# thangvubk/SoftGroup

Hardware: AMD Instinct MI355X
Metric: scans/sec ScanNet-v2-like inference (softgroup_scannet.yaml, full forward_test) (higher is better)
Workload: dtype f32

## Files before the change

### include/softgroup_hip.h

```cpp
#ifndef SOFTGROUP_HIP_H
#define SOFTGROUP_HIP_H

#include <stddef.h>
#include <stdint.h>

#ifdef __cplusplus
extern "C" {
#endif

typedef void *sg_stream_t;

#define SG_OK 0
#define SG_ERR_ARG (-1)
#define SG_ERR_WORKSPACE (-2)
#define SG_ERR_LAUNCH (-3)
#define SG_ERR_UNSUPPORTED (-4)

#define SG_BALLQUERY_MAX_NEIGHBORS 1000
#define SG_OCTREE_NUM_NODES 585
#define SG_OCTREE_NUM_LEAVES 512
#define SG_LISTS_SORTED 1
#define SG_LISTS_RADIUS 2

int sg_version(void);
const char *sg_last_error(void);
int sg_device_info(char *name_host, int name_cap, int *num_cu_host, int *clock_khz_host);

int sg_stream_release(sg_stream_t stream);
int sg_stream_create(sg_stream_t *stream_out);
int sg_stream_destroy(sg_stream_t stream);
int sg_stream_create_priority(sg_stream_t *stream_out, int level);

int sg_voxelize_idx_host(const int64_t *coords_host, int n, int ncol, int mode,
                         int32_t *input_map_host, int32_t *num_voxels_host,
                         int32_t *max_active_host);
int sg_voxelize_idx_fill_host(const int64_t *coords_host, int n, int ncol, int mode,
                              const int32_t *input_map_host, int num_voxels, int max_active,
                              int64_t *out_coords_host, int32_t *out_map_host);
size_t sg_voxelize_idx_workspace_bytes(int n);
int sg_voxelize_idx_build(const int64_t *coords, int n, int ncol, int mode, int32_t *input_map,
                          int32_t *meta, void *ws, size_t ws_bytes, sg_stream_t stream);
int sg_voxelize_idx_fill(const int64_t *coords, int n, int ncol, int mode,
                         const int32_t *input_map, int num_voxels, int max_active,
                         int64_t *out_coords, int32_t *out_map, void *ws, size_t ws_bytes,
                         sg_stream_t stream);

int sg_voxelize_fp(const float *feats, const int32_t *rules, int num_voxels, int max_active,
                   int channels, int average, float *out, sg_stream_t stream);
int sg_voxelize_bp(const float *d_out, const int32_t *rules, int num_voxels, int max_active,
                   int channels, int average, float *d_feats, sg_stream_t stream);

size_t sg_ballquery_workspace_bytes(int n);
int sg_ballquery_build_grid(const float *xyz, const int32_t *batch_idxs, int n, float radius,
                            void *ws, size_t ws_bytes, sg_stream_t stream);
int sg_ballquery_count(const float *xyz, const int32_t *batch_idxs, int n, float radius,
                       int32_t *start_len, int32_t *meta, void *ws, size_t ws_bytes,
                       sg_stream_t stream);
int sg_ballquery_fill(const float *xyz, const int32_t *batch_idxs, int n, float radius,
                      const int32_t *start_len, int32_t *idx, void *ws, size_t ws_bytes,
                      sg_stream_t stream);
size_t sg_scan_workspace_bytes(int n);
int sg_exclusive_scan_startlen(int32_t *start_len, int n, int32_t *meta, void *ws,
                               size_t ws_bytes, sg_stream_t stream);

int sg_octree_build_host(const float *points_host, const float *xyzwhl_host, int num_points,
                         int num_levels, float *boxes_host, int32_t *pt_inds_host,
                         int32_t *pt_start_len_host);
size_t sg_octree_build_workspace_bytes(int n);
int sg_octree_build(const float *points, int n, float *boxes, int32_t *pt_inds, int32_t *pt_start_len,
                    void *ws, size_t ws_bytes, sg_stream_t stream);
size_t sg_pyramid_inverse_map_workspace_bytes(int n_points, int n_voxels, int n_prop);
int sg_pyramid_inverse_map(const int32_t *proposals_idx, int64_t num_pairs, int n_prop,
                           const int32_t *l2p_map, int n_points, int n_voxels, int32_t *out_idx,
                           int32_t *out_offsets, int32_t *n_out_dev, void *ws, size_t ws_bytes,
                           sg_stream_t stream);
int sg_octree_ballquery_count(const float *points, const float *boxes, const int32_t *pt_inds,
                              const int32_t *pt_start_len, int n, float radius,
                              int32_t *start_len, sg_stream_t stream);
int sg_octree_ballquery_fill(const float *points, const float *boxes, const int32_t *pt_inds,
                             const int32_t *pt_start_len, int n, float radius,
                             const int32_t *start_len, int32_t *idx, sg_stream_t stream);

size_t sg_bfs_workspace_bytes(int n, int64_t n_edges);
int sg_bfs_cluster_label(const int32_t *bq_idxs, const int32_t *start_len, int n,
                         int64_t n_edges, int list_flags, const int32_t *seg_of_point,
                         const float *seg_thr, int n_seg, int32_t *n_cluster_host,
                         int32_t *sum_npoint_host, void *ws, size_t ws_bytes, sg_stream_t stream);
int sg_bfs_cluster_emit(const int32_t *bq_idxs, const int32_t *start_len, int n, int64_t n_edges,
                        const int32_t *seg_of_point, const float *seg_thr, int n_cluster,
                        int sum_npoint, int32_t *cluster_idxs, int32_t *cluster_offsets, void *ws,
                        size_t ws_bytes, sg_stream_t stream);

int sg_sec_mean(const float *inp, const int32_t *offsets, int n_seg, int channels, float *out,
                sg_stream_t stream);
int sg_sec_min(const float *inp, const int32_t *offsets, int n_seg, int channels, float *out,
               sg_stream_t stream);
int sg_sec_max(const float *inp, const int32_t *offsets, int n_seg, int channels, float *out,
               sg_stream_t stream);
int sg_global_avg_pool_fp(const float *feats, const int32_t *offsets, int n_seg, int channels,
                          float *out, sg_stream_t stream);
int sg_global_avg_pool_bp(float *d_feats, const int32_t *offsets, const float *d_out, int n_seg,
                          int channels, sg_stream_t stream);

int sg_get_mask_iou_on_cluster(const int32_t *proposals_idx, const int32_t *proposals_offset,
                               const int64_t *instance_labels, const int32_t *instance_pointnum,
                               int n_instance, int n_proposal, float *proposals_iou,
                               sg_stream_t stream);
int sg_get_mask_iou_on_pred(const int32_t *proposals_idx, const int32_t *proposals_offset,
                            const int64_t *instance_labels, const int32_t *instance_pointnum,
                            const float *mask_scores_sigmoid, int n_instance, int n_proposal,
                            float *proposals_iou, sg_stream_t stream);
int sg_get_mask_label(const int32_t *proposals_idx, const int32_t *proposals_offset,
                      const int64_t *instance_labels, const int64_t *instance_cls,
                      const float *proposals_iou, int n_instance, int n_proposal, float iou_thr,
                      float *mask_label, sg_stream_t stream);

size_t sg_spconv_hash_workspace_bytes(int num_rows);
int sg_spconv_subm_rulebook(const int32_t *indices, int num_rows, const int32_t *spatial_shape_host,
                            int32_t *nbr, void *ws, size_t ws_bytes, sg_stream_t stream);
int sg_spconv_down_build(const int32_t *indices, int num_rows, const int32_t *spatial_shape_host,
                         int32_t *in2out, int32_t *meta, void *ws, size_t ws_bytes,
                         sg_stream_t stream);
int sg_spconv_down_fill(const int32_t *indices, int num_rows, const int32_t *in2out,
                        int num_out_rows, int32_t *out_indices, int32_t *child, void *ws,
                        size_t ws_bytes, sg_stream_t stream);
int sg_spconv_inverse_rulebook(const int32_t *indices_fine, const int32_t *in2out, int num_rows,
                               int32_t *inv_nbr, sg_stream_t stream);

#define SG_PLAN_HIST_WORDS 40
size_t sg_spconv_plan_workspace_bytes(int num_out_rows);
int sg_spconv_plan(const int32_t *nbr, int num_out_rows, int kvol, int32_t *order,
                   uint32_t *tile_mask, int32_t *nbr_tiles, void *ws, size_t ws_bytes,
                   sg_stream_t stream);

#define SG_PYRAMID_MAX_LEVELS 10
typedef struct sg_plan_ptrs {
  int32_t *order;
  uint32_t *tile_mask;
  int32_t *nbr_tiles;
} sg_plan_ptrs;
typedef struct sg_pyramid_level {
  int rows;
  int32_t *indices;
  int32_t *nbr;
  sg_plan_ptrs subm;
  int32_t *in2out;
  int32_t *child;
  sg_plan_ptrs down;
  int32_t *inv;
  sg_plan_ptrs up;
} sg_pyramid_level;
size_t sg_spconv_pyramid_workspace_bytes(int num_rows, int n_levels);
int sg_spconv_pyramid_rows(const int32_t *indices, int num_rows, const int32_t *spatial_shape_host,
                           int n_levels, int32_t *rows_dev, void *ws, size_t ws_bytes,
                           sg_stream_t stream);
size_t sg_spconv_pyramid_build_workspace_bytes(const sg_pyramid_level *levels_host, int n_levels);
int sg_spconv_pyramid_build(const int32_t *indices, int num_rows, const int32_t *spatial_shape_host,
                            int n_levels, const sg_pyramid_level *levels_host, void *ws,
                            size_t ws_bytes, void *ws2, size_t ws2_bytes, sg_stream_t stream);

size_t sg_spconv_packed_weight_elems(int kvol, int cin, int cout);
int sg_spconv_pack_weight(const float *w, int cout, int kvol, int cin, int src_is_kio, float *w_k8,
                          sg_stream_t stream);

size_t sg_spconv_conv_workspace_bytes(int num_out_rows, int cout);
int sg_spconv_gather_conv_f32(const float *in, int num_in_rows, const int32_t *nbr,
                              int num_out_rows, int kvol, int cin, int cout, const float *w_k8,
                              const float *post_scale, const float *post_shift,
                              const float *residual, const float *act_scale,
                              const float *act_shift, float *out_act, const int32_t *order,
                              const uint32_t *tile_mask, const int32_t *nbr_tiles, float *out,
                              void *ws, size_t ws_bytes, sg_stream_t stream);

int sg_spconv_set_arithmetic(int mode);

int sg_spconv_set_combine(int mode);

int sg_grouping_set_lanes(int lanes);

int sg_spconv_set_chain(int mode);
int sg_spconv_chain_stats(int64_t *launches, int64_t *steps);

int sg_spconv_profile(int enable);
int sg_spconv_profile_read(double *total_ms, int *launches);
int sg_spconv_profile_detail(float *ms, int32_t *dims, int cap, int *calls);

typedef struct sg_mlp2 {
  const float *w1, *b1, *bn_scale, *bn_shift, *w2, *b2;
  int out;
} sg_mlp2;
int sg_pointwise_heads(const float *voxel_feats, const void *v2p_map, int v2p_is_int64, int n_points,
                       int channels, const sg_mlp2 *semantic, const sg_mlp2 *offset, float *output_feats,
                       float *semantic_scores, float *pt_offsets, int64_t *semantic_preds,
                       sg_stream_t stream);

size_t sg_spconv_packed_weight_elems_bf16(int kvol, int cin, int cout);
int sg_spconv_pack_weight_bf16(const float *w, int cout, int kvol, int cin, int src_is_kio,
                               uint16_t *w_k8_bf16, sg_stream_t stream);
size_t sg_spconv_conv_bf16_workspace_bytes(int num_out_rows, int cout);
int sg_spconv_gather_conv_bf16(const uint16_t *in, int num_in_rows, const int32_t *nbr, int num_out_rows,
                               int kvol, int cin, int cout, const uint16_t *w_k8_bf16,
                               const int32_t *order, const uint32_t *tile_mask, const int32_t *nbr_tiles,
                               uint16_t *out, void *ws, size_t ws_bytes, sg_stream_t stream);

int sg_spconv_transpose_table(const int32_t *nbr, int num_out_rows, int kvol, int32_t *nbr_t,
                              sg_stream_t stream);
size_t sg_spconv_wgrad_workspace_bytes(int num_out_rows, int kvol, int cin, int cout);
int sg_spconv_wgrad(const void *in, int in_is_bf16, const void *g_out, int g_is_bf16, const int32_t *nbr_t,
                    int num_out_rows, int kvol, int cin, int cout, float *dw_kio, void *ws,
                    size_t ws_bytes, sg_stream_t stream);

typedef struct sg_unet_block {
  int cin, cout;
  const float *bn1_scale, *bn1_shift;
  const float *w1;
  const float *bn2_scale, *bn2_shift;
  const float *w2;
  const float *w_i;
} sg_unet_block;
typedef struct sg_unet_level {
  int planes, n_blocks;
  const sg_unet_block *blocks;
  const sg_unet_block *tail;
  const float *down_bn_scale, *down_bn_shift, *down_w;
  const float *up_bn_scale, *up_bn_shift, *up_w;
} sg_unet_level;
typedef struct sg_unet_desc {
  int n_levels;
  const sg_unet_level *levels;
  int input_cin;
  const float *input_w;
  const float *out_bn_scale, *out_bn_shift;
  int input_cin_packed;
  int arithmetic;
} sg_unet_desc;
size_t sg_unet_arena_bytes(const sg_unet_desc *desc, int num_rows);
int sg_unet_forward(const sg_unet_desc *desc, const float *feats, const int32_t *indices,
                    int num_rows, const int32_t *spatial_shape_host, float *out, void *arena,
                    size_t arena_bytes, sg_stream_t stream);

typedef struct sg_train_bn {
  const float *weight, *bias;
  float *running_mean, *running_var;
  float momentum, eps;
  float *g_weight, *g_bias;
} sg_train_bn;
typedef struct sg_train_conv {
  const float *w;
  float *g_w;
} sg_train_conv;
typedef struct sg_unet_train_block {
  int cin, cout;
  sg_train_bn bn1, bn2;
  sg_train_conv c1, c2, ci;
} sg_unet_train_block;
typedef struct sg_unet_train_level {
  int planes, n_blocks;
  const sg_unet_train_block *blocks, *tail;
  sg_train_bn down_bn, up_bn;
  sg_train_conv down, up;
} sg_unet_train_level;
typedef struct sg_unet_train_desc {
  int n_levels;
  const sg_unet_train_level *levels;
  int input_cin;
  sg_train_conv input;
  sg_train_bn out_bn;
  int arithmetic;
} sg_unet_train_desc;
size_t sg_unet_train_arena_hint(const sg_unet_train_desc *desc, int num_rows);
int sg_unet_train_forward(const sg_unet_train_desc *desc, const float *feats, const int32_t *indices,
                          int num_rows, const int32_t *spatial_shape_host, float *out, void *arena,
                          size_t arena_bytes, size_t *arena_needed, void **tape, sg_stream_t stream);
int sg_unet_train_backward(void *tape, const float *g_out, float *g_feats, sg_stream_t stream);
void sg_unet_train_release(void *tape);

int sg_bn_relu_f32(const float *x, const float *scale, const float *shift, int64_t num_rows,
                   int channels, int relu, float *out, sg_stream_t stream);

int sg_gather_rows_f32(const float *in, const int32_t *index, int64_t num_out_rows, int channels,
                       float *out, sg_stream_t stream);
int sg_gather_rows_i64idx_f32(const float *in, const int64_t *index, int64_t num_out_rows,
                              int channels, float *out, sg_stream_t stream);

int sg_instance_npoint(const int32_t *proposals_idx, const float *mask_scores, int64_t num_pairs,
                       int stride, int n_classes, float mask_thr, int n_prop, int32_t *npoint,
                       sg_stream_t stream);
size_t sg_instance_runs_workspace_bytes(int n_kept, int n_points);
int sg_instance_runs(const int32_t *proposals_idx, const float *mask_scores, int64_t num_pairs,
                     int stride, int n_classes, float mask_thr, const int32_t *inst_of, int n_prop,
                     int n_kept, int n_points, int32_t *starts, int32_t *ends, int64_t *bounds,
                     int64_t runs_capacity, void *ws, size_t ws_bytes, sg_stream_t stream);

int64_t sg_rle_format_bound(int64_t total_runs, int digits);
int sg_rle_format_host(const int64_t *starts_host, const int64_t *lens_host,
                       const int64_t *bounds_host, int n_groups, char *out_host,
                       int64_t out_capacity, int64_t *out_offsets_host);
size_t sg_rle_format_device_workspace_bytes(int64_t run_capacity);
int64_t sg_rle_format_device_text_bytes(int64_t run_capacity, int64_t length);
int sg_rle_format_device(const int32_t *starts, const int32_t *ends, const int64_t *bounds, int n_inst,
                         int64_t run_capacity, int64_t length, uint8_t *text, int64_t text_capacity,
                         int64_t *text_off, void *ws, size_t ws_bytes, sg_stream_t stream);
int sg_rle_format_runs_host(const int32_t *starts_host, const int32_t *ends_host,
                            const int64_t *bounds_host, int n_groups, char *out_host,
                            int64_t out_capacity, int64_t *out_offsets_host);

size_t sg_panoptic_fusion_workspace_bytes(int n_inst, int n_points);
int sg_panoptic_fusion(const uint32_t *bits, int n_inst, int n_points, const int32_t *order,
                       const int32_t *label_id, const int64_t *semantic_preds, int cls_offset,
                       double skip_iou, int semantic_classes, int thing_class_min, uint32_t *out,
                       void *ws, size_t ws_bytes, sg_stream_t stream);

#define SG_NMS_IOU 0
#define SG_NMS_MIN 1
size_t sg_mask_nms_workspace_bytes(int n_inst, int64_t n_points);
int sg_mask_nms(const uint32_t *bits, int n_inst, int64_t n_points, const float *scores, const int32_t *labels,
                double thr, int measure, int class_agnostic, uint8_t *keep, int32_t *n_keep, int32_t *inter_out,
                void *ws, size_t ws_bytes, sg_stream_t stream);
int sg_mask_bits_from_runs(const int32_t *starts, const int32_t *ends, const int64_t *bounds, int64_t n_runs,
                           int n_inst, int64_t n_points, uint32_t *bits, sg_stream_t stream);

typedef struct sg_grouping_cfg {
  int n_points;
  int n_sem_classes;
  int n_seg;
  const int32_t *seg_class;
  const float *seg_thr;
  float score_thr;
  int min_npoint;
  float radius;
  int batch_size;
  float voxel_scale;
  int voxel_shape;
  int feat_channels;
} sg_grouping_cfg;
typedef struct sg_grouping_result {
  int n_selected, n_neighbours, n_proposals, sum_npoint, n_voxels, max_active;
  size_t proposals_idx;
  size_t proposals_offset;
  size_t voxel_coords;
  size_t voxel_offsets;
  size_t voxel_feats;
  size_t point_to_voxel;
  size_t arena_used, arena_needed;
  int deferred_classes;
  int reserved_;
} sg_grouping_result;
int sg_scan_grouping(const sg_grouping_cfg *cfg, const float *scores, const float *pt_offsets,
                     const float *coords_float, const int32_t *batch_idxs, const float *point_feats,
                     void *arena, size_t arena_bytes, sg_grouping_result *result_host,
                     sg_stream_t stream);

typedef struct sg_grouping_pp_cfg {
  sg_grouping_cfg base;
  int with_pyramid, with_octree, lvl_fusion;
  double radius;
  double base_size;
} sg_grouping_pp_cfg;
int sg_scan_grouping_pp(const sg_grouping_pp_cfg *cfg, const float *scores, const float *pt_offsets,
                        const float *coords_float, const int32_t *batch_idxs, const float *point_feats,
                        void *arena, size_t arena_bytes, sg_grouping_result *result_host,
                        sg_stream_t stream);

int sg_host_copy_2d(void *dst, int64_t dst_pitch_bytes, const void *src, int64_t src_pitch_bytes, int64_t rows,
                    int64_t row_bytes);
int sg_host_cast_f64_f32(float *dst, const double *src, int64_t n);
int sg_host_fill_i64_strided(int64_t *dst, int64_t pitch_elems, int64_t rows, int64_t value);
int sg_host_colmax_i64(const int64_t *src, int64_t rows, int64_t cols, int64_t *out_max);

typedef struct sg_instances_cfg {
  int n_proposals, n_classes;
  int score_stride;
  int64_t sum_npoint;
  int n_points;
  float cls_score_thr, mask_score_thr;
  int min_npoint;
} sg_instances_cfg;
typedef struct sg_instances_result {
  int n_kept;
  size_t off_class, off_score, off_text, text_bytes;
  size_t host_needed, arena_used, arena_needed;
  size_t bits;
  size_t label_id;
} sg_instances_result;
int sg_scan_instances(const sg_instances_cfg *cfg, const int32_t *proposals_idx, const float *mask_scores,
                      const float *cls_prob, const float *iou_scores, void *arena, size_t arena_bytes,
                      void *host_out, size_t host_bytes, sg_instances_result *result_host,
                      sg_stream_t stream);

typedef struct sg_linear {
  const float *w, *b;
  int out, in;
// ... 288 lines not shown
```

### softgroup_amd/_lib.py

```python
import ctypes as C
import os

_HERE = os.path.dirname(os.path.abspath(__file__))
LIB_PATH = os.path.join(_HERE, 'lib', os.environ.get('SG_LIB_NAME', 'libsoftgroup_hip.so'))

_lib = None

_vp, _i, _f, _i64, _sz, _d = C.c_void_p, C.c_int, C.c_float, C.c_int64, C.c_size_t, C.c_double
_pi32 = C.POINTER(C.c_int32)

SIGNATURES = {
    'sg_version': (_i, []),
    'sg_last_error': (C.c_char_p, []),
    'sg_device_info': (_i, [C.c_char_p, _i, C.POINTER(_i), C.POINTER(_i)]),
    'sg_stream_release': (_i, [_vp]),
    'sg_host_copy_2d': (_i, [_vp, _i64, _vp, _i64, _i64, _i64]),
    'sg_host_cast_f64_f32': (_i, [_vp, _vp, _i64]),
    'sg_host_fill_i64_strided': (_i, [_vp, _i64, _i64, _i64]),
    'sg_host_colmax_i64': (_i, [_vp, _i64, _i64, _vp]),
    'sg_stream_create': (_i, [_vp]),
    'sg_stream_create_priority': (_i, [_vp, _i]),
    'sg_stream_destroy': (_i, [_vp]),
    'sg_voxelize_idx_host': (_i, [_vp, _i, _i, _i, _vp, _pi32, _pi32]),
    'sg_voxelize_idx_fill_host': (_i, [_vp, _i, _i, _i, _vp, _i, _i, _vp, _vp]),
    'sg_voxelize_idx_workspace_bytes': (_sz, [_i]),
    'sg_voxelize_idx_build': (_i, [_vp, _i, _i, _i, _vp, _vp, _vp, _sz, _vp]),
    'sg_voxelize_idx_fill': (_i, [_vp, _i, _i, _i, _vp, _i, _i, _vp, _vp, _vp, _sz, _vp]),
    'sg_voxelize_fp': (_i, [_vp, _vp, _i, _i, _i, _i, _vp, _vp]),
    'sg_voxelize_bp': (_i, [_vp, _vp, _i, _i, _i, _i, _vp, _vp]),
    'sg_ballquery_workspace_bytes': (_sz, [_i]),
    'sg_ballquery_build_grid': (_i, [_vp, _vp, _i, _f, _vp, _sz, _vp]),
    'sg_ballquery_count': (_i, [_vp, _vp, _i, _f, _vp, _vp, _vp, _sz, _vp]),
    'sg_ballquery_fill': (_i, [_vp, _vp, _i, _f, _vp, _vp, _vp, _sz, _vp]),
    'sg_scan_workspace_bytes': (_sz, [_i]),
    'sg_exclusive_scan_startlen': (_i, [_vp, _i, _vp, _vp, _sz, _vp]),
    'sg_octree_build_host': (_i, [_vp, _vp, _i, _i, _vp, _vp, _vp]),
    'sg_octree_build_workspace_bytes': (_sz, [_i]),
    'sg_octree_build': (_i, [_vp, _i, _vp, _vp, _vp, _vp, _sz, _vp]),
    'sg_pyramid_inverse_map_workspace_bytes': (_sz, [_i, _i, _i]),
    'sg_pyramid_inverse_map': (_i, [_vp, _i64, _i, _vp, _i, _i, _vp, _vp, _vp, _vp, _sz, _vp]),
    'sg_octree_ballquery_count': (_i, [_vp, _vp, _vp, _vp, _i, _f, _vp, _vp]),
    'sg_octree_ballquery_fill': (_i, [_vp, _vp, _vp, _vp, _i, _f, _vp, _vp, _vp]),
    'sg_bfs_workspace_bytes': (_sz, [_i, _i64]),
    'sg_bfs_cluster_label': (_i, [_vp, _vp, _i, _i64, _i, _vp, _vp, _i, _pi32, _pi32, _vp, _sz, _vp]),
    'sg_bfs_cluster_emit': (_i, [_vp, _vp, _i, _i64, _vp, _vp, _i, _i, _vp, _vp, _vp, _sz, _vp]),
    'sg_sec_mean': (_i, [_vp, _vp, _i, _i, _vp, _vp]),
    'sg_sec_min': (_i, [_vp, _vp, _i, _i, _vp, _vp]),
    'sg_sec_max': (_i, [_vp, _vp, _i, _i, _vp, _vp]),
    'sg_global_avg_pool_fp': (_i, [_vp, _vp, _i, _i, _vp, _vp]),
    'sg_global_avg_pool_bp': (_i, [_vp, _vp, _vp, _i, _i, _vp]),
    'sg_get_mask_iou_on_cluster': (_i, [_vp, _vp, _vp, _vp, _i, _i, _vp, _vp]),
    'sg_get_mask_iou_on_pred': (_i, [_vp, _vp, _vp, _vp, _vp, _i, _i, _vp, _vp]),
    'sg_get_mask_label': (_i, [_vp, _vp, _vp, _vp, _vp, _i, _i, _f, _vp, _vp]),
    'sg_spconv_hash_workspace_bytes': (_sz, [_i]),
    'sg_spconv_subm_rulebook': (_i, [_vp, _i, _pi32, _vp, _vp, _sz, _vp]),
    'sg_spconv_pyramid_workspace_bytes': (_sz, [_i, _i]),
    'sg_spconv_pyramid_rows': (_i, [_vp, _i, _pi32, _i, _vp, _vp, _sz, _vp]),
    'sg_spconv_pyramid_build_workspace_bytes': (_sz, [_vp, _i]),
    'sg_spconv_pyramid_build': (_i, [_vp, _i, _pi32, _i, _vp, _vp, _sz, _vp, _sz, _vp]),
    'sg_spconv_down_build': (_i, [_vp, _i, _pi32, _vp, _vp, _vp, _sz, _vp]),
    'sg_spconv_down_fill': (_i, [_vp, _i, _vp, _i, _vp, _vp, _vp, _sz, _vp]),
    'sg_spconv_inverse_rulebook': (_i, [_vp, _vp, _i, _vp, _vp]),
    'sg_spconv_plan_workspace_bytes': (_sz, [_i]),
    'sg_spconv_plan': (_i, [_vp, _i, _i, _vp, _vp, _vp, _vp, _sz, _vp]),
    'sg_spconv_set_arithmetic': (_i, [_i]),
    'sg_spconv_set_combine': (_i, [_i]),
    'sg_spconv_set_chain': (_i, [_i]),
    'sg_grouping_set_lanes': (_i, [_i]),
    'sg_spconv_chain_stats': (_i, [_vp, _vp]),
    'sg_spconv_profile': (_i, [_i]),
    'sg_spconv_profile_read': (_i, [_vp, _vp]),
    'sg_spconv_profile_detail': (_i, [_vp, _vp, _i, _vp]),
    'sg_unet_arena_bytes': (_sz, [_vp, _i]),
    'sg_unet_forward': (_i, [_vp, _vp, _vp, _i, _vp, _vp, _vp, _sz, _vp]),
    'sg_unet_train_arena_hint': (_sz, [_vp, _i]),
    'sg_unet_train_forward': (_i, [_vp, _vp, _vp, _i, _vp, _vp, _vp, _sz, _vp, _vp, _vp]),
    'sg_unet_train_backward': (_i, [_vp, _vp, _vp, _vp]),
    'sg_unet_train_release': (None, [_vp]),
    'sg_pointwise_heads': (_i, [_vp, _vp, _i, _i, _i, _vp, _vp, _vp, _vp, _vp, _vp, _vp]),
    'sg_spconv_packed_weight_elems': (_sz, [_i, _i, _i]),
    'sg_spconv_pack_weight': (_i, [_vp, _i, _i, _i, _i, _vp, _vp]),
    'sg_spconv_conv_workspace_bytes': (_sz, [_i, _i]),
    'sg_spconv_gather_conv_f32': (_i, [_vp, _i, _vp, _i, _i, _i, _i, _vp, _vp, _vp, _vp, _vp, _vp,
                                       _vp, _vp, _vp, _vp, _vp, _vp, _sz, _vp]),
    'sg_spconv_packed_weight_elems_bf16': (_sz, [_i, _i, _i]),
    'sg_spconv_pack_weight_bf16': (_i, [_vp, _i, _i, _i, _i, _vp, _vp]),
    'sg_spconv_conv_bf16_workspace_bytes': (_sz, [_i, _i]),
    'sg_spconv_gather_conv_bf16': (_i, [_vp, _i, _vp, _i, _i, _i, _i, _vp, _vp, _vp, _vp, _vp, _vp, _sz,
                                        _vp]),
    'sg_spconv_transpose_table': (_i, [_vp, _i, _i, _vp, _vp]),
    'sg_spconv_wgrad_workspace_bytes': (_sz, [_i, _i, _i, _i]),
    'sg_spconv_wgrad': (_i, [_vp, _i, _vp, _i, _vp, _i, _i, _i, _i, _vp, _vp, _sz, _vp]),
    'sg_instance_npoint': (_i, [_vp, _vp, _i64, _i, _i, _f, _i, _vp, _vp]),
    'sg_instance_runs_workspace_bytes': (_sz, [_i, _i]),
    'sg_instance_runs': (_i, [_vp, _vp, _i64, _i, _i, _f, _vp, _i, _i, _i, _vp, _vp, _vp, _i64, _vp, _sz, _vp]),
    'sg_rle_format_bound': (_i64, [_i64, _i]),
    'sg_rle_format_host': (_i, [_vp, _vp, _vp, _i, _vp, _i64, _vp]),
    'sg_rle_format_device_workspace_bytes': (_sz, [_i64]),
    'sg_rle_format_device_text_bytes': (_i64, [_i64, _i64]),
    'sg_rle_format_device': (_i, [_vp, _vp, _vp, _i, _i64, _i64, _vp, _i64, _vp, _vp, _sz, _vp]),
    'sg_rle_format_runs_host': (_i, [_vp, _vp, _vp, _i, _vp, _i64, _vp]),
    'sg_panoptic_fusion_workspace_bytes': (_sz, [_i, _i]),
    'sg_panoptic_fusion': (_i, [_vp, _i, _i, _vp, _vp, _vp, _i, C.c_double, _i, _i, _vp, _vp, _sz, _vp]),
    'sg_mask_nms_workspace_bytes': (_sz, [_i, _i64]),
    'sg_mask_nms': (_i, [_vp, _i, _i64, _vp, _vp, _d, _i, _i, _vp, _vp, _vp, _vp, _sz, _vp]),
    'sg_mask_bits_from_runs': (_i, [_vp, _vp, _vp, _i64, _i, _i64, _vp, _vp]),
    'sg_scan_grouping': (_i, [_vp, _vp, _vp, _vp, _vp, _vp, _vp, _sz, _vp, _vp]),
    'sg_scan_grouping_pp': (_i, [_vp, _vp, _vp, _vp, _vp, _vp, _vp, _sz, _vp, _vp]),
    'sg_scan_instances': (_i, [_vp, _vp, _vp, _vp, _vp, _vp, _sz, _vp, _sz, _vp, _vp]),
    'sg_softmax_rows': (_i, [_vp, _i64, _i, _vp, _vp]),
    'sg_mlp_rows': (_i, [_vp, _vp, _i64, _i, _vp, _vp, _vp]),
    'sg_linear_rows': (_i, [_vp, _i64, _vp, _vp, _vp]),
    'sg_scan_arena_bytes': (_sz, [_vp, _i, _i]),
    'sg_scan_forward': (_i, [_vp, _vp, _vp, _sz, _vp, _sz, _vp, _sz, _vp, _vp]),
    'sg_eval_intersections': (_i, [_vp, _vp, _vp, _i, _i64, _vp, _i, _i, _vp, _vp]),
    'sg_eval_tally_workspace_bytes': (_sz, [_i64]),
    'sg_eval_class_tally': (_i, [_vp, _i, _vp, _i, _i64, _i64, _i, _i, _vp, _vp, _i, _vp, _vp, _vp, _vp, _vp,
                                 _vp, _sz, _vp]),
    'sg_eval_panoptic_workspace_bytes': (_sz, [_i64]),
    'sg_eval_panoptic_segments': (_i, [_vp, _i, _vp, _i, _vp, _i, _vp, _i, _i64, _i64, _i, _i64, _vp, _vp, _vp,
                                       _vp, _vp, _sz, _vp]),
    'sg_inst_rle_run_slots': (_i64, [_i64, _i]),
    'sg_inst_rle_parse': (_i, [_vp, _vp, _vp, _i, _i64, _i64, _vp, _vp, _vp, _i64, _vp, _vp, _vp]),
    'sg_inst_scan_workspace_bytes': (_sz, [_i64, _i, _i64, _i, _i, _i, _i, _vp]),
    'sg_inst_scan_update': (_i, [_vp, _i64, _vp, _vp, _vp, _i64, _vp, _vp, _vp, _i, _i, _i, _i64, _vp, _i, _i,
                                 _vp, _vp, _i64, _vp, _vp, _vp, _vp, _sz, _vp]),
    'sg_inst_scan_coverage': (_i, [_i64, _i, _i64, _i, _i, _i, _i, _vp, _vp, _vp, _i64, _d, _d, _vp, _vp, _vp, _vp,
                                   _sz, _vp]),
    'sg_inst_curves_workspace_bytes': (_sz, [_i64, _i]),
    'sg_inst_curves': (_i, [_vp, _vp, _i64, _vp, _i, _vp, _vp, _vp, _vp, _sz, _vp]),
    'sg_det_boxes_runs': (_i, [_vp, _i, _vp, _vp, _vp, _i64, _i64, _i64, _vp, _vp, _vp]),
    'sg_det_boxes_labels': (_i, [_vp, _i, _vp, _vp, _vp, _i, _i64, _i64, _vp, _vp, _vp, _vp, _vp]),
    'sg_det_match_workspace_bytes': (_sz, [_i64, _i]),
    'sg_det_match': (_i, [_vp, _vp, _vp, _i64, _vp, _vp, _i64, _vp, _i, _vp, _vp, _vp, _vp, _sz, _vp]),
    'sg_bn_relu_f32': (_i, [_vp, _vp, _vp, _i64, _i, _i, _vp, _vp]),
    'sg_gather_rows_f32': (_i, [_vp, _vp, _i64, _i, _vp, _vp]),
    'sg_gather_rows_i64idx_f32': (_i, [_vp, _vp, _i64, _i, _vp, _vp]),
    'sg_train_augment': (_i, [_vp, _i64, _i, _f, _vp, C.c_double, C.c_double, _vp, _vp, _vp, _vp]),
    'sg_train_blur': (_i, [_vp, _vp, _i, _i, _i, _i, _vp]),
    'sg_train_elastic': (_i, [_vp, _i64, _vp, _i, _i, _i, C.c_double, C.c_double, _vp, _vp]),
    'sg_train_crop_count': (_i, [_vp, _i64, C.c_double, _vp, _vp, _i, _vp, _vp]),
    'sg_train_compact_workspace_bytes': (_sz, [_i64]),
    'sg_train_compact': (_i, [_vp, _vp, _vp, _i, _vp, _vp, _vp, _i64, C.c_double, _vp, _vp, _i64, _vp, _vp, _vp, _vp,
                              _vp, _vp, _vp, _sz, _vp]),
    'sg_train_gather': (_i, [_vp, _i64, _vp, _vp, _i, _vp, _vp, _vp, _vp, _vp, _vp, _vp]),
    'sg_train_id_set_workspace_bytes': (_sz, []),
    'sg_train_id_set': (_i, [_vp, _i64, _i64, _vp, _i, _vp, _sz, _vp]),
    'sg_train_remap': (_i, [_vp, _i64, _vp, _vp, _i, _vp]),
    'sg_train_instance_workspace_bytes': (_sz, [_i64, _i]),
    'sg_train_instance_info': (_i, [_vp, _vp, _vp, _i64, _i, _i64, _vp, _vp, _vp, _vp, _sz, _vp]),
    'sg_test_x4_minima': (_i, [_vp, _i64, _vp, C.c_double, _vp, _vp]),
    'sg_test_x4_split': (_i, [_vp, _vp, _i, _vp, _vp, _i64, _vp, C.c_double, _vp, _vp, _vp, _vp, _vp, _vp, _vp]),
    'sg_kitti_decode_labels': (_i, [_vp, _i64, _vp, _vp, _vp, _vp, _vp]),
    'sg_mask_text_runs': (_i, [_vp, _vp, _vp, _i64, _i, _i64, _i, _i, _vp, _i64, _vp]),
    'sg_mask_text_bits': (_i, [_vp, _i, _i64, _i, _i, _vp, _i64, _vp]),
    'sg_decimal_lines_workspace_bytes': (_sz, [_i64]),
    'sg_decimal_lines': (_i, [_vp, _i64, _vp, _i, _vp, _i64, _vp, _vp, _sz, _vp]),
    'sg_panoptic_kitti_words': (_i, [_vp, _i64, _vp, _i, _vp, _vp, _vp, _vp]),
    'sg_parse_decimal_lines_workspace_bytes': (_sz, [_i64]),
    'sg_parse_decimal_lines': (_i, [_vp, _i64, _vp, _i64, _vp, _vp, _sz, _vp]),
    'sg_parse_mask_text': (_i, [_vp, _i64, _vp, _vp, _vp, _vp]),
    'sg_viz_paint_bits': (_i, [_vp, _i, _i64, _vp, _vp, _vp, _vp, _vp]),
    'sg_viz_paint_runs_workspace_bytes': (_sz, [_i, _i64]),
    'sg_viz_paint_runs': (_i, [_vp, _vp, _vp, _i64, _i, _i64, _vp, _vp, _vp, _vp, _vp, _sz, _vp]),
    'sg_viz_gt_labels': (_i, [_vp, _i64, _vp, _vp, _vp]),
    'sg_viz_instance_rank_workspace_bytes': (_sz, [_i]),
    'sg_viz_instance_rank': (_i, [_vp, _i, _vp, _vp, _sz, _vp]),
    'sg_viz_colors': (_i, [_i, _vp, _vp, _vp, _vp, _i, _vp, _i, _i64, _vp, _vp, _vp]),
    'sg_viz_ply_vertices_workspace_bytes': (_sz, [_i64]),
    'sg_viz_ply_vertices': (_i, [_vp, _vp, _vp, _vp, _i64, _vp, _i64, _vp, _vp, _sz, _vp]),
    'sg_loss_reduce_workspace_bytes': (_sz, []),
    'sg_pointwise_loss_fwd': (_i, [_vp, _vp, _vp, _i64, _vp, _vp, _vp, _i64, _i, _vp, _vp, _sz, _vp]),
    'sg_pointwise_loss_bwd': (_i, [_vp, _vp, _vp, _i64, _vp, _vp, _vp, _i64, _i, _vp, _vp, _vp, _vp, _vp, _vp]),
    'sg_assign_proposals_workspace_bytes': (_sz, [_i]),
    'sg_assign_proposals': (_i, [_vp, _vp, _i64, _f, _i, _f, _i64, _i, _i, _vp, _vp, _sz, _vp]),
    'sg_proposal_loss_fwd': (_i, [_vp, _vp, _vp, _vp, _vp, _i64, _i, _i, _i, _vp, _vp, _vp, _sz, _vp]),
    'sg_proposal_loss_bwd': (_i, [_vp, _vp, _vp, _vp, _vp, _vp, _vp, _i, _i, _vp, _vp, _vp]),
    'sg_mask_loss_fwd': (_i, [_vp, _vp, _vp, _vp, _i64, _i, _i, _vp, _vp, _vp, _sz, _vp]),
    'sg_mask_loss_bwd': (_i, [_vp, _vp, _vp, _vp, _vp, _vp, _i64, _i, _i, _vp, _vp]),
    'sg_optim_chunk_elems': (_i, []),
    'sg_optim_plan': (_i64, [_vp, _i, _vp, _i64]),
    'sg_optim_workspace_bytes': (_sz, []),
    'sg_optim_grad_norm': (_i, [_vp, _i, _vp, _i64, _vp, _f, _vp, _vp, _sz, _vp]),
    'sg_optim_adam_step': (_i, [_vp, _i, _vp, _i64, _d, _d, _d, _d, _d, _i, _vp, _vp, _vp, _i, _vp, _vp]),
    'sg_optim_sgd_step': (_i, [_vp, _i, _vp, _i64, _d, _d, _d, _d, _i, _vp, _vp, _vp, _i, _vp, _vp]),
    'sg_optim_scale_grads': (_i, [_vp, _i, _vp, _i64, _vp, _vp]),
    'sg_grid_downsample_workspace_bytes': (_sz, [_i]),
    'sg_grid_downsample': (_i, [_vp, _i, _d, _i, _vp, _vp, _vp, _vp, _sz, _vp]),
    'sg_nearest_default_cell': (_d, [_vp, _vp, _i64]),
    'sg_nearest_grid_bytes': (_sz, [_i]),
    'sg_nearest_build': (_i, [_vp, _i, _d, _vp, _sz, _vp, _vp]),
    'sg_nearest_query_workspace_bytes': (_sz, [_i]),
    'sg_nearest_query': (_i, [_vp, _i, _d, _vp, _sz, _vp, _i, _d, _vp, _vp, _vp, _vp, _sz, _vp]),
    'sg_mask_bits_gather': (_i, [_vp, _i, _i64, _vp, _i64, _vp, _vp, _vp]),
    'sg_mask_runs_workspace_bytes': (_sz, [_i, _i64]),
    'sg_mask_runs_count': (_i, [_vp, _i, _i64, _vp, _vp, _sz, _vp]),
    'sg_mask_runs_fill': (_i, [_vp, _i, _i64, _vp, _sz, _vp, _vp, _i64, _vp]),
}


class SoftGroupHipError(RuntimeError):
    pass


def lib():
    global _lib
    if _lib is None:
        import torch
        if not os.path.exists(LIB_PATH):
            raise SoftGroupHipError(
                f'{LIB_PATH} not found: the HIP extension is required (no CPU fallback). '
                'Build it with `python -c "import __graft_entry__ as g; g.build()"`.')
        L = C.CDLL(LIB_PATH)
        for name, (res, args) in SIGNATURES.items():
            fn = getattr(L, name)
            fn.restype = res
            fn.argtypes = args
        _lib = L
    return _lib


def check(rc, what=''):
    if rc != 0:
        msg = lib().sg_last_error()
        raise SoftGroupHipError(f'{what} failed ({rc}): {msg.decode() if msg else ""}')


def ptr(t):
    return None if t is None else t.data_ptr()


_raw_stream = None


def stream():
    global _raw_stream
    import torch
# ... 10 lines not shown
```

### softgroup_amd/csrc/common.h

```cpp
#pragma once
#include <hip/hip_runtime.h>
#include <stdint.h>
#include <stdio.h>

#include "../../include/softgroup_hip.h"

namespace sg {

constexpr int kWave = 64;

void set_error(const char *fmt, ...);
int32_t *pinned_words();

inline hipStream_t as_stream(sg_stream_t s) { return reinterpret_cast<hipStream_t>(s); }

inline int check_launch(const char *what) {
  hipError_t e = hipGetLastError();
  if (e != hipSuccess) {
    set_error("%s: %s", what, hipGetErrorString(e));
    return SG_ERR_LAUNCH;
  }
  return SG_OK;
}

// ... 9 lines not shown

struct Workspace {
  char *base;
  size_t size, off;
  Workspace(void *p, size_t n) : base(static_cast<char *>(p)), size(n), off(0) {}
  template <typename T>
  T *take(size_t count) {
    size_t bytes = align_up(count * sizeof(T));
    if (off + bytes > size) return nullptr;
    T *r = reinterpret_cast<T *>(base + off);
    off += bytes;
    return r;
  }
};

inline int grid_for(int64_t work_items, int block, int max_blocks = 256 * 8) {
  int64_t g = (work_items + block - 1) / block;
  if (g < 1) g = 1;
  if (g > max_blocks) g = max_blocks;
  return static_cast<int>(g);
}

__device__ __forceinline__ int lane_id() { return threadIdx.x & 63; }

__device__ __forceinline__ uint64_t mix64(uint64_t x) {
  x ^= x >> 33;
  x *= 0xff51afd7ed558ccdULL;
  x ^= x >> 33;
  x *= 0xc4ceb9fe1a85ec53ULL;
  return x ^ (x >> 33);
}

__device__ __forceinline__ int mask_prefix(uint64_t m) {
  return __builtin_amdgcn_mbcnt_hi(static_cast<uint32_t>(m >> 32),
                                   __builtin_amdgcn_mbcnt_lo(static_cast<uint32_t>(m), 0u));
}

template <int CTRL, int ROW_MASK = 0xf, int BANK_MASK = 0xf>
__device__ __forceinline__ int dpp_or_zero(int v) {
  return __builtin_amdgcn_update_dpp(0, v, CTRL, ROW_MASK, BANK_MASK, false);
}
__device__ __forceinline__ int wave_incl_scan(int v) {
  v += dpp_or_zero<0x111>(v);
  v += dpp_or_zero<0x112>(v);
  v += dpp_or_zero<0x114>(v);
  v += dpp_or_zero<0x118>(v);
  v += dpp_or_zero<0x142, 0xa>(v);
  v += dpp_or_zero<0x143, 0xc>(v);
  return v;
}
__device__ __forceinline__ int wave_sum(int v) {
  return __builtin_amdgcn_readlane(wave_incl_scan(v), 63);
}
__device__ __forceinline__ int wave_max(int v) {
#pragma unroll
  for (int o = 32; o > 0; o >>= 1) v = max(v, __shfl_xor(v, o, 64));
  return v;
}

template <int G>
__device__ __forceinline__ int group_lane() { return static_cast<int>(threadIdx.x) & (G - 1); }
template <int G>
__device__ __forceinline__ uint64_t group_mask() { return G == 64 ? ~0ull : ((1ull << (G & 63)) - 1ull); }
template <int G>
__device__ __forceinline__ uint64_t group_ballot(bool p) {
  const uint64_t b = __ballot(p);
  if (G == 64) return b;
  return (b >> (lane_id() & ~(G - 1))) & group_mask<G>();
}
template <int G>
__device__ __forceinline__ bool group_any(bool p) { return group_ballot<G>(p) != 0ull; }
template <int G>
__device__ __forceinline__ int group_mask_prefix(uint64_t m) {
  if (G == 64) return mask_prefix(m);
  return __popcll(m & ((1ull << group_lane<G>()) - 1ull));
}
template <int G>
__device__ __forceinline__ int group_incl_scan(int v) {
  static_assert(G == 8 || G == 16 || G == 32 || G == 64, "lane groups are 8, 16, 32 or 64 lanes");
  if (G == 8) {
    const int gl = group_lane<8>();
    int t = dpp_or_zero<0x111>(v);
    v += gl >= 1 ? t : 0;
    t = dpp_or_zero<0x112>(v);
    v += gl >= 2 ? t : 0;
    t = dpp_or_zero<0x114>(v);
    v += gl >= 4 ? t : 0;
    return v;
  }
  v += dpp_or_zero<0x111>(v);
  v += dpp_or_zero<0x112>(v);
  v += dpp_or_zero<0x114>(v);
  v += dpp_or_zero<0x118>(v);
  if (G >= 32) v += dpp_or_zero<0x142, 0xa>(v);
  if (G == 64) v += dpp_or_zero<0x143, 0xc>(v);
  return v;
}
int grouping_lanes_for(int64_t n_edges, int n);
int grouping_lanes_forced();

constexpr int kFillMax = 16;
struct FillList {
  uint32_t *p[kFillMax];
  size_t words[kFillMax];
  uint32_t pattern[kFillMax];
  int n = 0;
  void add(void *ptr, size_t bytes, int byte) {
    if (bytes == 0 || ptr == nullptr || n >= kFillMax) return;
    p[n] = static_cast<uint32_t *>(ptr);
    words[n] = bytes / 4;
    pattern[n] = 0x01010101u * static_cast<uint32_t>(byte & 0xff);
    ++n;
  }
};
static __global__ void __launch_bounds__(256) fill_many_kernel(FillList f) {
  const int r = blockIdx.y;
  uint32_t *p = f.p[r];
  const size_t w = f.words[r];
  const uint32_t v = f.pattern[r];
  const size_t head = (16 - (reinterpret_cast<uintptr_t>(p) & 15)) / 4 % 4;
  const size_t h = head < w ? head : w;
  const size_t quads = (w - h) / 4;
  uint4 *q = reinterpret_cast<uint4 *>(p + h);
  const uint4 vv = make_uint4(v, v, v, v);
  for (size_t i = blockIdx.x * 256ull + threadIdx.x; i < quads; i += gridDim.x * 256ull) q[i] = vv;
  if (blockIdx.x == 0) {
    if (threadIdx.x < h) p[threadIdx.x] = v;
    const size_t t0 = h + quads * 4;
    if (threadIdx.x < w - t0) p[t0 + threadIdx.x] = v;
  }
}
inline void fill_many(const FillList &f, hipStream_t stream) {
  if (f.n == 0) return;
  size_t mx = 0;
  for (int i = 0; i < f.n; ++i) mx = f.words[i] > mx ? f.words[i] : mx;
  const int gx = grid_for(static_cast<int64_t>(mx / 4 + 1), 256, 1024);
  fill_many_kernel<<<dim3(gx, f.n), 256, 0, stream>>>(f);
}

extern thread_local int t_conv_arith;
void conv_chain_begin(hipStream_t stream);
bool conv_chain_recording();
int conv_chain_end();
void conv_chain_abort();
int conv_chain_concat(const float *a, const float *b, int64_t rows, int ca, int cb, const float *scale,
                      const float *shift, float *out, float *out_act);
int conv_chain_bn_relu(const float *x, const float *scale, const float *shift, int64_t rows, int c, float *out);
int conv_chain_check_abort(const char *who);
int conv_gather_rows(const void *in, int num_in_rows, const int32_t *nbr, int M_out, int K, int Cin, int Cout,
                     const float *w_k8, const float *post_scale, const float *post_shift, const void *residual,
                     const float *act_scale, const float *act_shift, void *out_act, const int32_t *order,
                     const uint32_t *tile_mask, const int32_t *nbr_tiles, void *out, void *ws, size_t ws_bytes,
                     sg_stream_t stream, int in16, int out16, int res16);
int spconv_wgrad_layout(const void *in, int in_bf16, const void *g_out, int g_bf16, const int32_t *nbr_t, int M_out,
                        int K, int Cin, int Cout, float *dw, int out_oki, void *ws, size_t ws_bytes,
                        sg_stream_t stream);
struct PackJob {
  const float *w;
  float *out;
  int cout, kvol, cin, mode;
};
int spconv_pack_weights(const PackJob *jobs, int n, sg_stream_t stream);
size_t octree_stash_bytes(int n);
int octree_ballquery_count_stash(const float *points, const float *boxes, const int32_t *pt_inds,
                                 const int32_t *pt_start_len, int n, float radius, int32_t *start_len, int32_t *stash,
                                 hipStream_t stream);
int octree_ballquery_fill_stash(const float *points, const float *boxes, const int32_t *pt_inds,
                                const int32_t *pt_start_len, int n, float radius, const int32_t *start_len,
                                const int32_t *stash, int32_t *idx, hipStream_t stream);
void conv_release_stream(int dev, hipStream_t stream);
void unet_release_stream(int dev, hipStream_t stream);
void scan_release_stream(int dev, hipStream_t stream);
void bfs_release_stream(int dev, hipStream_t stream);
constexpr int kBfsGiantMin = 16384;
struct BfsDefer {
  bool deferred = false;
  hipStream_t side = nullptr;
};
void bfs_emit_defer(BfsDefer *d);
int bfs_emit_join(const BfsDefer &d, hipStream_t stream);
int bfs_label_max_kept(const void *ws);
int bfs_count_kept_members(const void *ws, size_t ws_bytes, int n, int64_t n_edges, const int32_t *l2p, int n_pts,
                           const float *thr_dev, int32_t *out, hipStream_t stream);

}
```

### softgroup_amd/csrc/spconv_conv.hip

```cpp
#include <stdlib.h>

#include <atomic>
#include <cstdio>
#include <map>
#include <mutex>
#include <utility>
#include <vector>

#include "common.h"

namespace sg {

typedef float f32x16 __attribute__((ext_vector_type(16)));
typedef float f4 __attribute__((ext_vector_type(4)));
typedef float f2 __attribute__((ext_vector_type(2)));
typedef __bf16 bf16x8 __attribute__((ext_vector_type(8)));
typedef __bf16 bf16x2 __attribute__((ext_vector_type(2)));

__device__ __forceinline__ void split3(const float (&x)[8], bf16x8 &h, bf16x8 &m, bf16x8 &l) {
#pragma unroll
  for (int j = 0; j < 4; ++j) {
    const f2 v = {x[2 * j], x[2 * j + 1]};
    const bf16x2 hh = __builtin_convertvector(v, bf16x2);
    const f2 r = v - __builtin_convertvector(hh, f2);
    const bf16x2 mm = __builtin_convertvector(r, bf16x2);
    const f2 r2 = r - __builtin_convertvector(mm, f2);
    const bf16x2 ll = __builtin_convertvector(r2, bf16x2);
    h[2 * j] = hh[0]; h[2 * j + 1] = hh[1];
    m[2 * j] = mm[0]; m[2 * j + 1] = mm[1];
    l[2 * j] = ll[0]; l[2 * j + 1] = ll[1];
  }
}
__device__ __forceinline__ bf16x8 round_bf16(const float (&x)[8]) {
  bf16x8 h;
#pragma unroll
  for (int j = 0; j < 4; ++j) {
    const f2 v = {x[2 * j], x[2 * j + 1]};
    const bf16x2 hh = __builtin_convertvector(v, bf16x2);
    h[2 * j] = hh[0]; h[2 * j + 1] = hh[1];
  }
  return h;
}
__device__ __forceinline__ uint16_t bf16_rne(float x) {
  const uint32_t u = __builtin_bit_cast(uint32_t, x);
  return static_cast<uint16_t>((u + 0x7fffu + ((u >> 16) & 1u)) >> 16);
}
__device__ __forceinline__ float bf16_f32(uint16_t b) {
  return __builtin_bit_cast(float, static_cast<uint32_t>(b) << 16);
}

#ifndef SG_WHATIF
#define SG_WHATIF 0
#endif

constexpr int kTileRows = 32;
constexpr int kWavesPerWg = 4;
constexpr int kCk = 16;
constexpr int kMaxK = 27;
constexpr int kTicketStride = 32;
constexpr unsigned kOob = 0x80000000u;

__device__ __forceinline__ void lds_dma_b128(const void *gsrc, unsigned lds_dst) {
  unsigned keep;
  asm volatile("s_mov_b32 %0, m0\n\ts_mov_b32 m0, %2\n\ts_nop 0\n\tglobal_load_lds_dwordx4 %1, off\n\t"
               "s_mov_b32 m0, %0"
               : "=&s"(keep) : "v"(gsrc), "s"(lds_dst) : "memory");
}
__device__ __forceinline__ void lds_dma_b32(const void *gsrc, unsigned lds_dst) {
  unsigned keep;
  asm volatile("s_mov_b32 %0, m0\n\ts_mov_b32 m0, %2\n\ts_nop 0\n\tglobal_load_lds_dword %1, off\n\t"
               "s_mov_b32 m0, %0"
               : "=&s"(keep) : "v"(gsrc), "s"(lds_dst) : "memory");
}

struct ConvArgs {
  const float *in;
  const int32_t *nbr;
  const float *w;
  const float *post_scale;
  const float *post_shift;
  const float *residual;
  const float *act_scale;
  const float *act_shift;
  float *out_act;
  const int32_t *order;
  const uint32_t *tile_mask;
  const int32_t *nbr_tiles;
  float *out;
  int M_out, K, Cin, Cout;
  int col_units;
  int blocks_per_unit;
  int ksplit;
  int k_per_split;
  int num_units;
  unsigned magic_upt, magic_cu, magic_nsl;
  int out16, res16;
  int dyn_rounds;
  unsigned *queue;
  unsigned long long *trace;
  unsigned *done;
  float *out_final;
};

template <int NBW, bool VEC>
__global__ void __launch_bounds__(256) gather_conv_tile_kernel(ConvArgs p) {
  extern __shared__ __attribute__((aligned(16))) char smem_raw[];
  const int wave = threadIdx.x >> 6, lane = threadIdx.x & 63;
  int32_t *nbr_lds = reinterpret_cast<int32_t *>(smem_raw) + wave * kTileRows * kMaxK;
  const int cin_pad = (p.Cin + kCk - 1) / kCk * kCk;
  const int c8 = (p.Cin + 7) / 8;

  const int num_tiles = (p.M_out + kTileRows - 1) / kTileRows;
  const int units_per_tile = p.col_units * p.ksplit;
  const long long unit = static_cast<long long>(blockIdx.x) * kWavesPerWg + wave;
  const bool valid = unit < static_cast<long long>(num_tiles) * units_per_tile;
  int tile = valid ? static_cast<int>(unit / units_per_tile) : 0;
  const int sub = valid ? static_cast<int>(unit % units_per_tile) : 0;
  const int cu = sub % p.col_units, ks = sub / p.col_units;
  const int nb0 = cu * p.blocks_per_unit;
  const int nbw = valid ? min(p.blocks_per_unit, (p.Cout + 31) / 32 - nb0) : 0;
  const int k_lo = ks * p.k_per_split, k_hi = min(p.K, k_lo + p.k_per_split);

  const int arow = lane & 31, ahalf = lane >> 5;
  int my_row = -1;
  if (valid) {
    const int pos = tile * kTileRows + arow;
    if (p.order) my_row = p.order[pos];
    else if (pos < p.M_out) my_row = pos;
  }
  if (valid) {
    for (int e = lane; e < kTileRows * p.K; e += 64) {
      const int r = e / p.K, k = e - r * p.K;
      const int row = __shfl(my_row, r, 64);
      nbr_lds[r * kMaxK + k] = row >= 0 ? p.nbr[static_cast<long long>(row) * p.K + k] : -1;
    }
  }
  __syncthreads();
  if (!valid) return;

  uint32_t mask = p.tile_mask ? p.tile_mask[tile] : 0xffffffffu;
  mask &= (k_hi >= 32 ? 0xffffffffu : ((1u << k_hi) - 1u)) & ~((1u << k_lo) - 1u);

  f32x16 acc[NBW];
#pragma unroll
  for (int n = 0; n < NBW; ++n)
#pragma unroll
    for (int r = 0; r < 16; ++r) acc[n][r] = 0.f;

  const int n_slices = cin_pad / kCk;
  const int col = nb0 * 32 + arow;
  int coff[NBW];
#pragma unroll
  for (int n = 0; n < NBW; ++n) coff[n] = min(col + min(n, nbw - 1) * 32, p.Cout - 1);

  auto load_raw = [&](int k, int s, float (&a)[8], float (&b)[NBW][8]) {
    const int c = s * kCk + ahalf * 8;
    const int src = nbr_lds[arow * kMaxK + k];
    const bool present = src >= 0;
    const float *row = p.in + static_cast<unsigned>((present ? src : 0) * p.Cin + c);
    if (VEC) {
      const float4 v0 = *reinterpret_cast<const float4 *>(row);
      const float4 v1 = *reinterpret_cast<const float4 *>(row + 4);
      a[0] = v0.x; a[1] = v0.y; a[2] = v0.z; a[3] = v0.w;
      a[4] = v1.x; a[5] = v1.y; a[6] = v1.z; a[7] = v1.w;
#pragma unroll
      for (int j = 0; j < 8; ++j) a[j] = present ? a[j] : 0.f;
    } else {
#pragma unroll
      for (int j = 0; j < 8; ++j) {
        const float v = row[max(0, min(j, p.Cin - 1 - c))];
        a[j] = (present && c + j < p.Cin) ? v : 0.f;
      }
    }
    const int blk = min(c >> 3, c8 - 1);
    const unsigned wbase = static_cast<unsigned>((k * c8 + blk) * p.Cout) * 8u;
#pragma unroll
    for (int n = 0; n < NBW; ++n) {
      const float4 w0 = *reinterpret_cast<const float4 *>(p.w + wbase + coff[n] * 8);
      const float4 w1 = *reinterpret_cast<const float4 *>(p.w + wbase + coff[n] * 8 + 4);
      b[n][0] = w0.x; b[n][1] = w0.y; b[n][2] = w0.z; b[n][3] = w0.w;
      b[n][4] = w1.x; b[n][5] = w1.y; b[n][6] = w1.z; b[n][7] = w1.w;
    }
  };

  float a_cur[8], a_nxt[8];
  float b_cur[NBW][8], b_nxt[NBW][8];

  int k = mask ? __builtin_ctz(mask) : -1;
  int s = 0;
  if (k >= 0) load_raw(k, 0, a_nxt, b_nxt);
  while (k >= 0) {
#pragma unroll
    for (int j = 0; j < 8; ++j) {
      a_cur[j] = a_nxt[j];
#pragma unroll
      for (int n = 0; n < NBW; ++n) b_cur[n][j] = b_nxt[n][j];
    }
    int k2 = k, s2 = s + 1;
    if (s2 == n_slices) {
      s2 = 0;
      const uint32_t rest = mask & ~((2u << k) - 1u);
      k2 = rest ? __builtin_ctz(rest) : -1;
    }
    if (k2 >= 0) load_raw(k2, s2, a_nxt, b_nxt);
    __builtin_amdgcn_sched_barrier(0);
#pragma unroll
    for (int j = 0; j < 8; ++j)
#pragma unroll
      for (int n = 0; n < NBW; ++n)
        acc[n] = __builtin_amdgcn_mfma_f32_32x32x2f32(a_cur[j], b_cur[n][j], acc[n], 0, 0, 0);
    __builtin_amdgcn_sched_barrier(0);
    k = k2;
    s = s2;
  }

  const bool final_out = p.ksplit == 1;
  float *out = p.out + (final_out ? 0 : static_cast<long long>(ks) * p.M_out * p.Cout);
  const bool add_res = p.residual != nullptr && final_out;
  const bool post = p.post_scale != nullptr && final_out;
  const bool act = p.out_act != nullptr && final_out;
  float ps[NBW], pb[NBW], as[NBW], ab[NBW];
#pragma unroll
  for (int n = 0; n < NBW; ++n) {
    ps[n] = post ? p.post_scale[coff[n]] : 1.f;
    pb[n] = post ? p.post_shift[coff[n]] : 0.f;
    as[n] = act ? p.act_scale[coff[n]] : 1.f;
    ab[n] = act ? p.act_shift[coff[n]] : 0.f;
  }
#pragma unroll
  for (int reg = 0; reg < 16; ++reg) {
    const int r = (reg & 3) + 8 * (reg >> 2) + 4 * ahalf;
    const int row = __shfl(my_row, r, 64);
    if (row < 0) continue;
    const long long off = static_cast<long long>(row) * p.Cout + col;
#pragma unroll
    for (int n = 0; n < NBW; ++n) {
      if (n < nbw && col + n * 32 < p.Cout) {
        float v = acc[n][reg];
        if (add_res) v += p.residual[off + n * 32];
        if (post) v = fmaxf(fmaf(v, ps[n], pb[n]), 0.f);
        out[off + n * 32] = v;
        if (act) p.out_act[off + n * 32] = fmaxf(fmaf(v, as[n], ab[n]), 0.f);
      }
    }
  }
}

constexpr int kRowsAt = kTileRows * kMaxK, kMaskAt = kRowsAt + kTileRows;
constexpr int kMetaInts = kMaskAt + 4;

template <int CK, int DEPTH, int TRACE, int NBW, int SPLIT, int WV, int AT, int CHAIN, int R16 = 0>
__device__ __forceinline__ void conv_layer_body(const ConvArgs &p, unsigned in_bytes, unsigned w_bytes) {
  static_assert(!R16 || (SPLIT == 2 && AT), "bf16 rows: bf16-operand arithmetic, line-wise gather");
  constexpr int AUX = CHAIN ? 16 : 0;
  static_assert(!SPLIT || CK == 16 || AT, "split-precision path: 16-channel slices");
  static_assert(!AT || (SPLIT && CK == 32), "line-wise gather: split path, 32-channel items");
  static_assert(WV == 2 || WV == 4 || WV == 8 || WV == 16, "2, 4, 8 or 16 waves per workgroup");
  constexpr int RR = 16 / WV;
  constexpr int WV_SHIFT = WV == 2 ? 1 : WV == 4 ? 2 : WV == 8 ? 3 : 4;
  constexpr int HC = CK / 2;
  constexpr int NQ = HC / 4;
  extern __shared__ __attribute__((aligned(16))) char smem_raw[];
  const int wave = __builtin_amdgcn_readfirstlane(threadIdx.x >> 6), lane = threadIdx.x & 63;
  const int arow = lane & 31, ahalf = lane >> 5;
  float *red = reinterpret_cast<float *>(smem_raw);
  int32_t *meta_lds = reinterpret_cast<int32_t *>(red + WV * NBW * 16 * 64);

  const int G = gridDim.x;
  const int units_per_tile = p.col_units * p.ksplit;
  const int num_units = p.num_units;
  const int n_slices = R16 ? (p.Cin + 63) / 64 : p.Cin / CK;
  const int c8 = p.Cin / 8;
  const int tileK = kTileRows * p.K;
  const int nbr_base = arow * p.K;
  const bool final_out = p.ksplit == 1;
  const bool add_res = p.residual != nullptr && final_out;
  const bool post = p.post_scale != nullptr && final_out;
  const bool act = p.out_act != nullptr && final_out;
  const bool combine = p.done != nullptr && !final_out;
  const int num_tiles = (p.M_out + kTileRows - 1) / kTileRows;
  const unsigned out_bytes = static_cast<unsigned>(p.M_out) * p.Cout * 4u;
  const bool out16 = SPLIT == 2 && p.out16 != 0, res16 = SPLIT == 2 && p.res16 != 0;
  const unsigned fin_bytes = out16 ? out_bytes >> 1 : out_bytes;
  const unsigned res_bytes = res16 ? out_bytes >> 1 : out_bytes;

  const __amdgpu_buffer_rsrc_t rs_in =
      __builtin_amdgcn_make_buffer_rsrc(const_cast<float *>(p.in), 0, in_bytes, 0x00020000);
  const __amdgpu_buffer_rsrc_t rs_w =
      __builtin_amdgcn_make_buffer_rsrc(const_cast<float *>(p.w), 0, w_bytes, 0x00020000);
  const __amdgpu_buffer_rsrc_t rs_res = __builtin_amdgcn_make_buffer_rsrc(
      const_cast<float *>(add_res ? p.residual : p.in), 0, add_res ? res_bytes : 0u, 0x00020000);
  const __amdgpu_buffer_rsrc_t rs_out = __builtin_amdgcn_make_buffer_rsrc(
      p.out, 0, final_out ? fin_bytes : out_bytes * static_cast<unsigned>(p.ksplit), 0x00020000);
  const __amdgpu_buffer_rsrc_t rs_act = __builtin_amdgcn_make_buffer_rsrc(
      act ? p.out_act : p.out, 0, act ? fin_bytes : 0u, 0x00020000);
  const bool c_res = combine && p.residual != nullptr, c_act = combine && p.out_act != nullptr;
  const __amdgpu_buffer_rsrc_t rs_cres = __builtin_amdgcn_make_buffer_rsrc(
      const_cast<float *>(c_res ? p.residual : p.in), 0, c_res ? res_bytes : 0u, 0x00020000);
  const __amdgpu_buffer_rsrc_t rs_cout = __builtin_amdgcn_make_buffer_rsrc(
      combine ? p.out_final : p.out, 0, combine ? fin_bytes : 0u, 0x00020000);
  const __amdgpu_buffer_rsrc_t rs_cact = __builtin_amdgcn_make_buffer_rsrc(
      c_act ? p.out_act : p.out, 0, c_act ? fin_bytes : 0u, 0x00020000);
  auto ld_row = [&](const __amdgpu_buffer_rsrc_t &rs, unsigned off, int n, bool h16) -> float {
    if constexpr (SPLIT == 2) {
      if (h16)
        return bf16_f32(static_cast<uint16_t>(__builtin_amdgcn_raw_buffer_load_b16(rs, off >> 1, n * 64, AUX)));
    }
    return __builtin_bit_cast(float, __builtin_amdgcn_raw_buffer_load_b32(rs, off, n * 128, AUX));
  };
  auto st_row = [&](float v, const __amdgpu_buffer_rsrc_t &rs, unsigned off, unsigned base, int n, bool h16) {
    if constexpr (SPLIT == 2) {
      if (h16) {
        __builtin_amdgcn_raw_buffer_store_b16(static_cast<short>(bf16_rne(v)), rs, off >> 1, base + n * 64, AUX);
        return;
      }
    }
    __builtin_amdgcn_raw_buffer_store_b32(__builtin_bit_cast(unsigned, v), rs, off, base + n * 128, AUX);
  };

  auto udiv = [](unsigned x, unsigned magic) { return magic ? __umulhi(x, magic) : x; };

  const int group = 8 * units_per_tile;
  const int full = num_units / group * group;
  struct Unit { int tile, cu, ks; };
  auto decode = [&](int u) {
    Unit d;
    int sub;
    if (u < full) {
      const int blk = udiv(u >> 3, p.magic_upt);
      const int i = u - blk * group;
      d.tile = blk * 8 + (i & 7);
      sub = i >> 3;
    } else {
      d.tile = udiv(u, p.magic_upt);
      sub = u - d.tile * units_per_tile;
    }
    d.ks = udiv(sub, p.magic_cu);
    d.cu = sub - d.ks * p.col_units;
    return d;
  };

  int32_t *ctl = meta_lds + 2 * kMetaInts;
  const unsigned meta_lds_addr = __builtin_amdgcn_readfirstlane(
      static_cast<unsigned>(reinterpret_cast<uintptr_t>(meta_lds)));
  auto dma_meta = [&](int tile, int buf) {
    const unsigned dst = meta_lds_addr + static_cast<unsigned>(buf * kMetaInts) * 4u;
    const int32_t *blk = p.nbr_tiles + static_cast<long long>(tile) * tileK;
#pragma unroll
    for (int q = 0; q < 4; ++q) {
      const int e = q * 256 + lane * 4;
      if (e < tileK) lds_dma_b128(blk + e, dst + q * 1024);
    }
    if (lane < kTileRows) lds_dma_b32(p.order + tile * kTileRows + lane, dst + kRowsAt * 4);
    if (lane == 0) lds_dma_b32(p.tile_mask + tile, dst + kMaskAt * 4);
  };
  (void)num_tiles;

  constexpr int NPL = SPLIT == 2 ? 1 : 3;
  constexpr int NB_ = R16 ? 4 : AT ? 2 * NPL : SPLIT ? NPL : NQ;
  struct Slice { f4 a[NQ]; f4 b[NBW][NB_]; int nsl; };
  const int plane_bytes = p.K * c8 * p.Cout * 16;
  const int planes_at = 2 * plane_bytes;
  struct Ctx {
    const int32_t *meta;
    uint32_t wg_mask;
    int col, ks, k, s, kp, sp, rem;
    int pair;
    int v_w;
    float ps[NBW], pb[NBW], as[NBW], ab[NBW];
    unsigned o_off[RR];
    bool col_ok;
  };

  Slice S[DEPTH];
  float resv[NBW][RR];

  f4 *tr_lds = reinterpret_cast<f4 *>(ctl + 4) + wave * 256;
  const unsigned row_pitch = static_cast<unsigned>(p.Cin) * 4u, lane_chunk = static_cast<unsigned>(lane & 7) * 16u;
  auto load = [&](const Ctx &c, int k, int s, Slice &S) {
    if constexpr (R16) {
#pragma unroll
      for (int q = 0; q < 4; ++q) {
        const unsigned src = static_cast<unsigned>(c.meta[(8 * q + (lane >> 3)) * p.K + k]);
        const unsigned v_a = __umul24(src, row_pitch >> 1) + lane_chunk;
        S.a[q] = __builtin_bit_cast(f4, __builtin_amdgcn_raw_buffer_load_b128(rs_in, v_a, s * 128, AUX));
      }
      const int s_w = planes_at + (k * c8 + s * 8) * p.Cout * 16;
      const int nsl = s * 64 + 64 <= p.Cin ? 4 : 2;
      S.nsl = nsl;
#pragma unroll
      for (int n = 0; n < NBW; ++n)
#pragma unroll
        for (int sl = 0; sl < 4; ++sl)
          S.b[n][sl] = __builtin_bit_cast(f4, __builtin_amdgcn_raw_buffer_load_b128(
                                                  rs_w, c.v_w + n * 512, s_w + (sl < nsl ? sl : sl - 2) * (2 * p.Cout * 16), 0));
      return;
    }
    if constexpr (AT) {
#pragma unroll
      for (int q = 0; q < 4; ++q) {
        unsigned src = static_cast<unsigned>(c.meta[(8 * q + (lane >> 3)) * p.K + k]);
        if (SG_WHATIF & 16) src = static_cast<unsigned>(c.pair * 32 + 8 * q + (lane >> 3)) % static_cast<unsigned>(p.M_out);
        const unsigned v_a = __umul24(src, row_pitch) + lane_chunk;
        S.a[q] = __builtin_bit_cast(f4, __builtin_amdgcn_raw_buffer_load_b128(rs_in, v_a, s * 128, AUX));
      }
      const int s_w = planes_at + (k * c8 + s * 4) * p.Cout * 16;
#pragma unroll
      for (int n = 0; n < NBW; ++n)
#pragma unroll
        for (int sl = 0; sl < 2; ++sl)
#pragma unroll
          for (int pl = 0; pl < NPL; ++pl) {
            if ((SG_WHATIF & 1) && pl > 0) { S.b[n][sl * NPL + pl] = S.b[n][sl * NPL]; continue; }
            S.b[n][sl * NPL + pl] = __builtin_bit_cast(f4, __builtin_amdgcn_raw_buffer_load_b128(
                                                             rs_w, c.v_w + n * 512,
                                                             s_w + sl * (2 * p.Cout * 16) + pl * plane_bytes, 0));
          }
      return;
    }
    const int src = c.meta[nbr_base + k];
    const unsigned v_a = src >= 0 ? static_cast<unsigned>(src * p.Cin + ahalf * HC) * 4u : kOob;
    const int s_a = s * (CK * 4);
#pragma unroll
    for (int q = 0; q < NQ; ++q)
      S.a[q] = __builtin_bit_cast(f4, __builtin_amdgcn_raw_buffer_load_b128(rs_in, v_a + q * 16, s_a, AUX));
    if constexpr (SPLIT) {
      const int s_w = planes_at + (k * c8 + s * 2) * p.Cout * 16;
#pragma unroll
      for (int n = 0; n < NBW; ++n)
#pragma unroll
        for (int pl = 0; pl < NPL; ++pl)
          S.b[n][pl] = __builtin_bit_cast(f4, __builtin_amdgcn_raw_buffer_load_b128(
                                                  rs_w, c.v_w + n * 512, s_w + pl * plane_bytes, 0));
    } else {
      const int s_w = (k * c8 + s * (CK / 8)) * p.Cout * 32;
#pragma unroll
      for (int n = 0; n < NBW; ++n)
#pragma unroll
        for (int q = 0; q < NQ; ++q)
          S.b[n][q] = __builtin_bit_cast(f4, __builtin_amdgcn_raw_buffer_load_b128(
                                                 rs_w, c.v_w + n * 1024 + (q & 1) * 16,
                                                 s_w + (q >> 1) * (p.Cout * 32), 0));
    }
  };

  auto advance = [&](const Ctx &c, int &k, int &s) {
    if (++s == n_slices) {
      s = 0;
      const uint32_t rest = c.wg_mask & ~((2u << k) - 1u);
      k = rest ? __builtin_ctz(rest) : k;
    }
  };

  auto setup = [&](const Unit &d, int buf, Ctx &c) {
    c.ks = d.ks;
    c.pair = d.tile * p.col_units + d.cu;
    c.meta = meta_lds + buf * kMetaInts;
    uint32_t m = static_cast<uint32_t>(c.meta[kMaskAt]);
    if (!final_out) {
      const int k_lo = d.ks * p.k_per_split, k_hi = min(p.K, k_lo + p.k_per_split);
      m &= ((1u << k_hi) - 1u) & ~((1u << k_lo) - 1u);
    }
    m = __builtin_amdgcn_readfirstlane(m);
    c.wg_mask = m;
    c.col = d.cu * (32 * NBW) + arow;
    c.col_ok = c.col < p.Cout;
    const int colc = min(c.col, p.Cout - 1);
    c.v_w = SPLIT ? (ahalf * p.Cout + colc) * 16 : (ahalf * (HC / 8) * p.Cout + colc) * 32;
    const int items = __builtin_popcount(m) * n_slices;
    const int per = (items + WV - 1) >> WV_SHIFT;
    const int begin = min(items, wave * per);
    c.rem = min(items, begin + per) - begin;
    int rank = udiv(begin, p.magic_nsl);
    c.s = begin - rank * n_slices;
    uint32_t mm = m;
    for (; rank > 0; --rank) mm &= mm - 1u;
    c.k = mm ? __builtin_ctz(mm) : 0;
    load(c, c.k, c.s, S[0]);
    c.kp = c.k;
    c.sp = c.s;
#pragma unroll
    for (int i = 1; i < DEPTH - 1; ++i) {
      if (i < c.rem) advance(c, c.kp, c.sp);
      load(c, c.kp, c.sp, S[i]);
    }
    int row4[RR];
#pragma unroll
    for (int rr = 0; rr < RR; ++rr) {
      const int reg = wave * RR + rr;
      row4[rr] = c.meta[kRowsAt + (reg & 3) + 8 * (reg >> 2) + 4 * ahalf];
    }
#pragma unroll
    for (int rr = 0; rr < RR; ++rr) {
      const unsigned off = (row4[rr] >= 0 && c.col_ok)
                               ? static_cast<unsigned>(row4[rr] * p.Cout + c.col) * 4u : kOob;
      c.o_off[rr] = off;
#pragma unroll
      for (int n = 0; n < NBW; ++n)
        resv[n][rr] = ld_row(rs_res, off, n, res16);
    }
#pragma unroll
    for (int n = 0; n < NBW; ++n) {
      c.ps[n] = c.pb[n] = c.as[n] = c.ab[n] = 0.f;
      if (post) {
        c.ps[n] = p.post_scale[colc + 32 * n];
        c.pb[n] = p.post_shift[colc + 32 * n];
      }
      if (act) {
        c.as[n] = p.act_scale[colc + 32 * n];
        c.ab[n] = p.act_shift[colc + 32 * n];
      }
    }
  };

  f32x16 acc[NBW];
  auto compute = [&](Slice &S) {
    if constexpr (R16) {
#pragma unroll
      for (int q = 0; q < 4; ++q) {
        const int r = 8 * q + (lane >> 3);
        tr_lds[r * 8 + ((lane & 7) ^ ((r >> 1) & 7))] = S.a[q];
      }
      f4 fr[4];
#pragma unroll
      for (int sl = 0; sl < 4; ++sl) fr[sl] = tr_lds[arow * 8 + ((sl * 2 + ahalf) ^ ((arow >> 1) & 7))];
      const int nsl = __builtin_amdgcn_readfirstlane(S.nsl);
#pragma unroll
      for (int sl = 0; sl < 4; ++sl) {
        if (sl >= 2 && nsl == 2) break;
#pragma unroll
        for (int n = 0; n < NBW; ++n)
          acc[n] = __builtin_amdgcn_mfma_f32_32x32x16_bf16(__builtin_bit_cast(bf16x8, fr[sl]),
                                                           __builtin_bit_cast(bf16x8, S.b[n][sl]), acc[n], 0, 0, 0);
      }
      return;
    }
    if constexpr (AT) {
#pragma unroll
      for (int q = 0; q < 4; ++q) {
        const int r = 8 * q + (lane >> 3);
        if (!(SG_WHATIF & 8)) tr_lds[r * 8 + ((lane & 7) ^ ((r >> 1) & 7))] = S.a[q];
      }
      f4 fr[2][2];
#pragma unroll
      for (int sl = 0; sl < 2; ++sl)
#pragma unroll
        for (int j = 0; j < 2; ++j)
          fr[sl][j] = (SG_WHATIF & 8) ? S.a[sl * 2 + j] : tr_lds[arow * 8 + ((sl * 4 + ahalf * 2 + j) ^ ((arow >> 1) & 7))];
#pragma unroll
      for (int sl = 0; sl < 2; ++sl) {
        const float af[8] = {fr[sl][0][0], fr[sl][0][1], fr[sl][0][2], fr[sl][0][3],
                             fr[sl][1][0], fr[sl][1][1], fr[sl][1][2], fr[sl][1][3]};
        if constexpr (SPLIT == 2) {
          const bf16x8 ah = round_bf16(af);
#pragma unroll
          for (int n = 0; n < NBW; ++n)
            acc[n] = __builtin_amdgcn_mfma_f32_32x32x16_bf16(ah, __builtin_bit_cast(bf16x8, S.b[n][sl]), acc[n],
                                                             0, 0, 0);
          continue;
        }
        bf16x8 ah, am, al;
        if (SG_WHATIF & 2) {
          ah = __builtin_bit_cast(bf16x8, fr[sl][0]);
          am = __builtin_bit_cast(bf16x8, fr[sl][1]);
          al = ah;
        } else {
          split3(af, ah, am, al);
        }
#pragma unroll
        for (int n = 0; n < NBW; ++n) {
          const bf16x8 bh = __builtin_bit_cast(bf16x8, S.b[n][sl * 3 + 0]);
          const bf16x8 bm = __builtin_bit_cast(bf16x8, S.b[n][sl * 3 + 1]);
          const bf16x8 bl = __builtin_bit_cast(bf16x8, S.b[n][sl * 3 + 2]);
          if (SG_WHATIF & 4) {
            typedef int i4 __attribute__((ext_vector_type(4)));
            const i4 ax = __builtin_bit_cast(i4, al) ^ __builtin_bit_cast(i4, am) ^ __builtin_bit_cast(i4, ah);
            const i4 bx = __builtin_bit_cast(i4, bh) ^ __builtin_bit_cast(i4, bm) ^ __builtin_bit_cast(i4, bl);
            acc[n] = __builtin_amdgcn_mfma_f32_32x32x16_bf16(__builtin_bit_cast(bf16x8, ax), __builtin_bit_cast(bf16x8, bx),
                                                             acc[n], 0, 0, 0);
            continue;
          }
          acc[n] = __builtin_amdgcn_mfma_f32_32x32x16_bf16(al, bh, acc[n], 0, 0, 0);
          acc[n] = __builtin_amdgcn_mfma_f32_32x32x16_bf16(am, bm, acc[n], 0, 0, 0);
          acc[n] = __builtin_amdgcn_mfma_f32_32x32x16_bf16(ah, bl, acc[n], 0, 0, 0);
          acc[n] = __builtin_amdgcn_mfma_f32_32x32x16_bf16(am, bh, acc[n], 0, 0, 0);
          acc[n] = __builtin_amdgcn_mfma_f32_32x32x16_bf16(ah, bm, acc[n], 0, 0, 0);
          acc[n] = __builtin_amdgcn_mfma_f32_32x32x16_bf16(ah, bh, acc[n], 0, 0, 0);
        }
      }
      return;
    }
    if constexpr (SPLIT) {
      const float af[8] = {S.a[0][0], S.a[0][1], S.a[0][2], S.a[0][3], S.a[1][0], S.a[1][1], S.a[1][2], S.a[1][3]};
      if constexpr (SPLIT == 2) {
        const bf16x8 ah = round_bf16(af);
#pragma unroll
        for (int n = 0; n < NBW; ++n)
          acc[n] = __builtin_amdgcn_mfma_f32_32x32x16_bf16(ah, __builtin_bit_cast(bf16x8, S.b[n][0]), acc[n], 0,
                                                           0, 0);
        return;
      }
      bf16x8 ah, am, al;
      split3(af, ah, am, al);
#pragma unroll
      for (int n = 0; n < NBW; ++n) {
        const bf16x8 bh = __builtin_bit_cast(bf16x8, S.b[n][0]);
        const bf16x8 bm = __builtin_bit_cast(bf16x8, S.b[n][1]);
        const bf16x8 bl = __builtin_bit_cast(bf16x8, S.b[n][2]);
        acc[n] = __builtin_amdgcn_mfma_f32_32x32x16_bf16(al, bh, acc[n], 0, 0, 0);
        acc[n] = __builtin_amdgcn_mfma_f32_32x32x16_bf16(am, bm, acc[n], 0, 0, 0);
        acc[n] = __builtin_amdgcn_mfma_f32_32x32x16_bf16(ah, bl, acc[n], 0, 0, 0);
        acc[n] = __builtin_amdgcn_mfma_f32_32x32x16_bf16(am, bh, acc[n], 0, 0, 0);
        acc[n] = __builtin_amdgcn_mfma_f32_32x32x16_bf16(ah, bm, acc[n], 0, 0, 0);
        acc[n] = __builtin_amdgcn_mfma_f32_32x32x16_bf16(ah, bh, acc[n], 0, 0, 0);
      }
      return;
    }
#pragma unroll
    for (int q = 0; q < NQ; ++q) {
      asm volatile("" : "+v"(S.a[q]));
#pragma unroll
      for (int n = 0; n < NBW; ++n) asm volatile("" : "+v"(S.b[n][q]));
    }
    __builtin_amdgcn_sched_barrier(0);
#pragma unroll
    for (int q = 0; q < NQ; ++q)
#pragma unroll
      for (int j = 0; j < 4; ++j)
#pragma unroll
        for (int n = 0; n < NBW; ++n)
          acc[n] = __builtin_amdgcn_mfma_f32_32x32x2f32(S.a[q][j], S.b[n][q][j], acc[n], 0, 0, 0);
  };

  unsigned long long stamp[8];
  auto mark = [&](int i) {
    if constexpr (TRACE) stamp[i] = __builtin_readcyclecounter();
  };

  const int xcd = blockIdx.x & 7;
  const int dyn0 = (p.dyn_rounds == 1 ? 1 : 2) * G;
  const bool draws = p.queue != nullptr && dyn0 < num_units;
  const bool draw_first = draws && p.dyn_rounds == 1;
  auto barrier = [] {
    asm volatile("s_waitcnt lgkmcnt(0)\n\ts_barrier" ::: "memory");
  };

  if (static_cast<int>(blockIdx.x) >= num_units) return;
  int round = 0, u = blockIdx.x, buf = 0;
  Unit du = decode(u);
  unsigned ticket = 0;
  bool drawing = true;
  if (wave == 0) {
    if (lane == 0 && draw_first)
      ticket = __hip_atomic_fetch_add(p.queue + xcd * kTicketStride, 1u, __ATOMIC_RELAXED, __HIP_MEMORY_SCOPE_AGENT);
    dma_meta(du.tile, 0);
    asm volatile("s_waitcnt vmcnt(0)" ::: "memory");
  }
  barrier();
  Ctx c;
  setup(du, 0, c);

  while (true) {
    mark(0);
    int un_w0 = -1;
    if (wave == 0) {
      if ((round == 0 && !draw_first) || !draws) {
        const int r = round + 1;
        const int b = static_cast<int>(blockIdx.x);
        const int rev = (G & 7) == 0 ? G - 8 - (b & ~7) + (b & 7) : G - 1 - b;
        un_w0 = r * G + ((__builtin_popcount(r) & 1) ? rev : b);
      } else if (drawing) {
        const unsigned t = __builtin_amdgcn_readfirstlane(ticket);
        un_w0 = dyn0 + static_cast<int>(t) * 8 + xcd;
      }
      if (un_w0 >= num_units || un_w0 < 0) {
        un_w0 = -1;
        drawing = false;
      }
      if (un_w0 >= 0) dma_meta(decode(un_w0).tile, buf ^ 1);
      if (lane == 0) ctl[buf ^ 1] = un_w0;
    }
#pragma unroll
    for (int n = 0; n < NBW; ++n)
#pragma unroll
      for (int r = 0; r < 16; ++r) acc[n][r] = 0.f;
    {
      int kp = c.kp, sp = c.sp, issued = DEPTH - 1;
      const int rem = c.rem;
      for (int g = rem / DEPTH; g > 0; --g) {
#pragma unroll
        for (int i = 0; i < DEPTH; ++i) {
          int k2 = kp, s2 = sp;
          advance(c, k2, s2);
          const bool more = issued < rem;
          kp = more ? k2 : kp;
          sp = more ? s2 : sp;
          ++issued;
          load(c, kp, sp, S[(i + DEPTH - 1) % DEPTH]);
          __builtin_amdgcn_sched_barrier(0);
          compute(S[i]);
          __builtin_amdgcn_sched_barrier(0);
        }
      }
      const int tail = rem % DEPTH;
#pragma unroll
      for (int i = 0; i < DEPTH - 1; ++i)
        if (i < tail) compute(S[i]);
    }
    if constexpr (TRACE) { asm volatile("" : "+v"(acc[0][0])); }
    mark(1);

    if (wave == 0) {
      asm volatile("s_waitcnt vmcnt(0)" ::: "memory");
      if (lane == 0 && draws)
        ticket = __hip_atomic_fetch_add(p.queue + xcd * kTicketStride, 1u, __ATOMIC_RELAXED,
                                        __HIP_MEMORY_SCOPE_AGENT);
    }

    barrier();
    mark(2);
#pragma unroll
    for (int n = 0; n < NBW; ++n)
#pragma unroll
      for (int reg = 0; reg < 16; ++reg) red[((wave * NBW + n) * 16 + reg) * 64 + lane] = acc[n][reg];
    barrier();
    mark(3);
    const int un = __builtin_amdgcn_readfirstlane(ctl[buf ^ 1]);
    const bool has_next = un >= 0;
    const Unit dn = decode(has_next ? un : u);

    float v[NBW][RR], va[NBW][RR];
    unsigned o_off[RR];
    {
      float part[NBW][RR][WV];
#pragma unroll
      for (int n = 0; n < NBW; ++n)
#pragma unroll
        for (int rr = 0; rr < RR; ++rr) {
          const int reg = wave * RR + rr;
#pragma unroll
          for (int w = 0; w < WV; ++w) part[n][rr][w] = red[((w * NBW + n) * 16 + reg) * 64 + lane];
        }
#pragma unroll
      for (int rr = 0; rr < RR; ++rr) {
#pragma unroll
        for (int n = 0; n < NBW; ++n) {
          float t = part[n][rr][0];
#pragma unroll
          for (int w = 1; w < WV; ++w) t += part[n][rr][w];
          t += resv[n][rr];
          if (post) t = fmaxf(fmaf(t, c.ps[n], c.pb[n]), 0.f);
          v[n][rr] = t;
          va[n][rr] = fmaxf(fmaf(t, c.as[n], c.ab[n]), 0.f);
        }
        o_off[rr] = c.o_off[rr];
      }
    }
    const unsigned o_base = final_out ? 0u : static_cast<unsigned>(c.ks) * out_bytes;
    const int rem_done = c.rem;
    const int pair_done = c.pair, col_done = c.col;
    setup(dn, has_next ? (buf ^ 1) : buf, c);
    mark(4);
    if (combine) {
#pragma unroll
      for (int rr = 0; rr < RR; ++rr)
#pragma unroll
        for (int n = 0; n < NBW; ++n)
          __builtin_amdgcn_raw_buffer_store_b32(__builtin_bit_cast(unsigned, v[n][rr]), rs_out, o_off[rr],
                                                o_base + n * 128, 16);
    } else {
#pragma unroll
    for (int rr = 0; rr < RR; ++rr)
#pragma unroll
      for (int n = 0; n < NBW; ++n) st_row(v[n][rr], rs_out, o_off[rr], o_base, n, out16 && final_out);
    }
    if (act) {
#pragma unroll
      for (int rr = 0; rr < RR; ++rr)
#pragma unroll
        for (int n = 0; n < NBW; ++n) st_row(va[n][rr], rs_act, o_off[rr], 0u, n, out16);
    }
    if (combine) {
      asm volatile("s_waitcnt vmcnt(0)" ::: "memory");
      barrier();
      if (wave == 0 && lane == 0) {
        const unsigned arrived = __hip_atomic_fetch_add(p.done + pair_done, 1u, __ATOMIC_RELAXED,
                                                        __HIP_MEMORY_SCOPE_AGENT);
        ctl[3] = arrived == static_cast<unsigned>(p.ksplit - 1);
      }
      barrier();
      if (__builtin_amdgcn_readfirstlane(ctl[3]) != 0) {
        const int colc = min(col_done, p.Cout - 1);
        float ps[NBW], pb[NBW], as[NBW], ab[NBW];
#pragma unroll
        for (int n = 0; n < NBW; ++n) {
          ps[n] = pb[n] = as[n] = ab[n] = 0.f;
          if (p.post_scale) { ps[n] = p.post_scale[colc + 32 * n]; pb[n] = p.post_shift[colc + 32 * n]; }
          if (c_act) { as[n] = p.act_scale[colc + 32 * n]; ab[n] = p.act_shift[colc + 32 * n]; }
        }
        auto part = [&](int ks, int rr, int n) {
          return __builtin_bit_cast(float, __builtin_amdgcn_raw_buffer_load_b32(
                                               rs_out, o_off[rr], static_cast<unsigned>(ks) * out_bytes + n * 128, 16));
        };
        float t[NBW][RR];
#pragma unroll
        for (int rr = 0; rr < RR; ++rr)
#pragma unroll
          for (int n = 0; n < NBW; ++n) t[n][rr] = part(0, rr, n);
        int ks = 1;
        for (; ks + 3 < p.ksplit; ks += 4) {
          float q[4][NBW][RR];
#pragma unroll
          for (int j = 0; j < 4; ++j)
#pragma unroll
            for (int rr = 0; rr < RR; ++rr)
#pragma unroll
              for (int n = 0; n < NBW; ++n) q[j][n][rr] = part(ks + j, rr, n);
#pragma unroll
          for (int j = 0; j < 4; ++j)
#pragma unroll
            for (int rr = 0; rr < RR; ++rr)
#pragma unroll
              for (int n = 0; n < NBW; ++n) t[n][rr] += q[j][n][rr];
        }
        for (; ks < p.ksplit; ++ks) {
          float q[NBW][RR];
#pragma unroll
          for (int rr = 0; rr < RR; ++rr)
#pragma unroll
            for (int n = 0; n < NBW; ++n) q[n][rr] = part(ks, rr, n);
#pragma unroll
          for (int rr = 0; rr < RR; ++rr)
#pragma unroll
            for (int n = 0; n < NBW; ++n) t[n][rr] += q[n][rr];
        }
        float res[NBW][RR];
#pragma unroll
        for (int rr = 0; rr < RR; ++rr)
#pragma unroll
          for (int n = 0; n < NBW; ++n)
            res[n][rr] = ld_row(rs_cres, o_off[rr], n, res16);
#pragma unroll
        for (int rr = 0; rr < RR; ++rr)
#pragma unroll
          for (int n = 0; n < NBW; ++n) {
            float x = t[n][rr] + res[n][rr];
            if (p.post_scale) x = fmaxf(fmaf(x, ps[n], pb[n]), 0.f);
            st_row(x, rs_cout, o_off[rr], 0u, n, out16);
            st_row(fmaxf(fmaf(x, as[n], ab[n]), 0.f), rs_cact, o_off[rr], 0u, n, out16);
          }
      }
    }
    mark(5);
    if constexpr (TRACE) {
      if (lane == 0 && p.trace && wave < kWavesPerWg) {
        unsigned long long *t = p.trace + (static_cast<long long>(u) * kWavesPerWg + wave) * 8;
        for (int i = 0; i < 6; ++i) t[i] = stamp[i];
        unsigned hw, xcc;
        asm volatile("s_getreg_b32 %0, hwreg(HW_REG_HW_ID)" : "=s"(hw));
        asm volatile("s_getreg_b32 %0, hwreg(HW_REG_XCC_ID)" : "=s"(xcc));
        t[6] = static_cast<unsigned long long>(blockIdx.x);
        t[7] = (static_cast<unsigned long long>(rem_done) << 48) | (static_cast<unsigned long long>(xcc & 0xf) << 32) | hw;
      }
    }
    if (!has_next) break;
    u = un;
    ++round;
    buf ^= 1;
  }
}

template <int CK, int DEPTH, int TRACE, int WPE, int NBW = 1, int SPLIT = 0, int WV = 4, int AT = 0, int R16 = 0>
__global__ void __launch_bounds__(64 * WV, WPE) gather_conv_persistent_kernel(ConvArgs p, unsigned in_bytes,
                                                                             unsigned w_bytes) {
  conv_layer_body<CK, DEPTH, TRACE, NBW, SPLIT, WV, AT, 0, R16>(p, in_bytes, w_bytes);
}

struct ChainStep {
  const float *in, *w, *post_scale, *post_shift, *residual, *act_scale, *act_shift;
  float *out_act;
  const int32_t *order;
  const uint32_t *tile_mask;
  const int32_t *nbr_tiles;
  float *out;
  unsigned *done;
  float *out_final;
  int M_out, K, Cin, Cout, col_units, ksplit, k_per_split, num_units;
  unsigned magic_upt, magic_cu, magic_nsl, in_bytes, w_bytes;
  int kind;
  int pad_[2];
};
constexpr int kChainMax = 22;
struct ChainArgs {
  ChainStep s[kChainMax];
  unsigned *bar;
  unsigned *abort_host;
  unsigned long long *trace;
  int n;
};
static_assert(sizeof(ChainArgs) <= 4096, "the step list must fit the kernel-argument segment");
constexpr int kChainWV = 8;
constexpr int kChainBarWords = 18 * 32;
constexpr unsigned long long kChainTimeout = 200000000ull;

__device__ __forceinline__ bool chain_barrier(unsigned *bar, unsigned epoch, unsigned *abort_host, int *flag_lds,
                                              unsigned long long *stamp) {
  asm volatile("s_waitcnt vmcnt(0)" ::: "memory");
  __syncthreads();
  if (threadIdx.x == 0) {
    if (stamp) stamp[2] = __builtin_amdgcn_s_memrealtime();
    const unsigned x = blockIdx.x & 7, nx = (gridDim.x + 7u - x) >> 3;
    int ok = 1;
    const unsigned old = __hip_atomic_fetch_add(bar + x * 32, 1u, __ATOMIC_RELAXED, __HIP_MEMORY_SCOPE_AGENT);
    if (old == nx * epoch - 1u) {
      const unsigned groups = gridDim.x < 8u ? gridDim.x : 8u;
      const unsigned o2 = __hip_atomic_fetch_add(bar + 8 * 32, 1u, __ATOMIC_RELAXED, __HIP_MEMORY_SCOPE_AGENT);
      if (o2 == groups * epoch - 1u)
        for (unsigned j = 0; j < groups; ++j)
          __hip_atomic_store(bar + (9 + j) * 32, epoch, __ATOMIC_RELAXED, __HIP_MEMORY_SCOPE_AGENT);
    }
    const unsigned long long t0 = __builtin_amdgcn_s_memrealtime();
    unsigned spins = 0;
    while (__hip_atomic_load(bar + (9 + x) * 32, __ATOMIC_RELAXED, __HIP_MEMORY_SCOPE_AGENT) < epoch) {
      __builtin_amdgcn_s_sleep(2);
      if ((++spins & 255u) == 0u) {
        if (__hip_atomic_load(bar + 17 * 32, __ATOMIC_RELAXED, __HIP_MEMORY_SCOPE_AGENT) != 0u) { ok = 0; break; }
        if (__builtin_amdgcn_s_memrealtime() - t0 > kChainTimeout) {
          __hip_atomic_store(bar + 17 * 32, 1u, __ATOMIC_RELAXED, __HIP_MEMORY_SCOPE_AGENT);
          __hip_atomic_store(abort_host, 1u, __ATOMIC_RELAXED, __HIP_MEMORY_SCOPE_SYSTEM);
          ok = 0;
          break;
        }
      }
    }
    *flag_lds = ok;
    if (stamp) stamp[3] = __builtin_amdgcn_s_memrealtime();
  }
  __syncthreads();
  return *flag_lds != 0;
}

__device__ __forceinline__ void chain_elementwise(const ChainStep &s) {
  const int ca4 = s.Cin >> 2, cb4 = s.kind == 1 ? s.Cout >> 2 : 0, c4 = ca4 + cb4;
  const unsigned total = static_cast<unsigned>(s.M_out) * c4;
  const __amdgpu_buffer_rsrc_t ra = __builtin_amdgcn_make_buffer_rsrc(
      const_cast<float *>(s.in), 0, static_cast<unsigned>(s.M_out) * ca4 * 16u, 0x00020000);
  const __amdgpu_buffer_rsrc_t rb = __builtin_amdgcn_make_buffer_rsrc(
      const_cast<float *>(cb4 ? s.residual : s.in), 0, static_cast<unsigned>(s.M_out) * cb4 * 16u, 0x00020000);
  const __amdgpu_buffer_rsrc_t ro = __builtin_amdgcn_make_buffer_rsrc(s.out, 0, total * 16u, 0x00020000);
  const __amdgpu_buffer_rsrc_t roa = __builtin_amdgcn_make_buffer_rsrc(
      s.out_act ? s.out_act : s.out, 0, s.out_act ? total * 16u : 0u, 0x00020000);
  const float *sc = s.kind == 1 ? s.act_scale : s.post_scale, *sh = s.kind == 1 ? s.act_shift : s.post_shift;
  for (unsigned t = blockIdx.x * blockDim.x + threadIdx.x; t < total; t += gridDim.x * blockDim.x) {
    const unsigned r = t / c4, c = t - r * c4;
    f4 v;
    if (c < static_cast<unsigned>(ca4))
      v = __builtin_bit_cast(f4, __builtin_amdgcn_raw_buffer_load_b128(ra, (r * ca4 + c) * 16u, 0, 16));
    else
      v = __builtin_bit_cast(f4, __builtin_amdgcn_raw_buffer_load_b128(rb, (r * cb4 + (c - ca4)) * 16u, 0, 16));
    f4 a = v;
    if (sc != nullptr) {
      const f4 k = *reinterpret_cast<const f4 *>(sc + 4 * c), h = *reinterpret_cast<const f4 *>(sh + 4 * c);
#pragma unroll
      for (int j = 0; j < 4; ++j) a[j] = fmaxf(fmaf(v[j], k[j], h[j]), 0.f);
    }
    if (s.kind == 1) {
      __builtin_amdgcn_raw_buffer_store_b128(__builtin_bit_cast(__attribute__((ext_vector_type(4))) unsigned, v), ro, t * 16u, 0, 16);
      __builtin_amdgcn_raw_buffer_store_b128(__builtin_bit_cast(__attribute__((ext_vector_type(4))) unsigned, a), roa, t * 16u, 0, 16);
    } else {
      __builtin_amdgcn_raw_buffer_store_b128(__builtin_bit_cast(__attribute__((ext_vector_type(4))) unsigned, a), ro, t * 16u, 0, 16);
    }
  }
}

template <int SPLIT>
__global__ void __launch_bounds__(64 * kChainWV, 1) conv_chain_kernel(ChainArgs a) {
  extern __shared__ __attribute__((aligned(16))) char smem_raw[];
  int *flag_lds = reinterpret_cast<int *>(smem_raw) + kChainWV * 16 * 64 + 2 * kMetaInts + 2;
#pragma nounroll
  for (int i = 0; i < a.n; ++i) {
    const ChainStep &s = a.s[i];
    unsigned long long *stamp = a.trace ? a.trace + (static_cast<size_t>(i) * gridDim.x + blockIdx.x) * 4 : nullptr;
    if (stamp && threadIdx.x == 0) stamp[0] = __builtin_amdgcn_s_memrealtime();
    if (s.kind == 0) {
      ConvArgs p;
      p.in = s.in; p.nbr = nullptr; p.w = s.w; p.post_scale = s.post_scale; p.post_shift = s.post_shift;
      p.residual = s.residual; p.act_scale = s.act_scale; p.act_shift = s.act_shift; p.out_act = s.out_act;
      p.order = s.order; p.tile_mask = s.tile_mask; p.nbr_tiles = s.nbr_tiles; p.out = s.out;
      p.M_out = s.M_out; p.K = s.K; p.Cin = s.Cin; p.Cout = s.Cout;
      p.col_units = s.col_units; p.blocks_per_unit = 1; p.ksplit = s.ksplit; p.k_per_split = s.k_per_split;
      p.num_units = s.num_units;
      p.magic_upt = s.magic_upt; p.magic_cu = s.magic_cu; p.magic_nsl = s.magic_nsl;
      p.queue = nullptr; p.dyn_rounds = 2; p.out16 = 0; p.res16 = 0; p.trace = nullptr; p.done = s.done; p.out_final = s.out_final;
      conv_layer_body<32, 2, 0, 1, SPLIT, kChainWV, 1, 1>(p, s.in_bytes, s.w_bytes);
    } else {
      chain_elementwise(s);
    }
    if (stamp && threadIdx.x == 0) stamp[1] = __builtin_amdgcn_s_memrealtime();
    if (i + 1 < a.n && !chain_barrier(a.bar, static_cast<unsigned>(i + 1), a.abort_host, flag_lds, stamp)) return;
  }
}

__global__ void __launch_bounds__(256) conv_reduce_kernel(const float4 *__restrict__ partial,
                                                         const float4 *__restrict__ residual,
                                                         const float *__restrict__ post_scale,
                                                         const float *__restrict__ post_shift,
                                                         const float *__restrict__ act_scale,
                                                         const float *__restrict__ act_shift,
                                                         float4 *__restrict__ out_act,
                                                         int ksplit, long long n4, int cout4,
                                                         float4 *__restrict__ out) {
  for (long long t = blockIdx.x * 256LL + threadIdx.x; t < n4; t += gridDim.x * 256LL) {
    float4 a = partial[t];
    for (int s = 1; s < ksplit; ++s) {
      const float4 b = partial[s * n4 + t];
      a.x += b.x; a.y += b.y; a.z += b.z; a.w += b.w;
    }
    if (residual) {
      const float4 r = residual[t];
      a.x += r.x; a.y += r.y; a.z += r.z; a.w += r.w;
    }
    if (post_scale) {
      const int c = static_cast<int>(t % cout4) * 4;
      a.x = fmaxf(fmaf(a.x, post_scale[c], post_shift[c]), 0.f);
      a.y = fmaxf(fmaf(a.y, post_scale[c + 1], post_shift[c + 1]), 0.f);
      a.z = fmaxf(fmaf(a.z, post_scale[c + 2], post_shift[c + 2]), 0.f);
      a.w = fmaxf(fmaf(a.w, post_scale[c + 3], post_shift[c + 3]), 0.f);
    }
    out[t] = a;
    if (out_act) {
      const int c = static_cast<int>(t % cout4) * 4;
      a.x = fmaxf(fmaf(a.x, act_scale[c], act_shift[c]), 0.f);
      a.y = fmaxf(fmaf(a.y, act_scale[c + 1], act_shift[c + 1]), 0.f);
      a.z = fmaxf(fmaf(a.z, act_scale[c + 2], act_shift[c + 2]), 0.f);
      a.w = fmaxf(fmaf(a.w, act_scale[c + 3], act_shift[c + 3]), 0.f);
      out_act[t] = a;
    }
  }
}

__global__ void __launch_bounds__(256) gather_conv_scalar_kernel(
    const float *__restrict__ in, const int32_t *__restrict__ nbr, int M_out, int K, int Cin,
    int Cout, const float *__restrict__ w_k8, const float *__restrict__ post_scale,
    const float *__restrict__ post_shift, const float *__restrict__ residual,
    const float *__restrict__ act_scale, const float *__restrict__ act_shift,
    float *__restrict__ out_act, float *__restrict__ out) {
  const int64_t total = static_cast<int64_t>(M_out) * Cout;
  const int c8 = (Cin + 7) / 8;
  for (int64_t t = blockIdx.x * 256LL + threadIdx.x; t < total; t += gridDim.x * 256LL) {
    const int j = static_cast<int>(t / Cout), co = static_cast<int>(t - static_cast<int64_t>(j) * Cout);
    float acc = 0.f;
    for (int k = 0; k < K; ++k) {
      const int s = nbr[static_cast<int64_t>(j) * K + k];
      if (s < 0) continue;
      const float *x = in + static_cast<int64_t>(s) * Cin;
      for (int ci = 0; ci < Cin; ++ci)
        acc = fmaf(x[ci], w_k8[((static_cast<int64_t>(k) * c8 + (ci >> 3)) * Cout + co) * 8 + (ci & 7)], acc);
    }
    if (residual) acc += residual[t];
    if (post_scale) acc = fmaxf(fmaf(acc, post_scale[co], post_shift[co]), 0.f);
    out[t] = acc;
    if (out_act) out_act[t] = fmaxf(fmaf(acc, act_scale[co], act_shift[co]), 0.f);
  }
}

__global__ void __launch_bounds__(256) pack_weight_kernel(const float *__restrict__ w, int cout, int K,
                                                         int cin, int src_kio,
                                                         float *__restrict__ out) {
  const int c8 = (cin + 7) / 8;
  const int64_t total = static_cast<int64_t>(K) * c8 * cout * 8;
  for (int64_t t = blockIdx.x * 256LL + threadIdx.x; t < total; t += gridDim.x * 256LL) {
    const int j = static_cast<int>(t & 7);
    int64_t r = t >> 3;
    const int co = static_cast<int>(r % cout);
    r /= cout;
    const int blk = static_cast<int>(r % c8), k = static_cast<int>(r / c8);
    const int ci = blk * 8 + j;
    float v = 0.f;
    if (ci < cin) {
      if (src_kio == 0) v = w[(static_cast<int64_t>(co) * K + k) * cin + ci];
      else if (src_kio == 1) v = w[(static_cast<int64_t>(k) * cin + ci) * cout + co];
      else v = w[(static_cast<int64_t>(ci) * K + (src_kio == 3 ? K - 1 - k : k)) * cout + co];
    }
    out[t] = v;
    uint16_t *planes = reinterpret_cast<uint16_t *>(out + total);
    const uint16_t h = bf16_rne(v);
    const float rest = v - bf16_f32(h);
    const uint16_t m = bf16_rne(rest);
    const uint16_t l = bf16_rne(rest - bf16_f32(m));
    planes[t] = h;
    planes[total + t] = m;
    planes[2 * total + t] = l;
  }
}

constexpr int kPackBatch = 64;
struct PackBatchArgs {
  const float *w[kPackBatch];
  float *out[kPackBatch];
  int cout[kPackBatch], K[kPackBatch], cin[kPackBatch], mode[kPackBatch];
  int block0[kPackBatch + 1];
  int n;
};
static_assert(sizeof(PackBatchArgs) <= 4096, "the batch travels as kernel arguments");
__global__ void __launch_bounds__(256) pack_weights_kernel(const PackBatchArgs a) {
  int j0 = 0, j1 = a.n;
  while (j1 - j0 > 1) {
    const int mid = (j0 + j1) >> 1;
    if (a.block0[mid] <= static_cast<int>(blockIdx.x)) j0 = mid; else j1 = mid;
  }
  const float *__restrict__ w = a.w[j0];
  float *__restrict__ out = a.out[j0];
  const int cout = a.cout[j0], K = a.K[j0], cin = a.cin[j0], src_kio = a.mode[j0];
  const int c8 = (cin + 7) / 8;
  const int64_t total = static_cast<int64_t>(K) * c8 * cout * 8;
  const int64_t stride = static_cast<int64_t>(a.block0[j0 + 1] - a.block0[j0]) * 256;
  for (int64_t t = (blockIdx.x - a.block0[j0]) * 256LL + threadIdx.x; t < total; t += stride) {
    const int j = static_cast<int>(t & 7);
    int64_t r = t >> 3;
    const int co = static_cast<int>(r % cout);
    r /= cout;
    const int blk = static_cast<int>(r % c8), k = static_cast<int>(r / c8);
    const int ci = blk * 8 + j;
    float v = 0.f;
    if (ci < cin) {
      if (src_kio == 0) v = w[(static_cast<int64_t>(co) * K + k) * cin + ci];
      else if (src_kio == 1) v = w[(static_cast<int64_t>(k) * cin + ci) * cout + co];
      else v = w[(static_cast<int64_t>(ci) * K + (src_kio == 3 ? K - 1 - k : k)) * cout + co];
    }
    out[t] = v;
    uint16_t *planes = reinterpret_cast<uint16_t *>(out + total);
    const uint16_t h = bf16_rne(v);
    const float rest = v - bf16_f32(h);
    const uint16_t m = bf16_rne(rest);
    const uint16_t l = bf16_rne(rest - bf16_f32(m));
    planes[t] = h;
    planes[total + t] = m;
    planes[2 * total + t] = l;
  }
}

int spconv_pack_weights(const PackJob *jobs, int n, sg_stream_t stream) {
  for (int at = 0; at < n; at += kPackBatch) {
    PackBatchArgs a;
    a.n = n - at < kPackBatch ? n - at : kPackBatch;
    a.block0[0] = 0;
// ... 153 lines not shown
    *static_cast<volatile unsigned *>(it->second) = 0u;
    set_error("%s: a grid barrier of an earlier multi-layer conv launch timed out (its workgroups were not "
              "co-resident: another process on this GPU?); that forward's results are invalid. "
              "SG_CONV_CHAIN=0 launches the layers one by one", who);
    return SG_ERR_LAUNCH;
  }
  return SG_OK;
}

static int chain_flush() {
  ChainRec &c = t_chain;
  if (c.args.n == 0) return SG_OK;
  int dev = 0;
  hipGetDevice(&dev);
  static int num_cu = 0;
  static std::once_flag once;
  std::call_once(once, [&] {
    hipDeviceGetAttribute(&num_cu, hipDeviceAttributeMultiprocessorCount, dev);
    if (num_cu <= 0) num_cu = 256;
  });
  c.args.bar = take_done(c.stream, kChainBarWords);
  if (c.args.bar == nullptr) {
    set_error("conv chain: no barrier block");
    return SG_ERR_LAUNCH;
  }
  const size_t lds = static_cast<size_t>(kChainWV) * 16 * 64 * sizeof(float) + 2 * kMetaInts * sizeof(int32_t) + 16 +
                     static_cast<size_t>(kChainWV) * 4096;
  static const int grid_env = getenv("SG_CHAIN_GRID") ? atoi(getenv("SG_CHAIN_GRID")) : 0;
  static const bool serial = !(getenv("SG_CHAIN_SERIAL") && atoi(getenv("SG_CHAIN_SERIAL")) == 0);
  int grid = num_cu >= 8 ? num_cu - num_cu % 8 : num_cu;
  if (grid_env >= 8 && grid_env < grid) grid = grid_env - grid_env % 8;
  const bool prof = g_conv_prof.enabled && c.conv_steps > 0;
  {
    std::lock_guard<std::mutex> lock(g_chain_mu);
    unsigned *&ab = g_chain_abort[dev];
    if (ab == nullptr) {
      if (hipHostMalloc(reinterpret_cast<void **>(&ab), 64, hipHostMallocMapped) != hipSuccess) {
        ab = nullptr;
        set_error("conv chain: pinned allocation failed");
        return SG_ERR_LAUNCH;
      }
      *ab = 0u;
    }
    c.args.abort_host = ab;
    hipEvent_t &mine = g_chain_events[{dev, c.stream}];
    if (mine == nullptr && hipEventCreateWithFlags(&mine, hipEventDisableTiming) != hipSuccess) {
      mine = nullptr;
      set_error("conv chain: event creation failed");
      return SG_ERR_LAUNCH;
    }
    hipEvent_t &last = g_chain_last[dev];
    if (serial && last != nullptr && last != mine) hipStreamWaitEvent(c.stream, last, 0);
    if (prof) {
      hipEventRecord(g_conv_prof.take(), c.stream);
      for (int v : {-c.conv_steps, 0, 0, 0, 0}) g_conv_prof.dims.push_back(v);
    }
    static const char *trace_env = getenv("SG_CHAIN_TRACE");
    c.args.trace = nullptr;
    const size_t trace_bytes = static_cast<size_t>(c.args.n) * grid * 4 * sizeof(unsigned long long);
    if (trace_env) {
      hipMalloc(&c.args.trace, trace_bytes);
      hipMemsetAsync(c.args.trace, 0, trace_bytes, c.stream);
    }
    if (c.b16)
      conv_chain_kernel<2><<<grid, 64 * kChainWV, lds, c.stream>>>(c.args);
    else
      conv_chain_kernel<1><<<grid, 64 * kChainWV, lds, c.stream>>>(c.args);
    if (prof) hipEventRecord(g_conv_prof.take(), c.stream);
    hipEventRecord(mine, c.stream);
    last = mine;
    if (trace_env && c.args.trace) {
      hipStreamSynchronize(c.stream);
      std::vector<unsigned long long> h(trace_bytes / 8);
      hipMemcpy(h.data(), c.args.trace, trace_bytes, hipMemcpyDeviceToHost);
      hipFree(c.args.trace);
      if (FILE *f = fopen(trace_env, "ab")) {
        long long hdr[4] = {c.args.n, grid, 0, 0};
        fwrite(hdr, 8, 4, f);
        for (int i = 0; i < c.args.n; ++i) {
          const ChainStep &st = c.args.s[i];
          long long d[8] = {st.kind, st.M_out, st.K, st.Cin, st.Cout, st.num_units, st.ksplit, st.col_units};
          fwrite(d, 8, 8, f);
        }
        fwrite(h.data(), 8, h.size(), f);
        fclose(f);
      }
    }
  }
  g_chain_launches.fetch_add(1, std::memory_order_relaxed);
  g_chain_steps.fetch_add(c.args.n, std::memory_order_relaxed);
  c.args.n = 0;
  c.conv_steps = 0;
  c.arith_set = false;
  return check_launch("conv chain");
}

static int chain_push(const ChainStep &st, bool b16, bool counts) {
  ChainRec &c = t_chain;
  const bool conv = st.kind == 0;
  if (c.args.n > 0 && (c.args.n == kChainMax || (conv && c.arith_set && c.b16 != b16))) {
    const int rc = chain_flush();
    if (rc != SG_OK) return rc;
  }
  if (conv) {
    c.b16 = b16;
    c.arith_set = true;
  }
  c.args.s[c.args.n++] = st;
  if (counts) ++c.conv_steps;
  return SG_OK;
}

void conv_chain_begin(hipStream_t stream) {
  ChainRec &c = t_chain;
  c.mode = chain_enabled() ? 2 : 1;
  c.stream = stream;
  c.args.n = 0;
  c.conv_steps = 0;
  c.arith_set = false;
}
bool conv_chain_recording() { return t_chain.mode == 2; }
int conv_chain_end() {
  const int rc = t_chain.mode == 2 ? chain_flush() : SG_OK;
  t_chain.mode = 0;
  t_chain.args.n = 0;
  return rc;
}
void conv_chain_abort() {
  t_chain.mode = 0;
  t_chain.args.n = 0;
  t_chain.conv_steps = 0;
}
int conv_chain_concat(const float *a, const float *b, int64_t rows, int ca, int cb, const float *scale,
                      const float *shift, float *out, float *out_act) {
  ChainStep st = {};
  st.kind = 1;
  st.in = a; st.residual = b; st.act_scale = scale; st.act_shift = shift; st.out = out; st.out_act = out_act;
  st.M_out = static_cast<int>(rows); st.Cin = ca; st.Cout = cb;
  return chain_push(st, t_chain.b16, false);
}
int conv_chain_bn_relu(const float *x, const float *scale, const float *shift, int64_t rows, int c, float *out) {
  ChainStep st = {};
  st.kind = 2;
  st.in = x; st.post_scale = scale; st.post_shift = shift; st.out = out;
  st.M_out = static_cast<int>(rows); st.Cin = c; st.Cout = 0;
  return chain_push(st, t_chain.b16, false);
}

typedef void (*PersistentFn)(ConvArgs, unsigned, unsigned);
struct SplitVariant {
  PersistentFn fn, fn_trace;
  PersistentFn fn_b16;
  PersistentFn fn_r16;
  int nbw, wv, ck, at;
  size_t lds;
  int occ, occ_b16, occ_r16;
};
#ifndef SG_B16_DEPTH
#define SG_B16_DEPTH 2
#endif
#ifndef SG_B16_WPE_PLUS
#define SG_B16_WPE_PLUS 0
#endif
template <int CK, int WPE, int NBW, int WV, int AT>
constexpr PersistentFn r16_variant() {
  if constexpr (AT) return gather_conv_persistent_kernel<CK, SG_B16_DEPTH, 0, WPE + SG_B16_WPE_PLUS, NBW, 2, WV, 1, 1>;
  else return nullptr;
}
#define SG_SPLIT_VARIANT(CK, DEPTH, WPE, NBW, WV, AT)                                            \
  {gather_conv_persistent_kernel<CK, DEPTH, 0, WPE, NBW, 1, WV, AT>,                              \
   gather_conv_persistent_kernel<CK, DEPTH, 1, WPE, NBW, 1, WV, AT>,                              \
   gather_conv_persistent_kernel<CK, SG_B16_DEPTH, 0, WPE + SG_B16_WPE_PLUS, NBW, 2, WV, AT>,     \
   r16_variant<CK, WPE, NBW, WV, AT>(), NBW, WV, CK, AT, 0, 0, 0, 0}
constexpr int kSplitVariants = 9;
static SplitVariant g_split_variants[kSplitVariants] = {
    SG_SPLIT_VARIANT(32, 2, 2, 2, 2, 1),  SG_SPLIT_VARIANT(32, 2, 3, 1, 2, 1),
    SG_SPLIT_VARIANT(32, 2, 2, 2, 4, 1),  SG_SPLIT_VARIANT(32, 2, 3, 1, 4, 1), SG_SPLIT_VARIANT(32, 2, 1, 1, 8, 1),
    SG_SPLIT_VARIANT(16, 2, 3, 2, 4, 0),  SG_SPLIT_VARIANT(16, 2, 4, 1, 4, 0), SG_SPLIT_VARIANT(16, 2, 2, 1, 8, 0),
    SG_SPLIT_VARIANT(16, 2, 1, 1, 16, 0),
};

static int launch_persistent_split(ConvArgs a, int num_tiles, long long in_bytes, long long w_bytes,
                                   hipStream_t stream, bool b16, bool in16) {
  static int num_cu = 0;
  static std::once_flag once;
  std::call_once(once, [] {
    int dev = 0;
    hipGetDevice(&dev);
    hipDeviceGetAttribute(&num_cu, hipDeviceAttributeMultiprocessorCount, dev);
    if (num_cu <= 0) num_cu = 256;
    auto prepare = [](SplitVariant &v) {
      v.lds = static_cast<size_t>(v.wv) * v.nbw * 16 * 64 * sizeof(float) + 2 * kMetaInts * sizeof(int32_t) + 16 +
              (v.at ? static_cast<size_t>(v.wv) * 4096 : 0);
      int o = 0;
      hipOccupancyMaxActiveBlocksPerMultiprocessor(&o, v.fn, 64 * v.wv, v.lds);
      v.occ = o < 1 ? 1 : o;
      o = 0;
      hipOccupancyMaxActiveBlocksPerMultiprocessor(&o, v.fn_b16, 64 * v.wv, v.lds);
      v.occ_b16 = o < 1 ? 1 : o;
      o = 0;
      if (v.fn_r16) hipOccupancyMaxActiveBlocksPerMultiprocessor(&o, v.fn_r16, 64 * v.wv, v.lds);
      v.occ_r16 = o < 1 ? 1 : o;
    };
    for (SplitVariant &v : g_split_variants) prepare(v);
  });
  static const int nbw_env = getenv("SG_CONV_NBW") ? atoi(getenv("SG_CONV_NBW")) : 2;
  static const int wv_env = getenv("SG_CONV_WV") ? atoi(getenv("SG_CONV_WV")) : 0;
  static const float min_rounds = getenv("SG_CONV_ROUNDS") ? atof(getenv("SG_CONV_ROUNDS")) : 2.5f;
  static const int at_env = getenv("SG_CONV_AT") ? atoi(getenv("SG_CONV_AT")) : 1;
  const int NB = (a.Cout + 31) / 32;
  const unsigned long long row_bytes = (in16 ? 2ull : 4ull) * a.Cin;
  const unsigned absent_at = static_cast<unsigned>((0xFFFFFFull * row_bytes) & 0xFFFFFFFFull);
  const int use_at = ((at_env != 0 || in16) && a.Cin % 32 == 0 && in_bytes / static_cast<long long>(row_bytes) < (1LL << 24) - 1 &&
                      static_cast<long long>(absent_at) >= in_bytes) ? 1 : 0;
  if (in16 && (!use_at || !b16)) {
    set_error("sg_unet_forward(bf16 rows): a layer with %d input channels / %lld input bytes cannot take the line-wise bf16 gather",
              a.Cin, in_bytes);
    return SG_ERR_ARG;
  }
  int pick = -1;
  static const int w2_max = getenv("SG_CONV_W2_MAX") ? atoi(getenv("SG_CONV_W2_MAX")) : 108;
  static const int w2_nbw = getenv("SG_CONV_W2_NBW") ? atoi(getenv("SG_CONV_W2_NBW")) : 2;
  static const float w2_rounds = getenv("SG_CONV_W2_ROUNDS") ? atof(getenv("SG_CONV_W2_ROUNDS")) : 1.5f;
  const bool use_w2 = wv_env == 2 || (wv_env == 0 && a.K * (a.Cin / 32) <= w2_max);
  for (int i = 0; i < kSplitVariants; ++i) {
    const SplitVariant &v = g_split_variants[i];
    if (v.at != use_at) continue;
    if (v.wv == 2 && (!use_w2 || a.ksplit > 1 || v.nbw > w2_nbw)) continue;
    if (a.ksplit > 1) {
      if (v.nbw == 1 && v.wv == 4) { pick = i; break; }
      continue;
    }
    pick = i;
    if (v.nbw == 2 && (a.Cout % 64 != 0 || nbw_env < 2)) continue;
    if (wv_env && v.wv != wv_env) continue;
    const long long units = static_cast<long long>(num_tiles) * (NB / v.nbw);
    if (wv_env || units >= static_cast<long long>((v.wv == 2 ? w2_rounds : min_rounds) * num_cu * (in16 ? v.occ_r16 : b16 ? v.occ_b16 : v.occ))) {
      pick = i;
      break;
    }
  }
  const bool chain_layer = t_chain.mode != 0 && use_at != 0;
  if (chain_layer) {
    for (int i = 0; i < kSplitVariants; ++i)
      if (g_split_variants[i].at == 1 && g_split_variants[i].nbw == 1 && g_split_variants[i].wv == kChainWV) pick = i;
  }
  const SplitVariant &v = g_split_variants[pick];
  a.col_units = NB / v.nbw;
  a.blocks_per_unit = v.nbw;
  const long long units = static_cast<long long>(num_tiles) * a.col_units * a.ksplit;
  a.num_units = static_cast<int>(units);
  auto magic = [](unsigned d) { return d <= 1 ? 0u : static_cast<unsigned>((1ULL << 32) / d) + 1u; };
  a.magic_upt = magic(static_cast<unsigned>(a.col_units * a.ksplit));
  a.magic_cu = magic(static_cast<unsigned>(a.col_units));
  a.magic_nsl = magic(static_cast<unsigned>(in16 ? (a.Cin + 63) / 64 : a.Cin / v.ck));
  if (t_chain.mode == 2) {
    if (chain_layer && !in16 && !a.out16 && !a.res16 && (a.ksplit == 1 || a.done != nullptr) && stream == t_chain.stream) {
      ChainStep st = {};
      st.kind = 0;
      st.in = a.in; st.w = a.w; st.post_scale = a.post_scale; st.post_shift = a.post_shift; st.residual = a.residual;
      st.act_scale = a.act_scale; st.act_shift = a.act_shift; st.out_act = a.out_act; st.order = a.order;
      st.tile_mask = a.tile_mask; st.nbr_tiles = a.nbr_tiles; st.out = a.out; st.done = a.done; st.out_final = a.out_final;
      st.M_out = a.M_out; st.K = a.K; st.Cin = a.Cin; st.Cout = a.Cout; st.col_units = a.col_units;
      st.ksplit = a.ksplit; st.k_per_split = a.k_per_split; st.num_units = a.num_units;
      st.magic_upt = a.magic_upt; st.magic_cu = a.magic_cu; st.magic_nsl = a.magic_nsl;
      st.in_bytes = static_cast<unsigned>(in_bytes); st.w_bytes = static_cast<unsigned>(w_bytes);
      return chain_push(st, b16, a.K > 1);
    }
    const int rc = chain_flush();
    if (rc != SG_OK) return rc;
  }
  static const bool dyn_env = getenv("SG_CONV_STATIC") && atoi(getenv("SG_CONV_STATIC")) == 0;
  static const int dyn_rounds_env = getenv("SG_CONV_DYN_ROUNDS") ? atoi(getenv("SG_CONV_DYN_ROUNDS")) : 2;
  a.queue = dyn_env ? take_tickets(stream) : nullptr;
  a.dyn_rounds = dyn_rounds_env == 1 ? 1 : 2;
  long long g = static_cast<long long>(num_cu) * (in16 ? v.occ_r16 : b16 ? v.occ_b16 : v.occ);
  if (g >= 8) g -= g % 8;
  if (units < g) g = units >= 8 ? (units + 7) / 8 * 8 : units;
  const unsigned ib = static_cast<unsigned>(in_bytes), wb = static_cast<unsigned>(w_bytes);
  if (in16) {
    v.fn_r16<<<static_cast<int>(g), 64 * v.wv, v.lds, stream>>>(a, ib, wb);
    return check_launch("sg_spconv_gather_conv(bf16 rows)");
  }
  if (b16) {
    v.fn_b16<<<static_cast<int>(g), 64 * v.wv, v.lds, stream>>>(a, ib, wb);
    return check_launch("sg_spconv_gather_conv_f32(bf16 operands)");
  }
  static const char *trace_env = getenv("SG_CONV_TRACE");
  if (trace_env) {
    const size_t nb = static_cast<size_t>(units) * kWavesPerWg * 8 * sizeof(unsigned long long);
    unsigned long long *dbuf = nullptr;
    hipMalloc(&dbuf, nb);
    hipMemsetAsync(dbuf, 0, nb, stream);
    a.trace = dbuf;
    v.fn_trace<<<static_cast<int>(g), 64 * v.wv, v.lds, stream>>>(a, ib, wb);
    hipStreamSynchronize(stream);
    std::vector<unsigned long long> h(nb / 8);
    hipMemcpy(h.data(), dbuf, nb, hipMemcpyDeviceToHost);
    hipFree(dbuf);
    if (FILE *f = fopen(trace_env, "ab")) {
      long long hdr[8] = {a.M_out, a.K, a.Cin, a.Cout, units, a.col_units, v.wv, g};
      fwrite(hdr, 8, 8, f);
      fwrite(h.data(), 8, h.size(), f);
      fclose(f);
    }
  } else {
    v.fn<<<static_cast<int>(g), 64 * v.wv, v.lds, stream>>>(a, ib, wb);
  }
  return check_launch("sg_spconv_gather_conv_f32(split)");
}


}

using namespace sg;

extern "C" {

int sg_spconv_set_arithmetic(int mode) {
  SG_REQUIRE(mode >= -1 && mode <= 2, "sg_spconv_set_arithmetic: mode must be -1, 0, 1 or 2");
  g_arith_override = mode;
  return SG_OK;
}

int sg_spconv_set_combine(int mode) {
  SG_REQUIRE(mode >= -1 && mode <= 1, "sg_spconv_set_combine: mode must be -1, 0 or 1");
  g_combine_override = mode;
  return SG_OK;
}

int sg_spconv_set_chain(int mode) {
  SG_REQUIRE(mode >= -1 && mode <= 1, "sg_spconv_set_chain: mode must be -1, 0 or 1");
  g_chain_override = mode;
  return SG_OK;
}

int sg_spconv_chain_stats(int64_t *launches, int64_t *steps) {
  if (launches) *launches = g_chain_launches.load(std::memory_order_relaxed);
  if (steps) *steps = g_chain_steps.load(std::memory_order_relaxed);
  return SG_OK;
}

int sg_spconv_profile(int enable) {
  g_conv_prof.enabled = enable != 0;
  if (enable) {
    g_conv_prof.used = 0;
    g_conv_prof.dims.clear();
  }
  return SG_OK;
}

int sg_spconv_profile_detail(float *ms, int32_t *dims, int cap, int *calls) {
  const int n = static_cast<int>(g_conv_prof.used / 2);
  if (calls) *calls = n;
  for (int i = 0; i < n && i < cap; ++i) {
    if (hipEventSynchronize(g_conv_prof.pool[2 * i + 1]) != hipSuccess) {
      set_error("sg_spconv_profile_detail: event synchronisation failed");
      return SG_ERR_LAUNCH;
    }
    float t = 0.f;
    hipEventElapsedTime(&t, g_conv_prof.pool[2 * i], g_conv_prof.pool[2 * i + 1]);
    if (ms) ms[i] = t;
    if (dims)
      for (int j = 0; j < 5; ++j) dims[5 * i + j] = g_conv_prof.dims[5 * static_cast<size_t>(i) + j];
  }
  return SG_OK;
}

int sg_spconv_profile_read(double *total_ms, int *launches) {
  double sum = 0.0;
  for (size_t i = 0; i + 1 < g_conv_prof.used; i += 2) {
    if (hipEventSynchronize(g_conv_prof.pool[i + 1]) != hipSuccess) {
      set_error("sg_spconv_profile_read: event synchronisation failed");
      return SG_ERR_LAUNCH;
    }
    float ms = 0.f;
    hipEventElapsedTime(&ms, g_conv_prof.pool[i], g_conv_prof.pool[i + 1]);
    sum += ms;
  }
  if (total_ms) *total_ms = sum;
  if (launches) *launches = static_cast<int>(g_conv_prof.used / 2);
  return SG_OK;
}

static size_t packed_k8_elems(int kvol, int cin, int cout) {
  return static_cast<size_t>(kvol) * ((cin + 7) / 8) * cout * 8;
}
size_t sg_spconv_packed_weight_elems(int kvol, int cin, int cout) {
  const size_t n = packed_k8_elems(kvol, cin, cout);
  return n + 3 * n / 2;
}

int sg_spconv_pack_weight(const float *w, int cout, int kvol, int cin, int src_is_kio, float *w_k8,
                          sg_stream_t stream) {
  SG_REQUIRE(cout > 0 && kvol > 0 && cin > 0 && src_is_kio >= 0 && src_is_kio <= 3,
             "sg_spconv_pack_weight: bad arguments");
  const int64_t total = static_cast<int64_t>(packed_k8_elems(kvol, cin, cout));
  pack_weight_kernel<<<grid_for(total, 256), 256, 0, as_stream(stream)>>>(w, cout, kvol, cin,
                                                                         src_is_kio, w_k8);
  return check_launch("sg_spconv_pack_weight");
}

size_t sg_spconv_conv_workspace_bytes(int M_out, int Cout) {
  const int num_tiles = (M_out + kTileRows - 1) / kTileRows;
  if (num_tiles * ((Cout + 31) / 32) >= 1024) return 256;
  return static_cast<size_t>(kMaxK) * M_out * Cout * sizeof(float) + 256;
}

static int gather_conv_impl(const float *in, int num_in_rows, const int32_t *nbr, int M_out,
                            int K, int Cin, int Cout, const float *w_k8, const float *post_scale,
                            const float *post_shift, const float *residual, const float *act_scale,
                            const float *act_shift, float *out_act, const int32_t *order,
                            const uint32_t *tile_mask, const int32_t *nbr_tiles, float *out,
                            void *ws, size_t ws_bytes, sg_stream_t stream_, int in16, int out16, int res16) {
  SG_REQUIRE(M_out >= 0 && K >= 1 && K <= kMaxK && Cin >= 1 && Cout >= 1,
             "sg_spconv_gather_conv_f32: bad arguments (M_out=%d K=%d Cin=%d Cout=%d)", M_out, K,
             Cin, Cout);
  SG_REQUIRE((post_scale == nullptr) == (post_shift == nullptr),
             "sg_spconv_gather_conv_f32: post_scale and post_shift must come together");
  SG_REQUIRE((out_act == nullptr) == (act_scale == nullptr) && (out_act == nullptr) == (act_shift == nullptr),
             "sg_spconv_gather_conv_f32: act_scale, act_shift and out_act must come together");
  if (M_out == 0) return SG_OK;
  hipStream_t stream = as_stream(stream_);
  struct ProfScope {
    hipStream_t st;
    bool on;
    ProfScope(hipStream_t s, bool count, int m, int k, int ci, int co, int rows_in)
        : st(s), on(g_conv_prof.enabled && count && t_chain.mode != 2) {
      if (on) {
        hipEventRecord(g_conv_prof.take(), st);
        for (int v : {m, k, ci, co, rows_in}) g_conv_prof.dims.push_back(v);
      }
    }
    ~ProfScope() {
      if (on) hipEventRecord(g_conv_prof.take(), st);
    }
  } prof_scope(stream, K > 1, M_out, K, Cin, Cout, num_in_rows);
  if (Cout % 4 != 0) {
    if (t_chain.mode == 2) {
      const int rc = chain_flush();
      if (rc != SG_OK) return rc;
    }
    gather_conv_scalar_kernel<<<grid_for(static_cast<int64_t>(M_out) * Cout, 256, 256 * 32), 256, 0,
                                stream>>>(in, nbr, M_out, K, Cin, Cout, w_k8, post_scale, post_shift,
                                          residual, act_scale, act_shift, out_act, out);
    return check_launch("sg_spconv_gather_conv_f32(scalar)");
  }
  const int NB = (Cout + 31) / 32;
  const int num_tiles = (M_out + kTileRows - 1) / kTileRows;
  const long long in_bytes_ll = static_cast<long long>(num_in_rows) * Cin * (in16 ? 2 : 4);
  const long long w_bytes_ll = static_cast<long long>(sg_spconv_packed_weight_elems(K, Cin, Cout)) * 4;
  const bool persistent = Cin % 16 == 0 && in_bytes_ll < (1LL << 31) && num_in_rows > 0 &&
                          static_cast<long long>(M_out) * Cout * 4 * kMaxK < (1LL << 32) &&
                          static_cast<long long>(num_tiles) * kTileRows * K * 4 < (1LL << 31) &&
                          order != nullptr && tile_mask != nullptr && nbr_tiles != nullptr &&
                          reinterpret_cast<uintptr_t>(nbr_tiles) % 16 == 0;
  static const int split_env = getenv("SG_CONV_SPLIT") ? atoi(getenv("SG_CONV_SPLIT")) : 1;
  static const int split_min_cin = getenv("SG_CONV_SPLIT_MIN_CIN") ? atoi(getenv("SG_CONV_SPLIT_MIN_CIN")) : 16;
  const int arith_ov = t_conv_arith >= 0 ? t_conv_arith : g_arith_override.load(std::memory_order_relaxed);
  const int split_on = arith_ov >= 0 ? arith_ov : split_env;
  const bool split = persistent && split_on != 0 && Cin >= split_min_cin;
  static const int target_env = getenv("SG_CONV_TARGET") ? atoi(getenv("SG_CONV_TARGET")) : 0;
  const int target = target_env > 0 ? target_env : split ? 1024 : 2048;
  const int waves_per_unit = persistent ? kWavesPerWg : 1;
  int bpu = 1;
  if (!persistent) {
    bpu = NB < 4 ? NB : 4;
    while (bpu > 1 && static_cast<long long>(num_tiles) * ((NB + bpu - 1) / bpu) < target) --bpu;
  }
  const int col_units = (NB + bpu - 1) / bpu;
  int ksplit = 1;
  const long long waves = static_cast<long long>(num_tiles) * col_units * waves_per_unit;
  if (waves < target / 2) {
    const long long want = (target / 2 + waves - 1) / waves;
    ksplit = static_cast<int>(want < K ? want : K);
    const size_t need = static_cast<size_t>(ksplit) * M_out * Cout * sizeof(float);
    if (ksplit > 1 && (ws == nullptr || ws_bytes < need)) ksplit = 1;
  }
  const int k_per_split = (K + ksplit - 1) / ksplit;
  ksplit = (K + k_per_split - 1) / k_per_split;

  ConvArgs a;
  a.in = in; a.nbr = nbr; a.w = w_k8; a.post_scale = post_scale; a.post_shift = post_shift;
  a.residual = residual; a.act_scale = act_scale; a.act_shift = act_shift; a.out_act = out_act;
  a.order = order; a.tile_mask = tile_mask; a.nbr_tiles = nbr_tiles;
  a.out = ksplit > 1 ? static_cast<float *>(ws) : out;
  a.M_out = M_out; a.K = K; a.Cin = Cin; a.Cout = Cout;
  a.col_units = col_units; a.blocks_per_unit = bpu; a.ksplit = ksplit; a.k_per_split = k_per_split;
  a.trace = nullptr;
  a.queue = nullptr;
  a.dyn_rounds = 2;
  a.out16 = out16;
  a.res16 = res16;
  static const int combine_env = getenv("SG_CONV_COMBINE") ? atoi(getenv("SG_CONV_COMBINE")) : 1;
  a.done = nullptr;
  a.out_final = out;
  const int combine_ov = g_combine_override.load(std::memory_order_relaxed);
  if ((combine_ov >= 0 ? combine_ov : combine_env) != 0 && persistent && ksplit > 1 &&
      static_cast<long long>(num_tiles) * col_units <= kDoneCounters)
    a.done = take_done(stream, static_cast<size_t>(num_tiles) * col_units);
  const long long units = static_cast<long long>(num_tiles) * col_units * ksplit;
  a.num_units = static_cast<int>(units);
  auto magic = [](unsigned d) { return d <= 1 ? 0u : static_cast<unsigned>((1ULL << 32) / d) + 1u; };
  a.magic_upt = magic(static_cast<unsigned>(col_units * ksplit));
  a.magic_cu = magic(static_cast<unsigned>(col_units));
  a.magic_nsl = 0;

  if (!split && t_chain.mode == 2) {
    const int rc = chain_flush();
    if (rc != SG_OK) return rc;
  }
  if (in16 || out16 || res16) {
    SG_REQUIRE(split && split_on == 2, "sg_unet_forward(bf16 rows): layer K=%d Cin=%d Cout=%d does not run on the bf16-operand "
               "persistent kernel", K, Cin, Cout);
    SG_REQUIRE(ksplit == 1 || a.done != nullptr, "sg_unet_forward(bf16 rows): an offset-split layer needs the in-launch combine");
  }
  if (split) {
    const int rc = launch_persistent_split(a, num_tiles, in_bytes_ll, w_bytes_ll, stream, split_on == 2, in16 != 0);
    if (rc != SG_OK) return rc;
    if (t_chain.mode == 2 && t_chain.args.n > 0) return SG_OK;
  } else if (persistent) {
    const size_t lds = static_cast<size_t>(kWavesPerWg) * 16 * 64 * sizeof(float) +
                       2 * kMetaInts * sizeof(int32_t) + 16;
    constexpr int kSliceCh = 16;
    static int num_cu = 0, occ = 0;
    static std::once_flag once;
    std::call_once(once, [&] {
      int dev = 0;
      hipGetDevice(&dev);
      hipDeviceGetAttribute(&num_cu, hipDeviceAttributeMultiprocessorCount, dev);
      if (num_cu <= 0) num_cu = 256;
      hipOccupancyMaxActiveBlocksPerMultiprocessor(&occ, gather_conv_persistent_kernel<kSliceCh, 2, 0, 5>, 256, lds);
      if (occ < 1) occ = 1;
    });
    a.magic_nsl = magic(static_cast<unsigned>(Cin / kSliceCh));
    static const bool dyn_env = getenv("SG_CONV_STATIC") && atoi(getenv("SG_CONV_STATIC")) == 0;
    a.queue = dyn_env ? take_tickets(stream) : nullptr;
    a.dyn_rounds = 2;
    long long g = static_cast<long long>(num_cu) * occ;
    if (g >= 8) g -= g % 8;
    if (units < g) g = units >= 8 ? (units + 7) / 8 * 8 : units;
    const unsigned ib_ = static_cast<unsigned>(in_bytes_ll), wb_ = static_cast<unsigned>(w_bytes_ll);
    static const char *trace_env = getenv("SG_CONV_TRACE");
    if (trace_env) {
      const size_t nb = static_cast<size_t>(units) * kWavesPerWg * 8 * sizeof(unsigned long long);
      unsigned long long *dbuf = nullptr;
      hipMalloc(&dbuf, nb);
      hipMemsetAsync(dbuf, 0, nb, stream);
      a.trace = dbuf;
      gather_conv_persistent_kernel<kSliceCh, 2, 1, 5><<<static_cast<int>(g), 256, lds, stream>>>(a, ib_, wb_);
      hipStreamSynchronize(stream);
      std::vector<unsigned long long> h(nb / 8);
      hipMemcpy(h.data(), dbuf, nb, hipMemcpyDeviceToHost);
      hipFree(dbuf);
      if (FILE *f = fopen(trace_env, "ab")) {
        long long hdr[8] = {M_out, K, Cin, Cout, units, col_units, ksplit, g};
        fwrite(hdr, 8, 8, f);
        fwrite(h.data(), 8, h.size(), f);
        fclose(f);
      }
    } else {
      gather_conv_persistent_kernel<kSliceCh, 2, 0, 5><<<static_cast<int>(g), 256, lds, stream>>>(a, ib_, wb_);
    }
  } else {
    const size_t lds = kWavesPerWg * kTileRows * kMaxK * sizeof(int32_t);
    const int grid = static_cast<int>((units + kWavesPerWg - 1) / kWavesPerWg);
    const bool vec = (Cin % kCk) == 0;
    switch (bpu) {
      case 1: launch_tile<1>(a, grid, lds, vec, stream); break;
      case 2: launch_tile<2>(a, grid, lds, vec, stream); break;
      case 3: launch_tile<3>(a, grid, lds, vec, stream); break;
      default: launch_tile<4>(a, grid, lds, vec, stream); break;
    }
  }
  if (ksplit > 1 && a.done == nullptr) {
    const long long n4 = static_cast<long long>(M_out) * Cout / 4;
    conv_reduce_kernel<<<grid_for(n4, 256), 256, 0, stream>>>(
        reinterpret_cast<const float4 *>(ws), reinterpret_cast<const float4 *>(residual), post_scale,
        post_shift, act_scale, act_shift, reinterpret_cast<float4 *>(out_act), ksplit, n4, Cout / 4,
        reinterpret_cast<float4 *>(out));
  }
  return check_launch("sg_spconv_gather_conv_f32");
}

int sg_spconv_gather_conv_f32(const float *in, int num_in_rows, const int32_t *nbr, int M_out,
                              int K, int Cin, int Cout, const float *w_k8, const float *post_scale,
                              const float *post_shift, const float *residual, const float *act_scale,
                              const float *act_shift, float *out_act, const int32_t *order,
                              const uint32_t *tile_mask, const int32_t *nbr_tiles, float *out,
                              void *ws, size_t ws_bytes, sg_stream_t stream_) {
  return gather_conv_impl(in, num_in_rows, nbr, M_out, K, Cin, Cout, w_k8, post_scale, post_shift, residual, act_scale,
                          act_shift, out_act, order, tile_mask, nbr_tiles, out, ws, ws_bytes, stream_, 0, 0, 0);
}

}

namespace sg {
int conv_gather_rows(const void *in, int num_in_rows, const int32_t *nbr, int M_out, int K, int Cin, int Cout,
                     const float *w_k8, const float *post_scale, const float *post_shift, const void *residual,
                     const float *act_scale, const float *act_shift, void *out_act, const int32_t *order,
                     const uint32_t *tile_mask, const int32_t *nbr_tiles, void *out, void *ws, size_t ws_bytes,
                     sg_stream_t stream, int in16, int out16, int res16) {
  return gather_conv_impl(static_cast<const float *>(in), num_in_rows, nbr, M_out, K, Cin, Cout, w_k8, post_scale, post_shift,
                          static_cast<const float *>(residual), act_scale, act_shift, static_cast<float *>(out_act), order,
                          tile_mask, nbr_tiles, static_cast<float *>(out), ws, ws_bytes, stream, in16, out16, res16);
}
}
```

### softgroup_amd/csrc/unet_exec.hip

```cpp
#include <map>
#include <mutex>
#include <utility>
#include <vector>

#include <stdlib.h>

#include "common.h"
#include "radix_sort.h"
#include "unet_common.h"

namespace sg {

__global__ void __launch_bounds__(256) batch_max_kernel(const int32_t *__restrict__ indices, int M,
                                                       int32_t *__restrict__ bmax) {
  int m = 0;
  for (int i = blockIdx.x * 256 + threadIdx.x; i < M; i += gridDim.x * 256) m = max(m, indices[4 * i]);
#pragma unroll
  for (int o = 32; o > 0; o >>= 1) m = max(m, __shfl_xor(m, o, 64));
  if ((threadIdx.x & 63) == 0 && m > 0) atomicMax(bmax, m);
}
__device__ __forceinline__ uint64_t spread3(uint32_t v) {
  uint64_t x = v & 0x1fffffu;
  x = (x | (x << 32)) & 0x1f00000000ffffull;
  x = (x | (x << 16)) & 0x1f0000ff0000ffull;
  x = (x | (x << 8)) & 0x100f00f00f00f00full;
  x = (x | (x << 4)) & 0x10c30c30c30c30c3ull;
  x = (x | (x << 2)) & 0x1249249249249249ull;
  return x;
}
__global__ void __launch_bounds__(256) morton_key_kernel(const int32_t *__restrict__ indices, int M,
                                                        int dim_bits, const int32_t *__restrict__ bmax,
                                                        uint32_t *__restrict__ key, int32_t *__restrict__ val) {
  const int i = blockIdx.x * 256 + threadIdx.x;
  if (i >= M) return;
  const int4 c = reinterpret_cast<const int4 *>(indices)[i];
  const int bb = 32 - __clz(*bmax);
  const uint64_t code = (static_cast<uint64_t>(static_cast<uint32_t>(c.x)) << (3 * dim_bits)) |
                        (spread3(c.y) << 2) | (spread3(c.z) << 1) | spread3(c.w);
  const int total = bb + 3 * dim_bits;
  key[i] = static_cast<uint32_t>(total > 24 ? code >> (total - 24) : code);
  val[i] = i;
}
__global__ void __launch_bounds__(256) permute_indices_kernel(const int32_t *__restrict__ indices,
                                                             const int32_t *__restrict__ perm, int M,
                                                             int32_t *__restrict__ out) {
  const int i = blockIdx.x * 256 + threadIdx.x;
  if (i < M) reinterpret_cast<int4 *>(out)[i] = reinterpret_cast<const int4 *>(indices)[perm[i]];
}
template <bool SCATTER>
__global__ void __launch_bounds__(256) permute_rows_kernel(const float4 *__restrict__ in,
                                                          const int32_t *__restrict__ perm, int64_t rows,
                                                          int c4, float4 *__restrict__ out) {
  const int64_t total = rows * c4;
  for (int64_t t = blockIdx.x * 256LL + threadIdx.x; t < total; t += gridDim.x * 256LL) {
    const int64_t r = t / c4;
    const int c = static_cast<int>(t - r * c4);
    const int64_t o = perm[r];
    if (SCATTER) out[o * c4 + c] = in[t];
    else out[t] = in[o * c4 + c];
  }
}

__global__ void __launch_bounds__(256) concat2_kernel(const float4 *__restrict__ a,
                                                     const float4 *__restrict__ b, int64_t rows,
                                                     int ca4, int cb4,
                                                     const float4 *__restrict__ scale,
                                                     const float4 *__restrict__ shift,
                                                     float4 *__restrict__ out,
                                                     float4 *__restrict__ out_act) {
  const int c4 = ca4 + cb4;
  const int64_t total = rows * c4;
  for (int64_t t = blockIdx.x * 256LL + threadIdx.x; t < total; t += gridDim.x * 256LL) {
    const int64_t r = t / c4;
    const int c = static_cast<int>(t - r * c4);
    const float4 v = c < ca4 ? a[r * ca4 + c] : b[r * cb4 + (c - ca4)];
    out[t] = v;
    if (out_act) {
      const float4 s = scale[c], h = shift[c];
      out_act[t] = make_float4(fmaxf(fmaf(v.x, s.x, h.x), 0.f), fmaxf(fmaf(v.y, s.y, h.y), 0.f),
                               fmaxf(fmaf(v.z, s.z, h.z), 0.f), fmaxf(fmaf(v.w, s.w, h.w), 0.f));
    }
  }
}

__device__ __forceinline__ float bf16_to_f32(uint32_t h) { return __builtin_bit_cast(float, h << 16); }
__device__ __forceinline__ uint32_t f32_to_bf16(float x) {
  const uint32_t u = __builtin_bit_cast(uint32_t, x);
  return (u + 0x7fffu + ((u >> 16) & 1u)) >> 16;
}
__global__ void __launch_bounds__(256) concat2_bf16_kernel(const uint2 *__restrict__ a, const uint2 *__restrict__ b,
                                                          int64_t rows, int ca4, int cb4,
                                                          const float4 *__restrict__ scale,
                                                          const float4 *__restrict__ shift, uint2 *__restrict__ out,
                                                          uint2 *__restrict__ out_act) {
  const int c4 = ca4 + cb4;
  const int64_t total = rows * c4;
  for (int64_t t = blockIdx.x * 256LL + threadIdx.x; t < total; t += gridDim.x * 256LL) {
    const int64_t r = t / c4;
    const int c = static_cast<int>(t - r * c4);
    const uint2 v = c < ca4 ? a[r * ca4 + c] : b[r * cb4 + (c - ca4)];
    out[t] = v;
    if (out_act) {
      const float4 s = scale[c], h = shift[c];
      const float x0 = fmaxf(fmaf(bf16_to_f32(v.x & 0xffffu), s.x, h.x), 0.f), x1 = fmaxf(fmaf(bf16_to_f32(v.x >> 16), s.y, h.y), 0.f);
      const float x2 = fmaxf(fmaf(bf16_to_f32(v.y & 0xffffu), s.z, h.z), 0.f), x3 = fmaxf(fmaf(bf16_to_f32(v.y >> 16), s.w, h.w), 0.f);
      out_act[t] = make_uint2(f32_to_bf16(x0) | (f32_to_bf16(x1) << 16), f32_to_bf16(x2) | (f32_to_bf16(x3) << 16));
    }
  }
}

struct IdentSegs {
  int32_t *order[SG_PYRAMID_MAX_LEVELS];
  uint32_t *mask[SG_PYRAMID_MAX_LEVELS];
  int rows[SG_PYRAMID_MAX_LEVELS];
  int n;
};
__global__ void __launch_bounds__(256) ident_plan_kernel(IdentSegs s) {
  const int l = blockIdx.y;
  const int rows = s.rows[l], tiles = (rows + 31) / 32, padded = tiles * 32;
  for (int i = blockIdx.x * 256 + threadIdx.x; i < padded; i += gridDim.x * 256) s.order[l][i] = i < rows ? i : -1;
  for (int i = blockIdx.x * 256 + threadIdx.x; i < tiles + SG_PLAN_HIST_WORDS; i += gridDim.x * 256)
    s.mask[l][i] = i < tiles ? 1u : (i == tiles + 1 ? static_cast<uint32_t>(tiles) : 0u);
}

static bool index_stream_on() {
  static const bool on = getenv("SG_UNET_INDEX_STREAM") && atoi(getenv("SG_UNET_INDEX_STREAM")) != 0;
  return on;
}
struct StreamState {
  std::mutex mu;
  int32_t *host_rows = nullptr;
  int32_t *dev_rows = nullptr;
  hipStream_t istream = nullptr;
  hipEvent_t ev_start = nullptr, ev_index = nullptr;
  bool ready = false;
};
static std::mutex table_mu;
static std::map<std::pair<int, hipStream_t>, StreamState *> table;

void unet_release_stream(int dev, hipStream_t stream) {
  StreamState *st = nullptr;
  {
    std::lock_guard<std::mutex> g(table_mu);
    auto it = table.find(std::make_pair(dev, stream));
    if (it == table.end()) return;
    st = it->second;
    table.erase(it);
  }
  {
    std::lock_guard<std::mutex> g(st->mu);
    if (st->ready) {
      if (st->istream != nullptr) {
// ... 4 lines not shown
      hipEventDestroy(st->ev_index);
      hipHostFree(st->host_rows);
      hipFree(st->dev_rows);
    }
  }
  delete st;
}

int unet_build_index(const char *who, int L, const int32_t *indices, int num_rows,
                     const int32_t *spatial_shape_host, void *arena, size_t arena_bytes, sg_stream_t stream,
                     LevelIdx *li, size_t *used, std::unique_lock<std::mutex> *lock) {
  int dev = 0;
  SG_REQUIRE(hipGetDevice(&dev) == hipSuccess && dev >= 0, "%s: no current device", who);
  StreamState *stp = nullptr;
  {
    std::lock_guard<std::mutex> g(table_mu);
    StreamState *&slot = table[std::make_pair(dev, as_stream(stream))];
    if (slot == nullptr) slot = new StreamState();
    stp = slot;
  }
  StreamState &st = *stp;
  std::unique_lock<std::mutex> guard(st.mu);
  if (!st.ready) {
    SG_REQUIRE(hipHostMalloc(reinterpret_cast<void **>(&st.host_rows), SG_PYRAMID_MAX_LEVELS * 4) == hipSuccess,
               "%s: pinned allocation failed", who);
    SG_REQUIRE(hipMalloc(reinterpret_cast<void **>(&st.dev_rows), SG_PYRAMID_MAX_LEVELS * 4) == hipSuccess,
               "%s: device allocation failed", who);
    SG_REQUIRE(!index_stream_on() || hipStreamCreateWithFlags(&st.istream, hipStreamNonBlocking) == hipSuccess,
               "%s: stream creation failed", who);
    SG_REQUIRE(hipEventCreateWithFlags(&st.ev_start, hipEventDisableTiming) == hipSuccess &&
                   hipEventCreateWithFlags(&st.ev_index, hipEventDisableTiming) == hipSuccess,
               "%s: event creation failed", who);
    st.ready = true;
  }
  const bool own_istream = index_stream_on();
  hipStream_t istream = own_istream ? st.istream : as_stream(stream);
  sg_stream_t is = reinterpret_cast<sg_stream_t>(istream);
  if (own_istream && (hipEventRecord(st.ev_start, as_stream(stream)) != hipSuccess ||
                      hipStreamWaitEvent(istream, st.ev_start, 0) != hipSuccess)) {
    set_error("%s: event record/wait failed", who);
    return SG_ERR_LAUNCH;
  }
  Arena ix(arena, arena_bytes);
#define SG_IALLOC(var, T, count)                                                       \
  T *var = ix.take<T>(count);                                                          \
  if (var == nullptr) {                                                                \
    set_error("%s: arena too small (%zu bytes) for the index tables", who, arena_bytes); \
    return SG_ERR_WORKSPACE;                                                           \
  }
  const size_t pws_bytes = sg_spconv_pyramid_workspace_bytes(num_rows, L);
  SG_IALLOC(pws, char, pws_bytes);
  SG_TRY(sg_spconv_pyramid_rows(indices, num_rows, spatial_shape_host, L, st.dev_rows, pws, pws_bytes, is));
  if (hipMemcpyAsync(st.host_rows, st.dev_rows, sizeof(int32_t) * L, hipMemcpyDeviceToHost, istream) != hipSuccess ||
      hipStreamSynchronize(istream) != hipSuccess) {
    set_error("%s: reading the level row counts failed", who);
    return SG_ERR_LAUNCH;
  }
  SG_REQUIRE(st.host_rows[0] == num_rows, "%s: duplicate voxel coordinates in the input "
             "(%d distinct of %d rows)", who, st.host_rows[0], num_rows);
  sg_pyramid_level pl[SG_PYRAMID_MAX_LEVELS];
  for (int l = 0; l < L; ++l) {
    const int rows = st.host_rows[l];
    const int rows2 = l + 1 < L ? st.host_rows[l + 1] : 0;
    const size_t r = static_cast<size_t>(rows ? rows : 1), r2 = static_cast<size_t>(rows2 ? rows2 : 1);
    const size_t t = (r + 31) / 32, t2 = (r2 + 31) / 32;
    sg_pyramid_level &P = pl[l];
    P = sg_pyramid_level();
    P.rows = rows;
    SG_IALLOC(indices_l, int32_t, r * 4);
    SG_IALLOC(nbr, int32_t, r * 27);
    SG_IALLOC(so, int32_t, t * 32);
    SG_IALLOC(sm, uint32_t, t + SG_PLAN_HIST_WORDS);
    SG_IALLOC(sn, int32_t, t * 32 * 27);
    P.indices = indices_l; P.nbr = nbr;
    P.subm = sg_plan_ptrs{so, sm, sn};
    LevelIdx &I = li[l];
    I.rows = rows;
    for (int a = 0; a < 3; ++a) I.shape[a] = spatial_shape_host[a] >> l;
    I.subm.nbr = nbr; I.subm.order = so; I.subm.tile_mask = sm; I.subm.nbr_tiles = sn;
    I.subm.rows = rows; I.subm.kvol = 27;
    if (l + 1 < L) {
      SG_IALLOC(in2out, int32_t, r);
      SG_IALLOC(child, int32_t, r2 * 8);
      SG_IALLOC(inv, int32_t, r * 8);
      SG_IALLOC(dord, int32_t, t2 * 32);
      SG_IALLOC(dm, uint32_t, t2 + SG_PLAN_HIST_WORDS);
      SG_IALLOC(dn, int32_t, t2 * 32 * 8);
      SG_IALLOC(uo, int32_t, t * 32);
      SG_IALLOC(um, uint32_t, t + SG_PLAN_HIST_WORDS);
      SG_IALLOC(un, int32_t, t * 32 * 8);
      P.in2out = in2out; P.child = child; P.inv = inv;
      P.down = sg_plan_ptrs{dord, dm, dn};
      P.up = sg_plan_ptrs{uo, um, un};
      I.down.nbr = child; I.down.order = dord; I.down.tile_mask = dm; I.down.nbr_tiles = dn;
      I.down.rows = rows2; I.down.kvol = 8;
      I.up.nbr = inv; I.up.order = uo; I.up.tile_mask = um; I.up.nbr_tiles = un;
      I.up.rows = rows; I.up.kvol = 8;
    }
  }
  {
    const size_t nb = sg_spconv_pyramid_build_workspace_bytes(pl, L);
    SG_IALLOC(ws2, char, nb);
    SG_TRY(sg_spconv_pyramid_build(indices, num_rows, spatial_shape_host, L, pl, pws, pws_bytes, ws2, nb, is));
  }
  if (L > 1) {
    IdentSegs segs;
    segs.n = L - 1;
    for (int l = 0; l + 1 < L; ++l) {
      const size_t tiles = (static_cast<size_t>(li[l].rows) + 31) / 32;
      SG_IALLOC(ord, int32_t, tiles ? tiles * 32 : 32);
      SG_IALLOC(tm, uint32_t, tiles + SG_PLAN_HIST_WORDS);
      segs.order[l] = ord;
      segs.mask[l] = tm;
      segs.rows[l] = li[l].rows;
      Plan &P = li[l].ident;
      P.nbr = ord; P.order = ord; P.nbr_tiles = ord; P.tile_mask = tm;
      P.rows = li[l].rows; P.kvol = 1;
    }
    ident_plan_kernel<<<dim3(grid_for(num_rows, 256), L - 1), 256, 0, istream>>>(segs);
  }
#undef SG_IALLOC
  if (own_istream && (hipEventRecord(st.ev_index, istream) != hipSuccess ||
                      hipStreamWaitEvent(as_stream(stream), st.ev_index, 0) != hipSuccess)) {
    set_error("%s: event record/wait failed", who);
    return SG_ERR_LAUNCH;
  }
  *used = ix.off;
  *lock = std::move(guard);
  return SG_OK;
}

__global__ void __launch_bounds__(256) pad_channels_kernel(const float *__restrict__ in, int64_t rows, int cin,
                                                          int cpad, const int32_t *__restrict__ perm,
                                                          float *__restrict__ out) {
  const int64_t total = rows * cpad;
  for (int64_t t = blockIdx.x * 256LL + threadIdx.x; t < total; t += gridDim.x * 256LL) {
    const int64_t r = t / cpad;
    const int c = static_cast<int>(t - r * cpad);
    const int64_t src = perm ? perm[r] : r;
    out[t] = c < cin ? in[src * cin + c] : 0.f;
  }
}

#define SG_ALLOC(var, T, count)                                                        \
  T *var = ar.take<T>(count);                                                          \
  if (var == nullptr) {                                                                \
    set_error("sg_unet_forward: arena too small (%zu bytes, need more than %zu)", ar.cap, ar.off); \
    return SG_ERR_WORKSPACE;                                                           \
  }

thread_local void (*t_unet_conv_hook)(void *) = nullptr;
thread_local void *t_unet_conv_ctx = nullptr;

struct Exec {
  const sg_unet_desc *d;
  Arena ar;
  sg_stream_t stream;
  const LevelIdx *idx;
  const int32_t *perm = nullptr;

  Exec(const sg_unet_desc *desc, void *arena, size_t bytes, sg_stream_t s, const LevelIdx *li)
      : d(desc), ar(arena, bytes), stream(s), idx(li) {}

  bool r16 = false;
  size_t fsz(size_t n) const { return r16 ? (n + 1) / 2 : n; }
  bool chain_open = false;
  bool chain_from(int l) const {
    static const int max_rows = getenv("SG_CONV_CHAIN_ROWS") ? atoi(getenv("SG_CONV_CHAIN_ROWS")) : 6144;
    if (r16 || chain_open || idx[l].rows > max_rows || idx[l].rows <= 0) return false;
    for (int k = l; k < d->n_levels; ++k)
      if (d->levels[k].planes % 32 != 0) return false;
    return true;
  }
  struct ChainScope {
    Exec &e;
    bool on;
    ChainScope(Exec &ex, bool open) : e(ex), on(open) {
      if (on) {
        conv_chain_begin(as_stream(e.stream));
        e.chain_open = true;
      }
    }
    int close() {
      if (!on) return SG_OK;
      on = false;
      e.chain_open = false;
      return conv_chain_end();
    }
    ~ChainScope() {
      if (on) {
        conv_chain_abort();
        e.chain_open = false;
      }
    }
  };

  struct Act {
    const float *scale = nullptr, *shift = nullptr;
    float *out = nullptr;
  };

  int conv(const float *in, int in_rows, const Plan &p, int cin, int cout, const float *w,
           const float *post_s, const float *post_b, const float *residual, const Act &act, float *out,
           bool in_f32 = false, bool out_f32 = false) {
    if (p.rows == 0) return SG_OK;
    const size_t m = ar.mark();
    const size_t nb = sg_spconv_conv_workspace_bytes(p.rows, cout);
    void *ws = nullptr;
    if (nb > 256) {
      ws = ar.take<char>(nb);
    }
    const int rc = !r16 ? sg_spconv_gather_conv_f32(in, in_rows, p.nbr, p.rows, p.kvol, cin, cout, w, post_s,
                                                    post_b, residual, act.scale, act.shift, act.out, p.order,
                                                    p.tile_mask, p.nbr_tiles, out, ws, ws ? nb : 0, stream)
                        : conv_gather_rows(in, in_rows, p.nbr, p.rows, p.kvol, cin, cout, w, post_s, post_b, residual,
                                           act.scale, act.shift, act.out, p.order, p.tile_mask, p.nbr_tiles, out, ws,
                                           ws ? nb : 0, stream, in_f32 ? 0 : 1, out_f32 ? 0 : 1, 1);
    ar.release(m);
    return rc;
  }

  int block(const sg_unet_block &b, const float *x, const float *xa, int rows, const Plan &subm,
            const Plan &ident, const float *post_s, const float *post_b, const Act &next, float *out,
            bool out_f32 = false) {
    const size_t m = ar.mark();
    const float *shortcut = x;
    if (b.w_i != nullptr) {
      SG_ALLOC(sc, float, fsz(static_cast<size_t>(rows) * b.cout));
      SG_TRY(conv(x, rows, ident, b.cin, b.cout, b.w_i, nullptr, nullptr, nullptr, Act(), sc));
      shortcut = sc;
    }
    SG_ALLOC(h, float, fsz(static_cast<size_t>(rows) * b.cout));
    SG_TRY(conv(xa, rows, subm, b.cin, b.cout, b.w1, b.bn2_scale, b.bn2_shift, nullptr, Act(), h));
    SG_TRY(conv(h, rows, subm, b.cout, b.cout, b.w2, post_s, post_b, shortcut, next, out, false, out_f32));
    ar.release(m);
    return SG_OK;
  }

  int level(int l, const float *x, const float *xa, const float *pre_in, int pre_cin,
            const float *post_s, const float *post_b, float *out) {
    const sg_unet_level &L = d->levels[l];
    const int c = L.planes;
    const bool deeper = l + 1 < d->n_levels;
    const size_t m0 = ar.mark();
    const LevelIdx &I = idx[l];
    const int rows = I.rows;
    const Plan &subm = I.subm, &ident = I.ident;
    const size_t feat = fsz(static_cast<size_t>(rows ? rows : 1) * c);
    if (pre_in != nullptr) {
      SG_ALLOC(x0, float, feat);
      SG_ALLOC(x0a, float, feat);
      const Act a0{L.blocks[0].bn1_scale, L.blocks[0].bn1_shift, x0a};
      const int cpk = d->input_cin_packed > pre_cin ? d->input_cin_packed : pre_cin;
      if ((cpk != pre_cin || perm != nullptr) && rows) {
        SG_ALLOC(xp, float, static_cast<size_t>(rows) * cpk);
        pad_channels_kernel<<<grid_for(static_cast<int64_t>(rows) * cpk, 256), 256, 0, as_stream(stream)>>>(
            pre_in, rows, pre_cin, cpk, perm, xp);
        pre_in = xp;
      }
      SG_TRY(conv(pre_in, rows, subm, cpk, c, d->input_w, nullptr, nullptr, nullptr, a0, x0, true, false));
      x = x0;
      xa = x0a;
    } else if (xa == nullptr) {
      SG_ALLOC(x0a, float, feat);
      if (conv_chain_recording())
        SG_TRY(conv_chain_bn_relu(x, L.blocks[0].bn1_scale, L.blocks[0].bn1_shift, rows, c, x0a));
      else
        SG_TRY(sg_bn_relu_f32(x, L.blocks[0].bn1_scale, L.blocks[0].bn1_shift, rows, c, 1, x0a, stream));
      xa = x0a;
    }
    const float *cur = x, *cur_a = xa;
    for (int i = 0; i < L.n_blocks; ++i) {
      const bool last = i == L.n_blocks - 1;
      float *dst = out;
      Act next;
      if (!(last && !deeper)) {
        SG_ALLOC(t, float, feat);
        SG_ALLOC(ta, float, feat);
        dst = t;
        next.out = ta;
        next.scale = last ? L.down_bn_scale : L.blocks[i + 1].bn1_scale;
        next.shift = last ? L.down_bn_shift : L.blocks[i + 1].bn1_shift;
      }
      const bool fin = last && !deeper;
      SG_TRY(block(L.blocks[i], cur, cur_a, rows, subm, ident, fin ? post_s : nullptr,
                   fin ? post_b : nullptr, next, dst, fin && l == 0));
      cur = dst;
      cur_a = next.out;
    }
    if (deeper) {
      const int c2 = d->levels[l + 1].planes;
      const int rows2 = idx[l + 1].rows;
      const Plan &down = I.down, &up = I.up;
      const sg_unet_level &L2 = d->levels[l + 1];
      const size_t feat2 = fsz(static_cast<size_t>(rows2 ? rows2 : 1) * c2);
      SG_ALLOC(y, float, feat2);
      SG_ALLOC(ya, float, feat2);
      const Act ay{L2.blocks[0].bn1_scale, L2.blocks[0].bn1_shift, ya};
      SG_ALLOC(z, float, feat2);
      {
        ChainScope chain(*this, chain_from(l + 1));
        SG_TRY(conv(cur_a, rows, down, c, c2, L.down_w, nullptr, nullptr, nullptr, ay, y));
        SG_TRY(level(l + 1, y, ya, nullptr, 0, L.up_bn_scale, L.up_bn_shift, z));
        SG_TRY(chain.close());
      }
      SG_ALLOC(cat, float, 2 * feat);
      SG_ALLOC(cata, float, 2 * feat);
      {
        const size_t m = ar.mark();
        SG_ALLOC(upf, float, feat);
        SG_TRY(conv(z, rows2, up, c2, c, L.up_w, nullptr, nullptr, nullptr, Act(), upf));
        if (rows && r16)
          concat2_bf16_kernel<<<grid_for(static_cast<int64_t>(rows) * (2 * c / 4), 256), 256, 0, as_stream(stream)>>>(
              reinterpret_cast<const uint2 *>(cur), reinterpret_cast<const uint2 *>(upf), rows, c / 4, c / 4,
              reinterpret_cast<const float4 *>(L.tail[0].bn1_scale), reinterpret_cast<const float4 *>(L.tail[0].bn1_shift),
              reinterpret_cast<uint2 *>(cat), reinterpret_cast<uint2 *>(cata));
        else if (rows && conv_chain_recording())
          SG_TRY(conv_chain_concat(cur, upf, rows, c, c, L.tail[0].bn1_scale, L.tail[0].bn1_shift, cat, cata));
        else if (rows)
          concat2_kernel<<<grid_for(static_cast<int64_t>(rows) * (2 * c / 4), 256), 256, 0, as_stream(stream)>>>(
              reinterpret_cast<const float4 *>(cur), reinterpret_cast<const float4 *>(upf), rows, c / 4,
              c / 4, reinterpret_cast<const float4 *>(L.tail[0].bn1_scale),
              reinterpret_cast<const float4 *>(L.tail[0].bn1_shift), reinterpret_cast<float4 *>(cat),
              reinterpret_cast<float4 *>(cata));
        ar.release(m);
      }
      cur = cat;
      cur_a = cata;
      for (int i = 0; i < L.n_blocks; ++i) {
        const bool last = i == L.n_blocks - 1;
        float *dst = out;
        Act next;
        if (!last) {
          SG_ALLOC(t, float, feat);
          SG_ALLOC(ta, float, feat);
          dst = t;
          next = Act{L.tail[i + 1].bn1_scale, L.tail[i + 1].bn1_shift, ta};
        }
        SG_TRY(block(L.tail[i], cur, cur_a, rows, subm, ident, last ? post_s : nullptr,
                     last ? post_b : nullptr, next, dst, last && l == 0));
        cur = dst;
        cur_a = next.out;
      }
    }
    ar.release(m0);
    return check_launch("sg_unet_forward");
  }
};

static size_t level_index_bytes(size_t rows, size_t rows_next, bool deeper) {
  const size_t t = (rows + 31) / 32, t2 = (rows_next + 31) / 32;
  size_t b = align_up(rows * 4 * 4) + align_up(rows * 27 * 4) +
             align_up(t * 32 * 4) + align_up((t + SG_PLAN_HIST_WORDS) * 4) + align_up(t * 32 * 27 * 4);
  if (deeper)
    b += align_up(rows * 4) + align_up(rows_next * 8 * 4) + align_up(rows * 8 * 4) +
         align_up(t2 * 32 * 4) + align_up((t2 + SG_PLAN_HIST_WORDS) * 4) + align_up(t2 * 32 * 8 * 4) +
         align_up(t * 32 * 4) + align_up((t + SG_PLAN_HIST_WORDS) * 4) + align_up(t * 32 * 8 * 4);
  return b + 4096;
}
size_t unet_index_bytes(int L, int num_rows) {
  const size_t rows = static_cast<size_t>(num_rows > 0 ? num_rows : 1);
  size_t total = (1 << 20) + sg_spconv_pyramid_workspace_bytes(num_rows, L) +
                 (L + 1) * (align_up(rows * 4) + align_up(rows / 8 + 256) + 4096);
  sg_pyramid_level bound[SG_PYRAMID_MAX_LEVELS];
  for (int l = 0; l < L && l < SG_PYRAMID_MAX_LEVELS; ++l) {
    total += level_index_bytes(rows, rows, l + 1 < L);
    bound[l].rows = num_rows;
  }
  total += sg_spconv_pyramid_build_workspace_bytes(bound, L < SG_PYRAMID_MAX_LEVELS ? L : SG_PYRAMID_MAX_LEVELS);
  return align_up(total, 4096);
}

}

using namespace sg;

extern "C" {

size_t sg_unet_arena_bytes(const sg_unet_desc *d, int num_rows) {
  size_t total = unet_index_bytes(d->n_levels, num_rows) + (1 << 20);
  const size_t rows = static_cast<size_t>(num_rows > 0 ? num_rows : 1);
  total += 2 * align_up(rows * 4) + radix_sort_workspace_bytes(static_cast<int64_t>(rows)) + align_up(rows * 16) +
           2 * align_up(rows * static_cast<size_t>(d->levels[0].planes) * 4) + 4096;
  for (int l = 0; l < d->n_levels; ++l)
    total += rows * 12 * 2 * static_cast<size_t>(d->levels[l].planes) * 4 + (64 << 10);
  return total;
}

int sg_unet_forward(const sg_unet_desc *d, const float *feats, const int32_t *indices, int num_rows,
                    const int32_t *spatial_shape_host, float *out, void *arena, size_t arena_bytes,
                    sg_stream_t stream) {
  SG_REQUIRE(d != nullptr && d->n_levels >= 1 && d->levels != nullptr, "sg_unet_forward: bad descriptor");
  SG_REQUIRE(d->n_levels <= SG_PYRAMID_MAX_LEVELS, "sg_unet_forward: at most %d levels", SG_PYRAMID_MAX_LEVELS);
  SG_REQUIRE(num_rows >= 0, "sg_unet_forward: bad num_rows");
  for (int l = 0; l < d->n_levels; ++l)
    SG_REQUIRE(d->levels[l].planes % 4 == 0 && d->levels[l].n_blocks >= 1,
               "sg_unet_forward: level %d: planes must be a multiple of 4", l);
  SG_REQUIRE(d->arithmetic == 0 || d->arithmetic == 2 || d->arithmetic == 3, "sg_unet_forward: arithmetic must be 0, 2 or 3");
  if (num_rows == 0) return SG_OK;
  SG_TRY(conv_chain_check_abort("sg_unet_forward"));
  const int L = d->n_levels;
  struct ArithScope {
    int keep;
    explicit ArithScope(int a) : keep(t_conv_arith) { if (a > 0) t_conv_arith = a; }
    ~ArithScope() { t_conv_arith = keep; }
  } arith_scope(d->arithmetic == 3 ? 2 : d->arithmetic);
  bool rows16 = d->arithmetic == 3 && d->input_w != nullptr;
  for (int l = 0; l < d->n_levels; ++l) rows16 = rows16 && d->levels[l].planes % 32 == 0;
  static const int morton_env = getenv("SG_UNET_MORTON") ? atoi(getenv("SG_UNET_MORTON")) : 0;
  static const int morton_min = getenv("SG_UNET_MORTON_MIN") ? atoi(getenv("SG_UNET_MORTON_MIN")) : 16384;
  const bool pre = d->input_w != nullptr;
  const int c0 = d->levels[0].planes;
  const bool morton = morton_env != 0 && num_rows >= morton_min;
  Arena head(arena, arena_bytes);
  const int32_t *perm = nullptr;
  const int32_t *idx_in = indices;
  const float *feats_in = feats;
  float *out_int = out;
  if (morton) {
    hipStream_t st = as_stream(stream);
    const size_t M = static_cast<size_t>(num_rows);
    uint32_t *key = head.take<uint32_t>(M);
    int32_t *val = head.take<int32_t>(M);
    const size_t rs_bytes = radix_sort_workspace_bytes(static_cast<int64_t>(M));
    void *rs_ws = head.take<char>(rs_bytes);
    int32_t *idx_p = head.take<int32_t>(M * 4);
    int32_t *bmax = head.take<int32_t>(64);
    float *out_p = head.take<float>(M * c0);
    float *feats_p = pre ? out_p : head.take<float>(M * c0);
    if (feats_p == nullptr || out_p == nullptr) {
      set_error("sg_unet_forward: arena too small (%zu bytes) for the internal row order", arena_bytes);
      return SG_ERR_WORKSPACE;
    }
    int dim_bits = 1;
    for (int a = 0; a < 3; ++a)
      while ((1 << dim_bits) < spatial_shape_host[a]) ++dim_bits;
    SG_REQUIRE(dim_bits <= 20, "sg_unet_forward: spatial extent above 2^20");
    hipMemsetAsync(bmax, 0, 4, st);
    batch_max_kernel<<<grid_for(num_rows, 256, 256), 256, 0, st>>>(indices, num_rows, bmax);
    morton_key_kernel<<<(num_rows + 255) / 256, 256, 0, st>>>(indices, num_rows, dim_bits, bmax, key, val);
    uint32_t *ks;
    int32_t *vs;
    SG_TRY(radix_sort_pairs(key, val, static_cast<int64_t>(M), 24, rs_ws, rs_bytes, st, &ks, &vs));
    permute_indices_kernel<<<(num_rows + 255) / 256, 256, 0, st>>>(indices, vs, num_rows, idx_p);
    perm = vs;
    idx_in = idx_p;
    out_int = out_p;
    if (!pre) {
      permute_rows_kernel<false><<<grid_for(static_cast<int64_t>(M) * (c0 / 4), 256), 256, 0, st>>>(
          reinterpret_cast<const float4 *>(feats), vs, num_rows, c0 / 4, reinterpret_cast<float4 *>(feats_p));
      feats_in = feats_p;
    }
    SG_TRY(check_launch("sg_unet_forward(row order)"));
  }
  const size_t head_bytes = align_up(head.off, 4096);
  char *rest = static_cast<char *>(arena) + head_bytes;
  const size_t rest_bytes = arena_bytes > head_bytes ? arena_bytes - head_bytes : 0;
  LevelIdx li[SG_PYRAMID_MAX_LEVELS];
  std::unique_lock<std::mutex> guard;
  size_t index_bytes = 0;
  SG_TRY(unet_build_index("sg_unet_forward", L, idx_in, num_rows, spatial_shape_host, rest, rest_bytes, stream,
                          li, &index_bytes, &guard));
  const size_t used = align_up(index_bytes, 4096);
  if (rest_bytes <= used) {
    set_error("sg_unet_forward: arena too small (%zu bytes)", arena_bytes);
    return SG_ERR_WORKSPACE;
  }
  if (t_unet_conv_hook != nullptr) {
    void (*hook)(void *) = t_unet_conv_hook;
    t_unet_conv_hook = nullptr;
    hook(t_unet_conv_ctx);
  }
  Exec ex(d, rest + used, rest_bytes - used, stream, li);
  ex.perm = pre ? perm : nullptr;
  ex.r16 = rows16;
  int rc;
  {
    Exec::ChainScope chain(ex, !pre && ex.chain_from(0));
    rc = ex.level(0, pre ? nullptr : feats_in, nullptr, pre ? feats : nullptr, d->input_cin,
                  d->out_bn_scale, d->out_bn_shift, out_int);
    if (rc == SG_OK) rc = chain.close();
  }
  if (rc == SG_OK && morton) {
    permute_rows_kernel<true><<<grid_for(static_cast<int64_t>(num_rows) * (c0 / 4), 256), 256, 0, as_stream(stream)>>>(
        reinterpret_cast<const float4 *>(out_int), perm, num_rows, c0 / 4, reinterpret_cast<float4 *>(out));
    rc = check_launch("sg_unet_forward(row order)");
  }
  return rc;
}

}
```

Before: 434.1.

## Read UNet skip concat from two sources inside the conv instead of materialising it

Adds a two-source gather convolution that reads the first cin_a channels from one buffer and the rest from a second, plus a second fused activation output. The UNet decoder uses it to feed the tail block directly from the skip features and the up-conv output, whose BN-ReLU activations are written by the producing convs. This removes the concat kernel and the two double-width cat buffers with their memory traffic. In exchange it adds template variants and per-slice source selection in the gather loop, and it is disabled for bf16 rows, chain recording, or when the SG_UNET_CONCAT env var is set.

```diff
diff --git a/include/softgroup_hip.h b/include/softgroup_hip.h
--- a/include/softgroup_hip.h
+++ b/include/softgroup_hip.h
@@ -171,6 +171,15 @@
                               const float *act_shift, float *out_act, const int32_t *order,
                               const uint32_t *tile_mask, const int32_t *nbr_tiles, float *out,
                               void *ws, size_t ws_bytes, sg_stream_t stream);
+
+int sg_spconv_gather_conv2_f32(const float *in, const float *in2, int cin_a, int num_in_rows,
+                               const int32_t *nbr, int num_out_rows, int kvol, int cin, int cout,
+                               const float *w_k8, const float *post_scale, const float *post_shift,
+                               const float *residual, const float *act_scale, const float *act_shift,
+                               float *out_act, const float *act2_scale, const float *act2_shift,
+                               float *out_act2, const int32_t *order, const uint32_t *tile_mask,
+                               const int32_t *nbr_tiles, float *out, void *ws, size_t ws_bytes,
+                               sg_stream_t stream);
 
 int sg_spconv_set_arithmetic(int mode);
 
@@ -238,6 +247,7 @@
 int sg_unet_forward(const sg_unet_desc *desc, const float *feats, const int32_t *indices,
                     int num_rows, const int32_t *spatial_shape_host, float *out, void *arena,
                     size_t arena_bytes, sg_stream_t stream);
+int sg_unet_concat_stats(int64_t *in_place, int64_t *passes);
 
 typedef struct sg_train_bn {
   const float *weight, *bias;
diff --git a/softgroup_amd/_lib.py b/softgroup_amd/_lib.py
--- a/softgroup_amd/_lib.py
+++ b/softgroup_amd/_lib.py
@@ -72,6 +72,7 @@
     'sg_spconv_profile_read': (_i, [_vp, _vp]),
     'sg_spconv_profile_detail': (_i, [_vp, _vp, _i, _vp]),
     'sg_unet_arena_bytes': (_sz, [_vp, _i]),
+    'sg_unet_concat_stats': (_i, [_vp, _vp]),
     'sg_unet_forward': (_i, [_vp, _vp, _vp, _i, _vp, _vp, _vp, _sz, _vp]),
     'sg_unet_train_arena_hint': (_sz, [_vp, _i]),
     'sg_unet_train_forward': (_i, [_vp, _vp, _vp, _i, _vp, _vp, _vp, _sz, _vp, _vp, _vp]),
@@ -83,6 +84,8 @@
     'sg_spconv_conv_workspace_bytes': (_sz, [_i, _i]),
     'sg_spconv_gather_conv_f32': (_i, [_vp, _i, _vp, _i, _i, _i, _i, _vp, _vp, _vp, _vp, _vp, _vp,
                                        _vp, _vp, _vp, _vp, _vp, _vp, _sz, _vp]),
+    'sg_spconv_gather_conv2_f32': (_i, [_vp, _vp, _i, _i, _vp, _i, _i, _i, _i, _vp, _vp, _vp, _vp, _vp, _vp,
+                                        _vp, _vp, _vp, _vp, _vp, _vp, _vp, _vp, _vp, _sz, _vp]),
     'sg_spconv_packed_weight_elems_bf16': (_sz, [_i, _i, _i]),
     'sg_spconv_pack_weight_bf16': (_i, [_vp, _i, _i, _i, _i, _vp, _vp]),
     'sg_spconv_conv_bf16_workspace_bytes': (_sz, [_i, _i]),
diff --git a/softgroup_amd/csrc/common.h b/softgroup_amd/csrc/common.h
--- a/softgroup_amd/csrc/common.h
+++ b/softgroup_amd/csrc/common.h
@@ -185,6 +185,7 @@
                      const float *act_scale, const float *act_shift, void *out_act, const int32_t *order,
                      const uint32_t *tile_mask, const int32_t *nbr_tiles, void *out, void *ws, size_t ws_bytes,
                      sg_stream_t stream, int in16, int out16, int res16);
+bool conv_two_source_ok(int rows, int c);
 int spconv_wgrad_layout(const void *in, int in_bf16, const void *g_out, int g_bf16, const int32_t *nbr_t, int M_out,
                         int K, int Cin, int Cout, float *dw, int out_oki, void *ws, size_t ws_bytes,
                         sg_stream_t stream);
diff --git a/softgroup_amd/csrc/spconv_conv.hip b/softgroup_amd/csrc/spconv_conv.hip
--- a/softgroup_amd/csrc/spconv_conv.hip
+++ b/softgroup_amd/csrc/spconv_conv.hip
@@ -100,6 +100,12 @@
   unsigned long long *trace;
   unsigned *done;
   float *out_final;
+  const float *in2;
+  unsigned in2_bytes;
+  int cin_a;
+  const float *act2_scale;
+  const float *act2_shift;
+  float *out_act2;
 };
 
 template <int NBW, bool VEC>
@@ -249,9 +255,10 @@
 constexpr int kRowsAt = kTileRows * kMaxK, kMaskAt = kRowsAt + kTileRows;
 constexpr int kMetaInts = kMaskAt + 4;
 
-template <int CK, int DEPTH, int TRACE, int NBW, int SPLIT, int WV, int AT, int CHAIN, int R16 = 0>
+template <int CK, int DEPTH, int TRACE, int NBW, int SPLIT, int WV, int AT, int CHAIN, int R16 = 0, int TWO = 0>
 __device__ __forceinline__ void conv_layer_body(const ConvArgs &p, unsigned in_bytes, unsigned w_bytes) {
   static_assert(!R16 || (SPLIT == 2 && AT), "bf16 rows: bf16-operand arithmetic, line-wise gather");
+  static_assert(!TWO || (!R16 && !CHAIN), "two row sources: fp32 rows, single launches");
   constexpr int AUX = CHAIN ? 16 : 0;
   static_assert(!SPLIT || CK == 16 || AT, "split-precision path: 16-channel slices");
   static_assert(!AT || (SPLIT && CK == 32), "line-wise gather: split path, 32-channel items");
@@ -288,6 +295,10 @@
       __builtin_amdgcn_make_buffer_rsrc(const_cast<float *>(p.in), 0, in_bytes, 0x00020000);
   const __amdgpu_buffer_rsrc_t rs_w =
       __builtin_amdgcn_make_buffer_rsrc(const_cast<float *>(p.w), 0, w_bytes, 0x00020000);
+  constexpr bool ACT2 = (TWO & 2) != 0;
+  const int cin_a = TWO && p.in2 != nullptr ? p.cin_a : p.Cin;
+  const bool act2 = ACT2 && p.out_act2 != nullptr && final_out;
+  const bool c_act2 = ACT2 && p.out_act2 != nullptr && p.done != nullptr && !final_out;
   const __amdgpu_buffer_rsrc_t rs_res = __builtin_amdgcn_make_buffer_rsrc(
       const_cast<float *>(add_res ? p.residual : p.in), 0, add_res ? res_bytes : 0u, 0x00020000);
   const __amdgpu_buffer_rsrc_t rs_out = __builtin_amdgcn_make_buffer_rsrc(
@@ -301,6 +312,10 @@
       combine ? p.out_final : p.out, 0, combine ? fin_bytes : 0u, 0x00020000);
   const __amdgpu_buffer_rsrc_t rs_cact = __builtin_amdgcn_make_buffer_rsrc(
       c_act ? p.out_act : p.out, 0, c_act ? fin_bytes : 0u, 0x00020000);
+  const __amdgpu_buffer_rsrc_t rs_act2 = __builtin_amdgcn_make_buffer_rsrc(
+      act2 ? p.out_act2 : p.out, 0, act2 ? fin_bytes : 0u, 0x00020000);
+  const __amdgpu_buffer_rsrc_t rs_cact2 = __builtin_amdgcn_make_buffer_rsrc(
+      c_act2 ? p.out_act2 : p.out, 0, c_act2 ? fin_bytes : 0u, 0x00020000);
   auto ld_row = [&](const __amdgpu_buffer_rsrc_t &rs, unsigned off, int n, bool h16) -> float {
     if constexpr (SPLIT == 2) {
       if (h16)
@@ -376,7 +391,19 @@
   float resv[NBW][RR];
 
   f4 *tr_lds = reinterpret_cast<f4 *>(ctl + 4) + wave * 256;
-  const unsigned row_pitch = static_cast<unsigned>(p.Cin) * 4u, lane_chunk = static_cast<unsigned>(lane & 7) * 16u;
+  const unsigned row_pitch = static_cast<unsigned>(cin_a) * 4u, lane_chunk = static_cast<unsigned>(lane & 7) * 16u;
+  struct Src { __amdgpu_buffer_rsrc_t rs; int cin, s_a; };
+  auto source = [&](int s) {
+    Src r = {rs_in, cin_a, s * (CK * 4)};
+    if constexpr (TWO) {
+      if (__builtin_amdgcn_readfirstlane(s * CK >= cin_a)) {
+        r.rs = __builtin_amdgcn_make_buffer_rsrc(const_cast<float *>(p.in2), 0, p.in2_bytes, 0x00020000);
+        r.cin = p.Cin - cin_a;
+        r.s_a = (s * CK - cin_a) * 4;
+      }
+    }
+    return r;
+  };
   auto load = [&](const Ctx &c, int k, int s, Slice &S) {
     if constexpr (R16) {
 #pragma unroll
@@ -397,12 +424,18 @@
       return;
     }
     if constexpr (AT) {
+      [[maybe_unused]] const Src from = source(s);
 #pragma unroll
       for (int q = 0; q < 4; ++q) {
         unsigned src = static_cast<unsigned>(c.meta[(8 * q + (lane >> 3)) * p.K + k]);
         if (SG_WHATIF & 16) src = static_cast<unsigned>(c.pair * 32 + 8 * q + (lane >> 3)) % static_cast<unsigned>(p.M_out);
-        const unsigned v_a = __umul24(src, row_pitch) + lane_chunk;
-        S.a[q] = __builtin_bit_cast(f4, __builtin_amdgcn_raw_buffer_load_b128(rs_in, v_a, s * 128, AUX));
+        if constexpr (TWO) {
+          const unsigned v_a = __umul24(src, static_cast<unsigned>(from.cin) * 4u) + lane_chunk;
+          S.a[q] = __builtin_bit_cast(f4, __builtin_amdgcn_raw_buffer_load_b128(from.rs, v_a, from.s_a, AUX));
+        } else {
+          const unsigned v_a = __umul24(src, row_pitch) + lane_chunk;
+          S.a[q] = __builtin_bit_cast(f4, __builtin_amdgcn_raw_buffer_load_b128(rs_in, v_a, s * 128, AUX));
+        }
       }
       const int s_w = planes_at + (k * c8 + s * 4) * p.Cout * 16;
 #pragma unroll
@@ -419,11 +452,19 @@
       return;
     }
     const int src = c.meta[nbr_base + k];
-    const unsigned v_a = src >= 0 ? static_cast<unsigned>(src * p.Cin + ahalf * HC) * 4u : kOob;
-    const int s_a = s * (CK * 4);
-#pragma unroll
-    for (int q = 0; q < NQ; ++q)
-      S.a[q] = __builtin_bit_cast(f4, __builtin_amdgcn_raw_buffer_load_b128(rs_in, v_a + q * 16, s_a, AUX));
+    if constexpr (TWO) {
+      const Src from = source(s);
+      const unsigned v_a = src >= 0 ? static_cast<unsigned>(src * from.cin + ahalf * HC) * 4u : kOob;
+#pragma unroll
+      for (int q = 0; q < NQ; ++q)
+        S.a[q] = __builtin_bit_cast(f4, __builtin_amdgcn_raw_buffer_load_b128(from.rs, v_a + q * 16, from.s_a, AUX));
+    } else {
+      const unsigned v_a = src >= 0 ? static_cast<unsigned>(src * p.Cin + ahalf * HC) * 4u : kOob;
+      const int s_a = s * (CK * 4);
+#pragma unroll
+      for (int q = 0; q < NQ; ++q)
+        S.a[q] = __builtin_bit_cast(f4, __builtin_amdgcn_raw_buffer_load_b128(rs_in, v_a + q * 16, s_a, AUX));
+    }
     if constexpr (SPLIT) {
       const int s_w = planes_at + (k * c8 + s * 2) * p.Cout * 16;
 #pragma unroll
@@ -709,6 +750,18 @@
     }
     if constexpr (TRACE) { asm volatile("" : "+v"(acc[0][0])); }
     mark(1);
+    [[maybe_unused]] float as2[NBW], ab2[NBW];
+    if constexpr (ACT2) {
+      const int colc = min(c.col, p.Cout - 1);
+#pragma unroll
+      for (int n = 0; n < NBW; ++n) {
+        as2[n] = ab2[n] = 0.f;
+        if (act2) {
+          as2[n] = p.act2_scale[colc + 32 * n];
+          ab2[n] = p.act2_shift[colc + 32 * n];
+        }
+      }
+    }
 
     if (wave == 0) {
       asm volatile("s_waitcnt vmcnt(0)" ::: "memory");
@@ -730,6 +783,7 @@
     const Unit dn = decode(has_next ? un : u);
 
     float v[NBW][RR], va[NBW][RR];
+    [[maybe_unused]] float va2[NBW][RR];
     unsigned o_off[RR];
     {
       float part[NBW][RR][WV];
@@ -752,6 +806,7 @@
           if (post) t = fmaxf(fmaf(t, c.ps[n], c.pb[n]), 0.f);
           v[n][rr] = t;
           va[n][rr] = fmaxf(fmaf(t, c.as[n], c.ab[n]), 0.f);
+          if constexpr (ACT2) va2[n][rr] = fmaxf(fmaf(t, as2[n], ab2[n]), 0.f);
         }
         o_off[rr] = c.o_off[rr];
       }
@@ -779,6 +834,14 @@
       for (int rr = 0; rr < RR; ++rr)
 #pragma unroll
         for (int n = 0; n < NBW; ++n) st_row(va[n][rr], rs_act, o_off[rr], 0u, n, out16);
+    }
+    if constexpr (ACT2) {
+      if (act2) {
+#pragma unroll
+        for (int rr = 0; rr < RR; ++rr)
+#pragma unroll
+          for (int n = 0; n < NBW; ++n) st_row(va2[n][rr], rs_act2, o_off[rr], 0u, n, out16);
+      }
     }
     if (combine) {
       asm volatile("s_waitcnt vmcnt(0)" ::: "memory");
@@ -792,11 +855,16 @@
       if (__builtin_amdgcn_readfirstlane(ctl[3]) != 0) {
         const int colc = min(col_done, p.Cout - 1);
         float ps[NBW], pb[NBW], as[NBW], ab[NBW];
+        [[maybe_unused]] float as2[NBW], ab2[NBW];
 #pragma unroll
         for (int n = 0; n < NBW; ++n) {
           ps[n] = pb[n] = as[n] = ab[n] = 0.f;
           if (p.post_scale) { ps[n] = p.post_scale[colc + 32 * n]; pb[n] = p.post_shift[colc + 32 * n]; }
           if (c_act) { as[n] = p.act_scale[colc + 32 * n]; ab[n] = p.act_shift[colc + 32 * n]; }
+          if constexpr (ACT2) {
+            as2[n] = ab2[n] = 0.f;
+            if (c_act2) { as2[n] = p.act2_scale[colc + 32 * n]; ab2[n] = p.act2_shift[colc + 32 * n]; }
+          }
         }
         auto part = [&](int ks, int rr, int n) {
           return __builtin_bit_cast(float, __builtin_amdgcn_raw_buffer_load_b32(
@@ -848,6 +916,7 @@
             if (p.post_scale) x = fmaxf(fmaf(x, ps[n], pb[n]), 0.f);
             st_row(x, rs_cout, o_off[rr], 0u, n, out16);
             st_row(fmaxf(fmaf(x, as[n], ab[n]), 0.f), rs_cact, o_off[rr], 0u, n, out16);
+            if constexpr (ACT2) st_row(fmaxf(fmaf(x, as2[n], ab2[n]), 0.f), rs_cact2, o_off[rr], 0u, n, out16);
           }
       }
     }
@@ -870,10 +939,11 @@
   }
 }
 
-template <int CK, int DEPTH, int TRACE, int WPE, int NBW = 1, int SPLIT = 0, int WV = 4, int AT = 0, int R16 = 0>
+template <int CK, int DEPTH, int TRACE, int WPE, int NBW = 1, int SPLIT = 0, int WV = 4, int AT = 0, int R16 = 0,
+          int TWO = 0>
 __global__ void __launch_bounds__(64 * WV, WPE) gather_conv_persistent_kernel(ConvArgs p, unsigned in_bytes,
                                                                              unsigned w_bytes) {
-  conv_layer_body<CK, DEPTH, TRACE, NBW, SPLIT, WV, AT, 0, R16>(p, in_bytes, w_bytes);
+  conv_layer_body<CK, DEPTH, TRACE, NBW, SPLIT, WV, AT, 0, R16, TWO>(p, in_bytes, w_bytes);
 }
 
 struct ChainStep {
@@ -992,6 +1062,7 @@
       p.num_units = s.num_units;
       p.magic_upt = s.magic_upt; p.magic_cu = s.magic_cu; p.magic_nsl = s.magic_nsl;
       p.queue = nullptr; p.dyn_rounds = 2; p.out16 = 0; p.res16 = 0; p.trace = nullptr; p.done = s.done; p.out_final = s.out_final;
+      p.in2 = nullptr; p.in2_bytes = 0; p.cin_a = s.Cin; p.act2_scale = nullptr; p.act2_shift = nullptr; p.out_act2 = nullptr;
       conv_layer_body<32, 2, 0, 1, SPLIT, kChainWV, 1, 1>(p, s.in_bytes, s.w_bytes);
     } else {
       chain_elementwise(s);
@@ -1451,9 +1522,11 @@
   PersistentFn fn, fn_trace;
   PersistentFn fn_b16;
   PersistentFn fn_r16;
+  PersistentFn fn_two, fn_two_b16;
   int nbw, wv, ck, at;
   size_t lds;
   int occ, occ_b16, occ_r16;
+  int occ_two, occ_two_b16;
 };
 #ifndef SG_B16_DEPTH
 #define SG_B16_DEPTH 2
@@ -1466,11 +1539,19 @@
   if constexpr (AT) return gather_conv_persistent_kernel<CK, SG_B16_DEPTH, 0, WPE + SG_B16_WPE_PLUS, NBW, 2, WV, 1, 1>;
   else return nullptr;
 }
+template <int CK, int WPE, int NBW, int WV, int AT>
+constexpr PersistentFn two_b16_variant() {
+  if constexpr (AT) return gather_conv_persistent_kernel<CK, SG_B16_DEPTH, 0, WPE + SG_B16_WPE_PLUS, NBW, 2, WV, 1, 0, 3>;
+  else return nullptr;
+}
 #define SG_SPLIT_VARIANT(CK, DEPTH, WPE, NBW, WV, AT)                                            \
   {gather_conv_persistent_kernel<CK, DEPTH, 0, WPE, NBW, 1, WV, AT>,                              \
    gather_conv_persistent_kernel<CK, DEPTH, 1, WPE, NBW, 1, WV, AT>,                              \
    gather_conv_persistent_kernel<CK, SG_B16_DEPTH, 0, WPE + SG_B16_WPE_PLUS, NBW, 2, WV, AT>,     \
-   r16_variant<CK, WPE, NBW, WV, AT>(), NBW, WV, CK, AT, 0, 0, 0, 0}
+   r16_variant<CK, WPE, NBW, WV, AT>(),                                                           \
+   gather_conv_persistent_kernel<CK, DEPTH, 0, WPE, NBW, 1, WV, AT, 0, 3>,                        \
+   two_b16_variant<CK, WPE, NBW, WV, AT>(),                                                       \
+   NBW, WV, CK, AT, 0, 0, 0, 0, 0, 0}
 constexpr int kSplitVariants = 9;
 static SplitVariant g_split_variants[kSplitVariants] = {
     SG_SPLIT_VARIANT(32, 2, 2, 2, 2, 1),  SG_SPLIT_VARIANT(32, 2, 3, 1, 2, 1),
@@ -1479,8 +1560,16 @@
     SG_SPLIT_VARIANT(16, 2, 1, 1, 16, 0),
 };
 
+static bool line_wise_fits(int Cin, long long in_bytes, bool in16) {
+  const unsigned long long row_bytes = (in16 ? 2ull : 4ull) * Cin;
+  const unsigned absent_at = static_cast<unsigned>((0xFFFFFFull * row_bytes) & 0xFFFFFFFFull);
+  return Cin % 32 == 0 && in_bytes / static_cast<long long>(row_bytes) < (1LL << 24) - 1 &&
+         static_cast<long long>(absent_at) >= in_bytes;
+}
+
 static int launch_persistent_split(ConvArgs a, int num_tiles, long long in_bytes, long long w_bytes,
-                                   hipStream_t stream, bool b16, bool in16) {
+                                   hipStream_t stream, bool b16, bool in16, bool two = false,
+                                   long long in_a_bytes = 0) {
   static int num_cu = 0;
   static std::once_flag once;
   std::call_once(once, [] {
@@ -1500,6 +1589,12 @@
       o = 0;
       if (v.fn_r16) hipOccupancyMaxActiveBlocksPerMultiprocessor(&o, v.fn_r16, 64 * v.wv, v.lds);
       v.occ_r16 = o < 1 ? 1 : o;
+      o = 0;
+      hipOccupancyMaxActiveBlocksPerMultiprocessor(&o, v.fn_two, 64 * v.wv, v.lds);
+      v.occ_two = o < 1 ? 1 : o;
+      o = 0;
+      if (v.fn_two_b16) hipOccupancyMaxActiveBlocksPerMultiprocessor(&o, v.fn_two_b16, 64 * v.wv, v.lds);
+      v.occ_two_b16 = o < 1 ? 1 : o;
     };
     for (SplitVariant &v : g_split_variants) prepare(v);
   });
@@ -1508,10 +1603,7 @@
   static const float min_rounds = getenv("SG_CONV_ROUNDS") ? atof(getenv("SG_CONV_ROUNDS")) : 2.5f;
   static const int at_env = getenv("SG_CONV_AT") ? atoi(getenv("SG_CONV_AT")) : 1;
   const int NB = (a.Cout + 31) / 32;
-  const unsigned long long row_bytes = (in16 ? 2ull : 4ull) * a.Cin;
-  const unsigned absent_at = static_cast<unsigned>((0xFFFFFFull * row_bytes) & 0xFFFFFFFFull);
-  const int use_at = ((at_env != 0 || in16) && a.Cin % 32 == 0 && in_bytes / static_cast<long long>(row_bytes) < (1LL << 24) - 1 &&
-                      static_cast<long long>(absent_at) >= in_bytes) ? 1 : 0;
+  const int use_at = ((at_env != 0 || in16) && line_wise_fits(a.Cin, in_bytes, in16)) ? 1 : 0;
   if (in16 && (!use_at || !b16)) {
     set_error("sg_unet_forward(bf16 rows): a layer with %d input channels / %lld input bytes cannot take the line-wise bf16 gather",
               a.Cin, in_bytes);
@@ -1545,6 +1637,21 @@
       if (g_split_variants[i].at == 1 && g_split_variants[i].nbw == 1 && g_split_variants[i].wv == kChainWV) pick = i;
   }
   const SplitVariant &v = g_split_variants[pick];
+  if (two && b16 && v.fn_two_b16 == nullptr) {
+    set_error("sg_spconv_gather_conv2_f32: the bf16-operand kernels with 16-channel items (%d input channels) have no "
+              "two-source form", a.Cin);
+    return SG_ERR_ARG;
+  }
+  if (two && a.in2 != nullptr) {
+    const long long pitch_a = 4LL * a.cin_a, pitch_b = 4LL * (a.Cin - a.cin_a);
+    const bool past = static_cast<long long>((0xFFFFFFull * pitch_a) & 0xFFFFFFFFull) >= in_a_bytes &&
+                      static_cast<long long>((0xFFFFFFull * pitch_b) & 0xFFFFFFFFull) >= static_cast<long long>(a.in2_bytes);
+    if (a.cin_a % v.ck != 0 || (v.at && !past)) {
+      set_error("sg_spconv_gather_conv2_f32: %d | %d input channels do not split into the %d-channel items of this "
+                "layer's kernel", a.cin_a, a.Cin - a.cin_a, v.ck);
+      return SG_ERR_ARG;
+    }
+  }
   a.col_units = NB / v.nbw;
   a.blocks_per_unit = v.nbw;
   const long long units = static_cast<long long>(num_tiles) * a.col_units * a.ksplit;
@@ -1554,7 +1661,7 @@
   a.magic_cu = magic(static_cast<unsigned>(a.col_units));
   a.magic_nsl = magic(static_cast<unsigned>(in16 ? (a.Cin + 63) / 64 : a.Cin / v.ck));
   if (t_chain.mode == 2) {
-    if (chain_layer && !in16 && !a.out16 && !a.res16 && (a.ksplit == 1 || a.done != nullptr) && stream == t_chain.stream) {
+    if (chain_layer && !two && !in16 && !a.out16 && !a.res16 && (a.ksplit == 1 || a.done != nullptr) && stream == t_chain.stream) {
       ChainStep st = {};
       st.kind = 0;
       st.in = a.in; st.w = a.w; st.post_scale = a.post_scale; st.post_shift = a.post_shift; st.residual = a.residual;
@@ -1573,10 +1680,14 @@
   static const int dyn_rounds_env = getenv("SG_CONV_DYN_ROUNDS") ? atoi(getenv("SG_CONV_DYN_ROUNDS")) : 2;
   a.queue = dyn_env ? take_tickets(stream) : nullptr;
   a.dyn_rounds = dyn_rounds_env == 1 ? 1 : 2;
-  long long g = static_cast<long long>(num_cu) * (in16 ? v.occ_r16 : b16 ? v.occ_b16 : v.occ);
+  long long g = static_cast<long long>(num_cu) * (two ? (b16 ? v.occ_two_b16 : v.occ_two) : in16 ? v.occ_r16 : b16 ? v.occ_b16 : v.occ);
   if (g >= 8) g -= g % 8;
   if (units < g) g = units >= 8 ? (units + 7) / 8 * 8 : units;
-  const unsigned ib = static_cast<unsigned>(in_bytes), wb = static_cast<unsigned>(w_bytes);
+  const unsigned ib = static_cast<unsigned>(two ? in_a_bytes : in_bytes), wb = static_cast<unsigned>(w_bytes);
+  if (two) {
+    (b16 ? v.fn_two_b16 : v.fn_two)<<<static_cast<int>(g), 64 * v.wv, v.lds, stream>>>(a, ib, wb);
+    return check_launch("sg_spconv_gather_conv2_f32");
+  }
   if (in16) {
     v.fn_r16<<<static_cast<int>(g), 64 * v.wv, v.lds, stream>>>(a, ib, wb);
     return check_launch("sg_spconv_gather_conv(bf16 rows)");
@@ -1706,12 +1817,35 @@
   return static_cast<size_t>(kMaxK) * M_out * Cout * sizeof(float) + 256;
 }
 
+struct ConvExtra {
+  const float *in2;
+  int cin_a;
+  const float *act2_scale, *act2_shift;
+  float *out_act2;
+};
+
+static int conv_arith_mode() {
+  static const int split_env = getenv("SG_CONV_SPLIT") ? atoi(getenv("SG_CONV_SPLIT")) : 1;
+  const int arith_ov = t_conv_arith >= 0 ? t_conv_arith : g_arith_override.load(std::memory_order_relaxed);
+  return arith_ov >= 0 ? arith_ov : split_env;
+}
+static int conv_split_min_cin() {
+  static const int v = getenv("SG_CONV_SPLIT_MIN_CIN") ? atoi(getenv("SG_CONV_SPLIT_MIN_CIN")) : 16;
+  return v;
+}
+static bool conv_combine_on() {
+  static const int combine_env = getenv("SG_CONV_COMBINE") ? atoi(getenv("SG_CONV_COMBINE")) : 1;
+  const int combine_ov = g_combine_override.load(std::memory_order_relaxed);
+  return (combine_ov >= 0 ? combine_ov : combine_env) != 0;
+}
+
 static int gather_conv_impl(const float *in, int num_in_rows, const int32_t *nbr, int M_out,
                             int K, int Cin, int Cout, const float *w_k8, const float *post_scale,
                             const float *post_shift, const float *residual, const float *act_scale,
                             const float *act_shift, float *out_act, const int32_t *order,
                             const uint32_t *tile_mask, const int32_t *nbr_tiles, float *out,
-                            void *ws, size_t ws_bytes, sg_stream_t stream_, int in16, int out16, int res16) {
+                            void *ws, size_t ws_bytes, sg_stream_t stream_, int in16, int out16, int res16,
+                            const ConvExtra *x = nullptr) {
   SG_REQUIRE(M_out >= 0 && K >= 1 && K <= kMaxK && Cin >= 1 && Cout >= 1,
              "sg_spconv_gather_conv_f32: bad arguments (M_out=%d K=%d Cin=%d Cout=%d)", M_out, K,
              Cin, Cout);
@@ -1736,6 +1870,7 @@
     }
   } prof_scope(stream, K > 1, M_out, K, Cin, Cout, num_in_rows);
   if (Cout % 4 != 0) {
+    SG_REQUIRE(x == nullptr, "sg_spconv_gather_conv2_f32: Cout = %d does not run on the persistent kernel", Cout);
     if (t_chain.mode == 2) {
       const int rc = chain_flush();
       if (rc != SG_OK) return rc;
@@ -1754,11 +1889,20 @@
                           static_cast<long long>(num_tiles) * kTileRows * K * 4 < (1LL << 31) &&
                           order != nullptr && tile_mask != nullptr && nbr_tiles != nullptr &&
                           reinterpret_cast<uintptr_t>(nbr_tiles) % 16 == 0;
-  static const int split_env = getenv("SG_CONV_SPLIT") ? atoi(getenv("SG_CONV_SPLIT")) : 1;
-  static const int split_min_cin = getenv("SG_CONV_SPLIT_MIN_CIN") ? atoi(getenv("SG_CONV_SPLIT_MIN_CIN")) : 16;
-  const int arith_ov = t_conv_arith >= 0 ? t_conv_arith : g_arith_override.load(std::memory_order_relaxed);
-  const int split_on = arith_ov >= 0 ? arith_ov : split_env;
-  const bool split = persistent && split_on != 0 && Cin >= split_min_cin;
+  const int split_on = conv_arith_mode();
+  const bool split = persistent && split_on != 0 && Cin >= conv_split_min_cin();
+  const bool two = x != nullptr;
+  const int cin_a = two && x->in2 != nullptr ? x->cin_a : Cin;
+  if (two) {
+    SG_REQUIRE(!in16 && !out16 && !res16, "sg_spconv_gather_conv2_f32: fp32 rows only");
+    SG_REQUIRE(x->in2 == nullptr || (x->cin_a > 0 && x->cin_a < Cin),
+               "sg_spconv_gather_conv2_f32: cin_a = %d must split the %d input channels", x->cin_a, Cin);
+    SG_REQUIRE((x->out_act2 == nullptr) == (x->act2_scale == nullptr) && (x->out_act2 == nullptr) == (x->act2_shift == nullptr),
+               "sg_spconv_gather_conv2_f32: act2_scale, act2_shift and out_act2 must come together");
+    SG_REQUIRE(persistent, "sg_spconv_gather_conv2_f32: a layer with K=%d Cin=%d Cout=%d, %d rows and %s tile plan does not run "
+               "on the persistent kernel", K, Cin, Cout, M_out, order && tile_mask && nbr_tiles ? "a" : "no");
+    SG_REQUIRE(cin_a % 16 == 0, "sg_spconv_gather_conv2_f32: cin_a = %d is not a multiple of the 16-channel items", cin_a);
+  }
   static const int target_env = getenv("SG_CONV_TARGET") ? atoi(getenv("SG_CONV_TARGET")) : 0;
   const int target = target_env > 0 ? target_env : split ? 1024 : 2048;
   const int waves_per_unit = persistent ? kWavesPerWg : 1;
@@ -1791,11 +1935,16 @@
   a.dyn_rounds = 2;
   a.out16 = out16;
   a.res16 = res16;
-  static const int combine_env = getenv("SG_CONV_COMBINE") ? atoi(getenv("SG_CONV_COMBINE")) : 1;
+  a.in2 = two ? x->in2 : nullptr;
+  a.in2_bytes = two && x->in2 ? static_cast<unsigned>(static_cast<long long>(num_in_rows) * (Cin - cin_a) * 4) : 0u;
+  a.cin_a = cin_a;
+  a.act2_scale = two ? x->act2_scale : nullptr;
+  a.act2_shift = two ? x->act2_shift : nullptr;
+  a.out_act2 = two ? x->out_act2 : nullptr;
+  const long long in_a_bytes_ll = static_cast<long long>(num_in_rows) * cin_a * 4;
   a.done = nullptr;
   a.out_final = out;
-  const int combine_ov = g_combine_override.load(std::memory_order_relaxed);
-  if ((combine_ov >= 0 ? combine_ov : combine_env) != 0 && persistent && ksplit > 1 &&
+  if (conv_combine_on() && persistent && ksplit > 1 &&
       static_cast<long long>(num_tiles) * col_units <= kDoneCounters)
     a.done = take_done(stream, static_cast<size_t>(num_tiles) * col_units);
   const long long units = static_cast<long long>(num_tiles) * col_units * ksplit;
@@ -1814,8 +1963,11 @@
                "persistent kernel", K, Cin, Cout);
     SG_REQUIRE(ksplit == 1 || a.done != nullptr, "sg_unet_forward(bf16 rows): an offset-split layer needs the in-launch combine");
   }
+  SG_REQUIRE(!two || a.out_act2 == nullptr || ksplit == 1 || a.done != nullptr,
+             "sg_spconv_gather_conv2_f32: the third output of an offset-split layer needs the in-launch combine");
   if (split) {
-    const int rc = launch_persistent_split(a, num_tiles, in_bytes_ll, w_bytes_ll, stream, split_on == 2, in16 != 0);
+    const int rc = launch_persistent_split(a, num_tiles, in_bytes_ll, w_bytes_ll, stream, split_on == 2, in16 != 0, two,
+                                           in_a_bytes_ll);
     if (rc != SG_OK) return rc;
     if (t_chain.mode == 2 && t_chain.args.n > 0) return SG_OK;
   } else if (persistent) {
@@ -1839,9 +1991,11 @@
     long long g = static_cast<long long>(num_cu) * occ;
     if (g >= 8) g -= g % 8;
     if (units < g) g = units >= 8 ? (units + 7) / 8 * 8 : units;
-    const unsigned ib_ = static_cast<unsigned>(in_bytes_ll), wb_ = static_cast<unsigned>(w_bytes_ll);
+    const unsigned ib_ = static_cast<unsigned>(in_a_bytes_ll), wb_ = static_cast<unsigned>(w_bytes_ll);
     static const char *trace_env = getenv("SG_CONV_TRACE");
-    if (trace_env) {
+    if (two) {
+      gather_conv_persistent_kernel<kSliceCh, 2, 0, 5, 1, 0, 4, 0, 0, 3><<<static_cast<int>(g), 256, lds, stream>>>(a, ib_, wb_);
+    } else if (trace_env) {
       const size_t nb = static_cast<size_t>(units) * kWavesPerWg * 8 * sizeof(unsigned long long);
       unsigned long long *dbuf = nullptr;
       hipMalloc(&dbuf, nb);
@@ -1892,9 +2046,34 @@
                           act_shift, out_act, order, tile_mask, nbr_tiles, out, ws, ws_bytes, stream_, 0, 0, 0);
 }
 
+int sg_spconv_gather_conv2_f32(const float *in, const float *in2, int cin_a, int num_in_rows, const int32_t *nbr,
+                               int M_out, int K, int Cin, int Cout, const float *w_k8, const float *post_scale,
+                               const float *post_shift, const float *residual, const float *act_scale,
+                               const float *act_shift, float *out_act, const float *act2_scale,
+                               const float *act2_shift, float *out_act2, const int32_t *order,
+                               const uint32_t *tile_mask, const int32_t *nbr_tiles, float *out, void *ws,
+                               size_t ws_bytes, sg_stream_t stream_) {
+  const ConvExtra x = {in2, cin_a, act2_scale, act2_shift, out_act2};
+  return gather_conv_impl(in, num_in_rows, nbr, M_out, K, Cin, Cout, w_k8, post_scale, post_shift, residual, act_scale,
+                          act_shift, out_act, order, tile_mask, nbr_tiles, out, ws, ws_bytes, stream_, 0, 0, 0, &x);
+}
+
 }
 
 namespace sg {
+bool conv_two_source_ok(int rows, int c) {
+  if (rows <= 0 || c % 16 != 0 || !conv_combine_on()) return false;
+  const long long cat_bytes = static_cast<long long>(rows) * 2 * c * 4, half_bytes = cat_bytes / 2;
+  const long long num_tiles = (rows + kTileRows - 1) / kTileRows;
+  if (cat_bytes >= (1LL << 31) || static_cast<long long>(rows) * c * 4 * kMaxK >= (1LL << 32) ||
+      num_tiles * kTileRows * kMaxK * 4 >= (1LL << 31))
+    return false;
+  static const int at_env = getenv("SG_CONV_AT") ? atoi(getenv("SG_CONV_AT")) : 1;
+  const bool split = conv_arith_mode() != 0 && 2 * c >= conv_split_min_cin();
+  if (!split || at_env == 0 || !line_wise_fits(2 * c, cat_bytes, false)) return conv_arith_mode() != 2;
+  return c % 32 == 0 && static_cast<long long>((0xFFFFFFull * (4ull * c)) & 0xFFFFFFFFull) >= half_bytes;
+}
+
 int conv_gather_rows(const void *in, int num_in_rows, const int32_t *nbr, int M_out, int K, int Cin, int Cout,
                      const float *w_k8, const float *post_scale, const float *post_shift, const void *residual,
                      const float *act_scale, const float *act_shift, void *out_act, const int32_t *order,
diff --git a/softgroup_amd/csrc/unet_exec.hip b/softgroup_amd/csrc/unet_exec.hip
--- a/softgroup_amd/csrc/unet_exec.hip
+++ b/softgroup_amd/csrc/unet_exec.hip
@@ -1,3 +1,4 @@
+#include <atomic>
 #include <map>
 #include <mutex>
 #include <utility>
@@ -308,6 +309,13 @@
 thread_local void (*t_unet_conv_hook)(void *) = nullptr;
 thread_local void *t_unet_conv_ctx = nullptr;
 
+struct Act {
+  const float *scale = nullptr, *shift = nullptr;
+  float *out = nullptr;
+};
+
+static std::atomic<long long> g_concat_in_place{0}, g_concat_passes{0};
+
 struct Exec {
   const sg_unet_desc *d;
   Arena ar;
@@ -351,20 +359,30 @@
     }
   };
 
-  struct Act {
-    const float *scale = nullptr, *shift = nullptr;
-    float *out = nullptr;
-  };
+  bool concat_knob = false;
+  bool two_source(int l) const {
+    const sg_unet_level &L = d->levels[l];
+    return !concat_knob && !r16 && !conv_chain_recording() && L.tail[0].w_i != nullptr &&
+           L.tail[0].cin == 2 * L.planes && conv_two_source_ok(idx[l].rows, L.planes);
+  }
 
   int conv(const float *in, int in_rows, const Plan &p, int cin, int cout, const float *w,
            const float *post_s, const float *post_b, const float *residual, const Act &act, float *out,
-           bool in_f32 = false, bool out_f32 = false) {
+           bool in_f32 = false, bool out_f32 = false, const float *in2 = nullptr, int cin_a = 0,
+           const Act &act2 = Act()) {
     if (p.rows == 0) return SG_OK;
     const size_t m = ar.mark();
     const size_t nb = sg_spconv_conv_workspace_bytes(p.rows, cout);
     void *ws = nullptr;
     if (nb > 256) {
       ws = ar.take<char>(nb);
+    }
+    if (in2 != nullptr || act2.out != nullptr) {
+      const int rc2 = sg_spconv_gather_conv2_f32(in, in2, cin_a, in_rows, p.nbr, p.rows, p.kvol, cin, cout, w, post_s,
+                                                 post_b, residual, act.scale, act.shift, act.out, act2.scale, act2.shift,
+                                                 act2.out, p.order, p.tile_mask, p.nbr_tiles, out, ws, ws ? nb : 0, stream);
+      ar.release(m);
+      return rc2;
     }
     const int rc = !r16 ? sg_spconv_gather_conv_f32(in, in_rows, p.nbr, p.rows, p.kvol, cin, cout, w, post_s,
                                                     post_b, residual, act.scale, act.shift, act.out, p.order,
@@ -378,17 +396,18 @@
 
   int block(const sg_unet_block &b, const float *x, const float *xa, int rows, const Plan &subm,
             const Plan &ident, const float *post_s, const float *post_b, const Act &next, float *out,
-            bool out_f32 = false) {
+            bool out_f32 = false, const float *x2 = nullptr, const float *xa2 = nullptr, int cin_a = 0,
+            const Act &next2 = Act()) {
     const size_t m = ar.mark();
     const float *shortcut = x;
     if (b.w_i != nullptr) {
       SG_ALLOC(sc, float, fsz(static_cast<size_t>(rows) * b.cout));
-      SG_TRY(conv(x, rows, ident, b.cin, b.cout, b.w_i, nullptr, nullptr, nullptr, Act(), sc));
+      SG_TRY(conv(x, rows, ident, b.cin, b.cout, b.w_i, nullptr, nullptr, nullptr, Act(), sc, false, false, x2, cin_a));
       shortcut = sc;
     }
     SG_ALLOC(h, float, fsz(static_cast<size_t>(rows) * b.cout));
-    SG_TRY(conv(xa, rows, subm, b.cin, b.cout, b.w1, b.bn2_scale, b.bn2_shift, nullptr, Act(), h));
-    SG_TRY(conv(h, rows, subm, b.cout, b.cout, b.w2, post_s, post_b, shortcut, next, out, false, out_f32));
+    SG_TRY(conv(xa, rows, subm, b.cin, b.cout, b.w1, b.bn2_scale, b.bn2_shift, nullptr, Act(), h, false, false, xa2, cin_a));
+    SG_TRY(conv(h, rows, subm, b.cout, b.cout, b.w2, post_s, post_b, shortcut, next, out, false, out_f32, nullptr, 0, next2));
     ar.release(m);
     return SG_OK;
   }
@@ -403,6 +422,8 @@
     const int rows = I.rows;
     const Plan &subm = I.subm, &ident = I.ident;
     const size_t feat = fsz(static_cast<size_t>(rows ? rows : 1) * c);
+    const bool two = deeper && two_source(l);
+    float *tb = nullptr;
     if (pre_in != nullptr) {
       SG_ALLOC(x0, float, feat);
       SG_ALLOC(x0a, float, feat);
@@ -439,8 +460,14 @@
         next.shift = last ? L.down_bn_shift : L.blocks[i + 1].bn1_shift;
       }
       const bool fin = last && !deeper;
+      Act skip;
+      if (last && two) {
+        SG_ALLOC(tb_, float, feat);
+        tb = tb_;
+        skip = Act{L.tail[0].bn1_scale, L.tail[0].bn1_shift, tb};
+      }
       SG_TRY(block(L.blocks[i], cur, cur_a, rows, subm, ident, fin ? post_s : nullptr,
-                   fin ? post_b : nullptr, next, dst, fin && l == 0));
+                   fin ? post_b : nullptr, next, dst, fin && l == 0, nullptr, nullptr, 0, skip));
       cur = dst;
       cur_a = next.out;
     }
@@ -460,9 +487,22 @@
         SG_TRY(level(l + 1, y, ya, nullptr, 0, L.up_bn_scale, L.up_bn_shift, z));
         SG_TRY(chain.close());
       }
-      SG_ALLOC(cat, float, 2 * feat);
-      SG_ALLOC(cata, float, 2 * feat);
-      {
+      const float *cur2 = nullptr, *cur2_a = nullptr;
+      float *cat = nullptr, *cata = nullptr;
+      (two ? g_concat_in_place : g_concat_passes).fetch_add(1, std::memory_order_relaxed);
+      if (two) {
+        SG_ALLOC(upf, float, feat);
+        SG_ALLOC(upf_a, float, feat);
+        SG_TRY(conv(z, rows2, up, c2, c, L.up_w, nullptr, nullptr, nullptr,
+                    Act{L.tail[0].bn1_scale + c, L.tail[0].bn1_shift + c, upf_a}, upf));
+        cur2 = upf;
+        cur2_a = upf_a;
+        cur_a = tb;
+      } else {
+        SG_ALLOC(cat_, float, 2 * feat);
+        SG_ALLOC(cata_, float, 2 * feat);
+        cat = cat_;
+        cata = cata_;
         const size_t m = ar.mark();
         SG_ALLOC(upf, float, feat);
         SG_TRY(conv(z, rows2, up, c2, c, L.up_w, nullptr, nullptr, nullptr, Act(), upf));
@@ -480,9 +520,9 @@
               reinterpret_cast<const float4 *>(L.tail[0].bn1_shift), reinterpret_cast<float4 *>(cat),
               reinterpret_cast<float4 *>(cata));
         ar.release(m);
-      }
-      cur = cat;
-      cur_a = cata;
+        cur = cat;
+        cur_a = cata;
+      }
       for (int i = 0; i < L.n_blocks; ++i) {
         const bool last = i == L.n_blocks - 1;
         float *dst = out;
@@ -494,7 +534,8 @@
           next = Act{L.tail[i + 1].bn1_scale, L.tail[i + 1].bn1_shift, ta};
         }
         SG_TRY(block(L.tail[i], cur, cur_a, rows, subm, ident, last ? post_s : nullptr,
-                     last ? post_b : nullptr, next, dst, last && l == 0));
+                     last ? post_b : nullptr, next, dst, last && l == 0, i == 0 ? cur2 : nullptr,
+                     i == 0 ? cur2_a : nullptr, c));
         cur = dst;
         cur_a = next.out;
       }
@@ -541,6 +582,12 @@
   for (int l = 0; l < d->n_levels; ++l)
     total += rows * 12 * 2 * static_cast<size_t>(d->levels[l].planes) * 4 + (64 << 10);
   return total;
+}
+
+int sg_unet_concat_stats(int64_t *in_place, int64_t *passes) {
+  if (in_place) *in_place = g_concat_in_place.load(std::memory_order_relaxed);
+  if (passes) *passes = g_concat_passes.load(std::memory_order_relaxed);
+  return SG_OK;
 }
 
 int sg_unet_forward(const sg_unet_desc *d, const float *feats, const int32_t *indices, int num_rows,
@@ -630,6 +677,7 @@
   Exec ex(d, rest + used, rest_bytes - used, stream, li);
   ex.perm = pre ? perm : nullptr;
   ex.r16 = rows16;
+  ex.concat_knob = getenv("SG_UNET_CONCAT") != nullptr && atoi(getenv("SG_UNET_CONCAT")) != 0;
   int rc;
   {
     Exec::ChainScope chain(ex, !pre && ex.chain_from(0));
```

New measurement: 427.0. 1.7% lower.
